# omerbt/Splice

Measured on AMD Instinct MI355X. Metric: opt_steps_per_sec, higher is better.
Workload: dtype bf16

## Files before the change

### include/splice_hip.h

```cpp
#ifndef SPLICE_HIP_H
#define SPLICE_HIP_H
#include <stddef.h>
#include <stdint.h>

#ifdef __cplusplus
extern "C" {
#endif

typedef uint16_t splice_bf16;
typedef void* splice_stream_t;

#define SPLICE_OK 0
#define SPLICE_ERR_ARG -1
#define SPLICE_ERR_HIP -2
#define SPLICE_ERR_STATE -3
#define SPLICE_ERR_NOMEM -4

int splice_version(void);
int splice_dev_switches(void);
const char* splice_last_error(void);

typedef struct splice_gemm_epilogue {
    const float* bias;
    const float* resid;
    int ldr, resid_mod;
    float* out_f32;
    int ldo;
    splice_bf16* out_bf;
    int ldbf;
    splice_bf16* out_bf_t;
    int ldt;
    splice_bf16* out_pre;
    int ldp, pre_row_lo;
    const splice_bf16* aux;
    int ldaux;
    float* out_f32_cols;
    int ld_cols, col_lo, col_hi;
    float alpha;
    int ksplit;
    long long slab_stride;
    const splice_bf16* rd_other;
    int ld_rd, rd_rows;
    float* rowdot;
    const float* row_scale;
    const float* col_scale;
    uint8_t* out_f8;
    int ld8;
    uint8_t* out_f8_t;
    int ldt8;
} splice_gemm_epilogue;

enum {
    SPLICE_EPI_BIAS = 1, SPLICE_EPI_RESID = 2, SPLICE_EPI_OUT_F32 = 4, SPLICE_EPI_OUT_BF = 8,
    SPLICE_EPI_OUT_T = 16, SPLICE_EPI_GELU = 32, SPLICE_EPI_GELU_GRAD = 64,
    SPLICE_EPI_COLS_F32 = 128, SPLICE_EPI_ALPHA = 256, SPLICE_EPI_ROWDOT = 512, SPLICE_EPI_SCALE_RC = 1024, SPLICE_EPI_OUT_F8 = 2048,
    SPLICE_EPI_OUT_F8T = 4096
};

int splice_gemm_nt_bf16(unsigned flags, const splice_bf16* A, int lda, const splice_bf16* B, int ldb,
                        int M, int N, int K, const splice_gemm_epilogue* epi, splice_stream_t stream);

int splice_gemm_nt_fp8(unsigned flags, const uint8_t* A, int lda, const uint8_t* B, int ldb, int M, int N, int K,
                       const splice_gemm_epilogue* epi, splice_stream_t stream);
int splice_quantize_rows_fp8(const float* x, int ldx, uint8_t* q, int ldq, float* scale, int rows, int cols, splice_stream_t stream);
int splice_gemm_splitk_slabs(int M, int ksplit);
int splice_gemm_force_tile(int tile);
int splice_attention_variant(int variant);
int splice_attention_qfold(int on);
int splice_attention_bwd_variant(int variant);

int splice_layernorm_fwd(const float* x, const float* gamma, const float* beta, splice_bf16* y,
                         float* mean, float* rstd, int rows, int D, float eps, splice_stream_t stream);
int splice_layernorm_bwd(const float* dy, const float* x, const float* gamma, const float* mean,
                         const float* rstd, const float* g_in, float* g_out, splice_bf16* g_out_bf,
                         int rows, int D, splice_stream_t stream);

int splice_attention_fwd(const splice_bf16* qkv, const splice_bf16* qkvT, int ldt, int B, int T, int Tld,
                         int D, int H, float scale, splice_bf16* out, float* lse, splice_stream_t stream);
int splice_attention_fwd_fp8(const uint8_t* qkv8, const uint8_t* qkvT8, int ldt8, int B, int T, int Tld, int D, int H, float scale,
                             splice_bf16* out, float* lse, splice_stream_t stream);
int splice_attention_bwd(const splice_bf16* qkv, const splice_bf16* qkvT, int ldt, int B, int T, int Tld,
                         int D, int H, float scale, const splice_bf16* out, const float* lse,
                         const splice_bf16* dout, const splice_bf16* doutT, float* delta,
                         splice_bf16* dqkv, splice_stream_t stream);
int splice_attention_probs(const splice_bf16* qkv, int B, int T, int Tld, int D, int H, float scale,
                           const float* lse, float* probs, splice_stream_t stream);

int splice_augment_structure(const float* img, float* out, float* scratch, int H, int W, int flip, int n_ops, const int* order,
                             const float* factors, float blur_sigma, splice_stream_t stream);

size_t splice_keys_selfsim_ws_bytes(int T, int D);
int splice_keys_selfsim_fwd(const float* K, int ldk, int T, int D, float eps, float* S, void* ws,
                            splice_stream_t stream);
int splice_keys_selfsim_bwd(const float* dS, const float* S, int T, int D, float eps, float* dK, int lddk,
                            int accumulate, void* ws, splice_stream_t stream);

int splice_mse(const float* a, int lda, const float* b, int ldb, int rows, int cols, float weight,
               float* loss_accum, float* grad, int ldg, splice_stream_t stream);

int splice_patchify(const float* img, splice_bf16* patches, int B, int H, int W, int p, int Tld,
                    int normalize, splice_stream_t stream);
int splice_unpatchify(const float* dpatches, float* dimg, int B, int H, int W, int p, int Tld,
                      int normalize, splice_stream_t stream);
int splice_cast_f32_bf16(const float* x, splice_bf16* y, size_t n, splice_stream_t stream);
int splice_cast_bf16_f32(const splice_bf16* x, float* y, size_t n, splice_stream_t stream);
int splice_transpose_f32_bf16(const float* x, splice_bf16* y, int rows, int cols, int ldy, splice_stream_t stream);
int splice_resize_bilinear_fwd(const float* in, float* out, int planes, int h, int w, int oh, int ow, splice_stream_t stream);
int splice_resize_bilinear_bwd(const float* dout, float* din, int planes, int h, int w, int oh, int ow, splice_stream_t stream);

int splice_vit_create(int patch, int dim, int depth, int heads, void** out_handle);
void splice_vit_destroy(void* vit);
int splice_vit_set_param(void* vit, const char* name, const float* data, long long numel, splice_stream_t stream);
float splice_vit_qscale(void* vit);
int splice_vit_params_complete(void* vit);
int splice_vit_enable_fp8(void* vit, splice_stream_t stream);
int splice_vit_ctx_create(void* vit, int B, int H, int W, const float* pos_TD, int need_grad,
                          splice_stream_t stream, void** out_ctx);
void splice_vit_ctx_destroy(void* ctx);
int splice_vit_ctx_info(void* ctx, int* T, int* Tld, int* rows);
int splice_vit_ctx_set_top_cls_only(void* ctx, int on);
int splice_vit_ctx_set_fp8(void* ctx, int mode);
int splice_vit_forward(void* ctx, const float* img, int normalize, splice_stream_t stream);
int splice_vit_forward_ex(void* ctx, const float* img, int normalize, int grad_pass_begin, splice_stream_t stream);
int splice_vit_forward_passes(void* ctx, const float* img, int normalize, int grad_pass_begin, int pass_begin, int pass_end,
                              splice_stream_t stream);
int splice_vit_get_tensor(void* ctx, int kind, int layer, void** out_ptr);
int splice_vit_read_tensor(void* ctx, int kind, int layer, void* dst, size_t bytes, splice_stream_t stream);
int splice_vit_backward(void* ctx, int pass_begin, int pass_end, const float* const* d_block,
                        const float* const* d_qkv, const float* const* d_keys, float* d_img,
                        int normalize, splice_stream_t stream);

int splice_gen_create(void** out_handle);
// ... 106 lines not shown
int splice_step_stop_state(void* step, splice_stop_state* out, splice_stream_t stream);
int splice_step_restore(void* step, int next_step_idx, const splice_stop_state* stop, splice_stream_t stream);
int splice_step_set_input_rows(void* step, int pairs_in, const int* rows);
int splice_plateau_update(splice_stop_state* state, const float* losses8, int pairs, int window, float rel, int patience, int min_steps,
                          int step_idx, int counted, splice_stream_t stream);

int splice_step_set_ema(void* step, float* ema, float decay, int start);
int splice_optim_step_pairs_ema(int kind, float* params, float* grads, const float* g2, float* m, float* v, float* ema, int n_pairs,
                                long long stride, long long n, const float* lr_dev, float hp0, float hp1, float eps, const int* step_dev,
                                const splice_stop_state* stop, int zero_grad, float ema_decay, int ema_start, splice_stream_t stream);

#define SPLICE_CLIP_CHUNK 4096
typedef struct splice_clip_state {
    float sumsq;
    float norm;
    float coef;
    int skip;
    int clipped;
    int skipped;
} splice_clip_state;
int splice_grad_norm_pairs(const float* grads, const float* g2, int n_pairs, long long stride, long long n, float max_norm, float* partials,
                           splice_clip_state* state, const splice_stop_state* stop, const int* step_dev, splice_stream_t stream);
int splice_optim_step_pairs_clip(int kind, float* params, float* grads, const float* g2, float* m, float* v, float* ema, int n_pairs,
                                 long long stride, long long n, const float* lr_dev, float hp0, float hp1, float eps, const int* step_dev,
                                 const splice_stop_state* stop, int zero_grad, float ema_decay, int ema_start, const splice_clip_state* clip,
                                 splice_stream_t stream);
int splice_optim_step_clip(int kind, float* params, float* grads, const float* g2, float* m, float* v, float* ema, long long n, float lr,
                           const float* lr_dev, float hp0, float hp1, float eps, int step, int zero_grad, float ema_decay, int ema_start,
                           const splice_clip_state* clip, splice_stream_t stream);
int splice_step_set_grad_clip(void* step, float max_norm, splice_clip_state* state);

typedef struct splice_clip_auto_state {
    float ref[2];
    int count[2];
    float thr;
    int regime;
} splice_clip_auto_state;
int splice_grad_norm_pairs_auto(const float* grads, const float* g2, int n_pairs, long long stride, long long n, float max_norm, float k,
                                float beta, int warmup, int regime, float* partials, splice_clip_state* state,
                                splice_clip_auto_state* auto_state, const splice_stop_state* stop, const int* step_dev,
                                splice_stream_t stream);
int splice_step_set_grad_clip_auto(void* step, float max_norm, float k, float beta, int warmup, splice_clip_state* state,
                                   splice_clip_auto_state* auto_state);

#define SPLICE_STOP_HISTORY 64
typedef struct splice_best_state {
    int best_step;
    int best_window;
} splice_best_state;
int splice_plateau_update_best(splice_stop_state* state, splice_best_state* best, float* means, const float* losses8, int pairs, int window,
                               float rel, int patience, int min_steps, int step_idx, int counted, splice_stream_t stream);
int splice_optim_step_pairs_best(int kind, float* params, float* grads, const float* g2, float* m, float* v, float* ema, int n_pairs,
                                 long long stride, long long n, const float* lr_dev, float hp0, float hp1, float eps, const int* step_dev,
                                 const splice_stop_state* stop, int zero_grad, float ema_decay, int ema_start, const splice_clip_state* clip,
                                 const splice_best_state* best, float* best_params, float* best_ema, splice_stream_t stream);
int splice_optim_step_pairs_ext(int kind, float* params, float* grads, const float* g2, float* m, float* v, float* w, float* ema, int n_pairs,
                                long long stride, long long n, const float* lr_dev, float hp0, float hp1, float eps, int step,
                                const int* step_dev, const splice_stop_state* stop, int zero_grad, float ema_decay, int ema_start,
                                const splice_clip_state* clip, const splice_best_state* best, float* best_params, float* best_ema,
                                const splice_optim_ext* options, splice_stream_t stream);
int splice_step_set_optimizer_ext(void* step, const splice_optim_ext* options, float* w);
int splice_step_set_keep_best(void* step, float* best_params, float* best_ema, splice_best_state* state, float* means);

int splice_step_set_loss_trace(void* step, float* trace, int capacity);

typedef struct splice_lr_state {
    float scale;
    int bad;
    int cuts;
    int last_cut_step;
} splice_lr_state;
int splice_step_set_lr_plateau(void* step, float factor, int patience, float min_scale, splice_lr_state* state, int* cut_steps);
int splice_plateau_update_lr(splice_stop_state* state, splice_lr_state* lr_state, int* cut_steps, const float* losses8, const float* lr_in,
                             int per_pair, float* lr_eff, int pairs, int window, float rel, int patience, int min_steps, float factor,
                             int lr_patience, float min_scale, int step_idx, int counted, splice_stream_t stream);

size_t splice_selfsim_loss_pairs_ws_bytes(int T, int D, int pairs);
int splice_selfsim_loss_pairs(const splice_bf16* k_tgt, const splice_bf16* k_x, int ldk, size_t k_pstride, const splice_bf16* kT_x, int ldt,
                              size_t kT_pstride, int T, int D, int pairs, float lambda, const float* e_scale_tab, int fp8, float eps,
                              float* loss_part, size_t part_pstride, float* dk, int lddk, size_t dk_pstride, void* ws, splice_stream_t stream);
int splice_mse_pairs(const float* a, int lda, size_t a_ps, const float* b, int ldb, size_t b_ps, int rows, int cols, float loss_weight,
                     float grad_weight, float* part, size_t part_ps, float* grad, int ldg, size_t g_ps, int pairs, const float* grad_tab,
                     splice_stream_t stream);
int splice_total_loss_pairs(float* lbase, size_t lstride, int lp, float w_ssim, float w_essim, float w_ecls, float w_cls, float w_id,
                            float* out8, int pairs, int n_a, int n_b, int n_c, int n_e, const float* wtab, int ssim_on, int entire,
                            splice_stream_t stream);
int splice_total_loss_pairs_trace(float* lbase, size_t lstride, int lp, float w_ssim, float w_essim, float w_ecls, float w_cls, float w_id,
                                  float* out8, int pairs, int n_a, int n_b, int n_c, int n_e, const float* wtab, int ssim_on, int entire,
                                  splice_stop_state* stop, int window, float rel, int patience, int min_steps, const int* dev_t,
                                  float* trace, int capacity, splice_stream_t stream);

int splice_attn_cls_fwd(const splice_bf16* qkv, const splice_bf16* qkvT, int ldt, int B, int T, int Tld, int D, int H, float scale, splice_bf16* out,
                        float* probs, splice_stream_t stream);
int splice_attn_cls_bwd(const splice_bf16* qkv, const splice_bf16* qkvT, int ldt, int B, int T, int Tld, int D, int H, float scale, const float* probs,
                        const float* dout_slabs, int n_slabs, size_t slab_stride, splice_bf16* dqkv, splice_stream_t stream);
int splice_ln_rows_fwd(float* x, size_t xs, const float* gamma, const float* beta, splice_bf16* y, size_t ys, float* mean, float* rstd, size_t ss,
                       int rows, int D, float eps, const float* slabs, int n_slabs, size_t slab_stride, const float* bias, const float* resid, size_t rs,
                       splice_stream_t stream);
int splice_ln_rows_bwd(float* dy, size_t dys, const float* x, size_t xs, const float* gamma, const float* mean, const float* rstd, size_t ss, float* g,
                       splice_bf16* g_bf, int rows, int D, int n_slabs, size_t slab_stride, splice_stream_t stream);
int splice_rows_finish(int mode, const float* slabs, int n_slabs, size_t slab_stride, int rows, int N, const float* bias, const float* resid, size_t rs,
                       float* out_f32, size_t os, splice_bf16* out_bf, splice_bf16* pre_bf, const splice_bf16* aux, size_t ps, int pre_lo,
                       splice_stream_t stream);

typedef struct splice_gen_conv_args {
    const float* in;
    const float* w;
    const float* bias;
    float* out;
    size_t in_nstride, in_cstride, out_nstride, out_cstride, w_jstride, w_cstride, p_nstride;
    int N, Cin, Hi, Wi, Cout, Ho, Wo, ks, stride, pad;
    int reflect, act, transposed, accumulate;
    float* ws;
    size_t ws_floats;
    int p_group, defer_reduce;
} splice_gen_conv_args;
#define SPLICE_GEN_CONV_FORM_INTS 5
int splice_gen_conv(const splice_gen_conv_args* args, int* form_out, splice_stream_t stream);
int splice_gen_conv_pair(const splice_gen_conv_args* a, const splice_gen_conv_args* b, int* forms_out, splice_stream_t stream);
int splice_gen_conv_reflect_dgrad(const splice_gen_conv_args* args, float* pad_scratch, size_t scratch_floats, splice_stream_t stream);

typedef struct splice_gen_wgrad_args {
    const float* x;
    const float* dy;
    float* ws;
    size_t ws_floats;
    size_t x_nstride, x_cstride, dy_nstride, dy_cstride;
    int N, Cin, Hi, Wi, Cout, Ho, Wo, ks, stride, pad, reflect;
} splice_gen_wgrad_args;
#define SPLICE_GEN_WGRAD_FORM_INTS 6
size_t splice_gen_conv_wgrad_ws_floats(int N, int Cin, int Cout, int ks, int Ho, int Wo);
int splice_gen_conv_wgrad(const splice_gen_wgrad_args* args, float* dw, int accumulate, int n_img, size_t p_nstride, int* form_out,
                          splice_stream_t stream);
int splice_gen_wgrad_reduce(const float* partials, int n, int chunks, float* dw, int accumulate, int n_img, size_t p_nstride, splice_stream_t stream);

typedef struct splice_gen_bn_args {
    float* y;
    float* out;
    size_t y_nstride, out_nstride;
    int N, C, HW, batch;
    const float* gamma;
    const float* beta;
    float eps, slope;
    size_t p_nstride;
    float* part;
    size_t part_floats;
    float* mean;
    float* rstd;
    const float* up_src;
    float* up_d_src;
    size_t up_src_ns, up_d_src_ns;
    int up_c0, up_h, up_w, up_Ho, up_Wo;
    const float* slabs;
    const float* bias;
    int ksplit;
    const float* da;
    float* dy;
    size_t da_nstride, dy_nstride;
    float* dgamma;
    float* dbeta;
    int accumulate;
    const float* da_slabs;
    int da_ksplit, da_accumulate;
    float* pre_y;
    size_t pre_y_ns;
    const float* pre_slabs;
    const float* pre_bias;
    int pre_ksplit, pre_C;
    const float* pre_gamma;
    const float* pre_beta;
    float* pre_mean;
    float* pre_rstd;
    float pre_slope;
    float* pre_dy;
    float* pre_dgamma;
    float* pre_dbeta;
} splice_gen_bn_args;
#define SPLICE_GEN_BN_FORM_INTS 7
// ... 19 lines not shown
```

### splice_amd/_lib.py

```python
import ctypes as C
import os

_HERE = os.path.dirname(os.path.abspath(__file__))
LIB_PATH = os.path.join(_HERE, "libsplice_hip.so")

_lib = None


class GemmEpilogue(C.Structure):
    _fields_ = [
        ("bias", C.c_void_p), ("resid", C.c_void_p), ("ldr", C.c_int), ("resid_mod", C.c_int),
        ("out_f32", C.c_void_p), ("ldo", C.c_int),
        ("out_bf", C.c_void_p), ("ldbf", C.c_int),
        ("out_bf_t", C.c_void_p), ("ldt", C.c_int),
        ("out_pre", C.c_void_p), ("ldp", C.c_int), ("pre_row_lo", C.c_int),
        ("aux", C.c_void_p), ("ldaux", C.c_int),
        ("out_f32_cols", C.c_void_p), ("ld_cols", C.c_int), ("col_lo", C.c_int), ("col_hi", C.c_int),
        ("alpha", C.c_float), ("ksplit", C.c_int), ("slab_stride", C.c_longlong),
        ("rd_other", C.c_void_p), ("ld_rd", C.c_int), ("rd_rows", C.c_int), ("rowdot", C.c_void_p),
        ("row_scale", C.c_void_p), ("col_scale", C.c_void_p),
        ("out_f8", C.c_void_p), ("ld8", C.c_int),
        ("out_f8_t", C.c_void_p), ("ldt8", C.c_int),
    ]


class GenArch(C.Structure):
    _fields_ = [("n_scales", C.c_int), ("in_channels", C.c_int), ("out_channels", C.c_int),
                ("down", C.c_int * 6), ("up", C.c_int * 6), ("skip", C.c_int * 6),
                ("filter_down", C.c_int * 6), ("filter_up", C.c_int * 6), ("filter_skip", C.c_int), ("reflect", C.c_int)]


class StepConfig(C.Structure):
    _fields_ = [
        ("crop_h", C.c_int), ("crop_w", C.c_int), ("vit_h", C.c_int), ("vit_w", C.c_int),
        ("ent_h", C.c_int), ("ent_w", C.c_int), ("ent_vit_h", C.c_int), ("ent_vit_w", C.c_int),
        ("lambda_global_cls", C.c_float), ("lambda_global_ssim", C.c_float), ("lambda_global_identity", C.c_float),
        ("lambda_entire_cls", C.c_float), ("lambda_entire_ssim", C.c_float),
        ("entire_every", C.c_int), ("cls_warmup", C.c_int),
        ("lr", C.c_float), ("beta1", C.c_float), ("beta2", C.c_float), ("eps", C.c_float),
        ("pairs", C.c_int), ("arena_stride", C.c_longlong), ("fp8_selfsim", C.c_int), ("top_cls_only", C.c_int), ("n_crops", C.c_int), ("n_crops_b", C.c_int),
    ]


class StopState(C.Structure):
    _fields_ = [("sum", C.c_float), ("count", C.c_int), ("windows", C.c_int), ("best", C.c_float), ("bad", C.c_int), ("stop_step", C.c_int)]


class ClipState(C.Structure):
    _fields_ = [("sumsq", C.c_float), ("norm", C.c_float), ("coef", C.c_float), ("skip", C.c_int), ("clipped", C.c_int), ("skipped", C.c_int)]


class ClipAutoState(C.Structure):
    _fields_ = [("ref", C.c_float * 2), ("count", C.c_int * 2), ("thr", C.c_float), ("regime", C.c_int)]


class BestState(C.Structure):
    _fields_ = [("best_step", C.c_int), ("best_window", C.c_int)]


class LrState(C.Structure):
    _fields_ = [("scale", C.c_float), ("bad", C.c_int), ("cuts", C.c_int), ("last_cut_step", C.c_int)]


class OptimExt(C.Structure):
    _fields_ = [("weight_decay", C.c_float), ("momentum", C.c_float), ("dampening", C.c_float), ("nesterov", C.c_int), ("decoupled", C.c_int),
                ("amsgrad", C.c_int), ("centered", C.c_int)]


def optim_ext(options):
    if isinstance(options, OptimExt):
        return options
    return OptimExt(float(options.get("weight_decay", 0.0)), float(options.get("momentum", 0.0)), float(options.get("dampening", 0.0)),
                    int(bool(options.get("nesterov", False))), int(bool(options.get("decoupled", False))), int(bool(options.get("amsgrad", False))),
                    int(bool(options.get("centered", False))))


class GenConvArgs(C.Structure):
    _fields_ = [("in", C.c_void_p), ("w", C.c_void_p), ("bias", C.c_void_p), ("out", C.c_void_p)] + \
               [(n, C.c_size_t) for n in ("in_nstride", "in_cstride", "out_nstride", "out_cstride", "w_jstride", "w_cstride", "p_nstride")] + \
               [(n, C.c_int) for n in ("N", "Cin", "Hi", "Wi", "Cout", "Ho", "Wo", "ks", "stride", "pad", "reflect", "act", "transposed", "accumulate")] + \
               [("ws", C.c_void_p), ("ws_floats", C.c_size_t), ("p_group", C.c_int), ("defer_reduce", C.c_int)]


class GenWgradArgs(C.Structure):
    _fields_ = [("x", C.c_void_p), ("dy", C.c_void_p), ("ws", C.c_void_p), ("ws_floats", C.c_size_t)] + \
               [(n, C.c_size_t) for n in ("x_nstride", "x_cstride", "dy_nstride", "dy_cstride")] + \
               [(n, C.c_int) for n in ("N", "Cin", "Hi", "Wi", "Cout", "Ho", "Wo", "ks", "stride", "pad", "reflect")]


class GenBnArgs(C.Structure):
    _fields_ = [("y", C.c_void_p), ("out", C.c_void_p), ("y_nstride", C.c_size_t), ("out_nstride", C.c_size_t),
                ("N", C.c_int), ("C", C.c_int), ("HW", C.c_int), ("batch", C.c_int),
                ("gamma", C.c_void_p), ("beta", C.c_void_p), ("eps", C.c_float), ("slope", C.c_float), ("p_nstride", C.c_size_t),
                ("part", C.c_void_p), ("part_floats", C.c_size_t), ("mean", C.c_void_p), ("rstd", C.c_void_p),
                ("up_src", C.c_void_p), ("up_d_src", C.c_void_p), ("up_src_ns", C.c_size_t), ("up_d_src_ns", C.c_size_t),
                ("up_c0", C.c_int), ("up_h", C.c_int), ("up_w", C.c_int), ("up_Ho", C.c_int), ("up_Wo", C.c_int),
                ("slabs", C.c_void_p), ("bias", C.c_void_p), ("ksplit", C.c_int),
                ("da", C.c_void_p), ("dy", C.c_void_p), ("da_nstride", C.c_size_t), ("dy_nstride", C.c_size_t),
                ("dgamma", C.c_void_p), ("dbeta", C.c_void_p), ("accumulate", C.c_int),
                ("da_slabs", C.c_void_p), ("da_ksplit", C.c_int), ("da_accumulate", C.c_int),
                ("pre_y", C.c_void_p), ("pre_y_ns", C.c_size_t), ("pre_slabs", C.c_void_p), ("pre_bias", C.c_void_p),
                ("pre_ksplit", C.c_int), ("pre_C", C.c_int), ("pre_gamma", C.c_void_p), ("pre_beta", C.c_void_p),
                ("pre_mean", C.c_void_p), ("pre_rstd", C.c_void_p), ("pre_slope", C.c_float),
                ("pre_dy", C.c_void_p), ("pre_dgamma", C.c_void_p), ("pre_dbeta", C.c_void_p)]


GEN_CONV_FORM_INTS, GEN_WGRAD_FORM_INTS, GEN_BN_FORM_INTS = 5, 6, 7

STOP_HISTORY = 64

EPI_BIAS, EPI_RESID, EPI_OUT_F32, EPI_OUT_BF, EPI_OUT_T = 1, 2, 4, 8, 16
EPI_GELU, EPI_GELU_GRAD, EPI_COLS_F32, EPI_ALPHA, EPI_ROWDOT, EPI_SCALE_RC, EPI_OUT_F8, EPI_OUT_F8T = 32, 64, 128, 256, 512, 1024, 2048, 4096

_vp, _i, _f, _sz, _u = C.c_void_p, C.c_int, C.c_float, C.c_size_t, C.c_uint

_SIGNATURES = {
    "splice_version": ([], C.c_int),
    "splice_dev_switches": ([], C.c_int),
    "splice_last_error": ([], C.c_char_p),
    "splice_gemm_nt_bf16": ([_u, _vp, _i, _vp, _i, _i, _i, _i, C.POINTER(GemmEpilogue), _vp], _i),
    "splice_gemm_nt_fp8": ([_u, _vp, _i, _vp, _i, _i, _i, _i, C.POINTER(GemmEpilogue), _vp], _i),
    "splice_quantize_rows_fp8": ([_vp, _i, _vp, _i, _vp, _i, _i, _vp], _i),
    "splice_gemm_splitk_slabs": ([_i, _i], _i),
    "splice_gemm_force_tile": ([_i], _i),
    "splice_attention_variant": ([_i], _i),
    "splice_attention_qfold": ([_i], _i),
    "splice_attention_bwd_variant": ([_i], _i),
    "splice_layernorm_fwd": ([_vp, _vp, _vp, _vp, _vp, _vp, _i, _i, _f, _vp], _i),
    "splice_layernorm_bwd": ([_vp, _vp, _vp, _vp, _vp, _vp, _vp, _vp, _i, _i, _vp], _i),
    "splice_attention_fwd": ([_vp, _vp, _i, _i, _i, _i, _i, _i, _f, _vp, _vp, _vp], _i),
    "splice_attention_fwd_fp8": ([_vp, _vp, _i, _i, _i, _i, _i, _i, _f, _vp, _vp, _vp], _i),
    "splice_attention_bwd": ([_vp, _vp, _i, _i, _i, _i, _i, _i, _f, _vp, _vp, _vp, _vp, _vp, _vp, _vp], _i),
    "splice_attention_probs": ([_vp, _i, _i, _i, _i, _i, _f, _vp, _vp, _vp], _i),
    "splice_augment_structure": ([_vp, _vp, _vp, _i, _i, _i, _i, C.POINTER(C.c_int), C.POINTER(C.c_float), _f, _vp], _i),
    "splice_keys_selfsim_ws_bytes": ([_i, _i], _sz),
    "splice_keys_selfsim_fwd": ([_vp, _i, _i, _i, _f, _vp, _vp, _vp], _i),
    "splice_keys_selfsim_bwd": ([_vp, _vp, _i, _i, _f, _vp, _i, _i, _vp, _vp], _i),
    "splice_mse": ([_vp, _i, _vp, _i, _i, _i, _f, _vp, _vp, _i, _vp], _i),
    "splice_selfsim_loss_pairs_ws_bytes": ([_i, _i, _i], _sz),
    "splice_selfsim_loss_pairs": ([_vp, _vp, _i, _sz, _vp, _i, _sz, _i, _i, _i, _f, _vp, _i, _f, _vp, _sz, _vp, _i, _sz, _vp, _vp], _i),
    "splice_mse_pairs": ([_vp, _i, _sz, _vp, _i, _sz, _i, _i, _f, _f, _vp, _sz, _vp, _i, _sz, _i, _vp, _vp], _i),
    "splice_total_loss_pairs": ([_vp, _sz, _i, _f, _f, _f, _f, _f, _vp, _i, _i, _i, _i, _i, _vp, _i, _i, _vp], _i),
    "splice_attn_cls_fwd": ([_vp, _vp, _i, _i, _i, _i, _i, _i, _f, _vp, _vp, _vp], _i),
    "splice_attn_cls_bwd": ([_vp, _vp, _i, _i, _i, _i, _i, _i, _f, _vp, _vp, _i, _sz, _vp, _vp], _i),
    "splice_ln_rows_fwd": ([_vp, _sz, _vp, _vp, _vp, _sz, _vp, _vp, _sz, _i, _i, _f, _vp, _i, _sz, _vp, _vp, _sz, _vp], _i),
    "splice_ln_rows_bwd": ([_vp, _sz, _vp, _sz, _vp, _vp, _vp, _sz, _vp, _vp, _i, _i, _i, _sz, _vp], _i),
    "splice_rows_finish": ([_i, _vp, _i, _sz, _i, _i, _vp, _vp, _sz, _vp, _sz, _vp, _vp, _vp, _sz, _i, _vp], _i),
    "splice_gen_conv": ([C.POINTER(GenConvArgs), C.POINTER(_i), _vp], _i),
    "splice_gen_conv_pair": ([C.POINTER(GenConvArgs), C.POINTER(GenConvArgs), C.POINTER(_i), _vp], _i),
    "splice_gen_conv_reflect_dgrad": ([C.POINTER(GenConvArgs), _vp, _sz, _vp], _i),
    "splice_gen_conv_wgrad_ws_floats": ([_i, _i, _i, _i, _i, _i], _sz),
    "splice_gen_conv_wgrad": ([C.POINTER(GenWgradArgs), _vp, _i, _i, _sz, C.POINTER(_i), _vp], _i),
    "splice_gen_wgrad_reduce": ([_vp, _i, _i, _vp, _i, _i, _sz, _vp], _i),
    "splice_gen_bn_small_instance": ([_i], _i),
    "splice_gen_bn_form": ([_i, _i, _sz, _i, C.POINTER(_i)], _i),
    "splice_gen_bn_part_floats": ([_i, _i], _sz),
    "splice_gen_bn_fwd": ([C.POINTER(GenBnArgs), _vp], _i),
    "splice_gen_bn_bwd": ([C.POINTER(GenBnArgs), _vp], _i),
    "splice_gen_upsample2x_fwd": ([_vp, _sz, _vp, _sz, _i, _i, _i, _i, _i, _i, _vp], _i),
    "splice_gen_upsample2x_bwd": ([_vp, _sz, _vp, _sz, _i, _i, _i, _i, _i, _i, _vp], _i),
    "splice_gen_sigmoid_bias_part_floats": ([_i, _i], _sz),
    "splice_gen_sigmoid_bwd_bias": ([_vp, _vp, _vp, _i, _i, _i, _vp, _sz, _sz, _i, C.POINTER(_i), _vp], _i),
    "splice_patchify": ([_vp, _vp, _i, _i, _i, _i, _i, _i, _vp], _i),
    "splice_unpatchify": ([_vp, _vp, _i, _i, _i, _i, _i, _i, _vp], _i),
    "splice_cast_f32_bf16": ([_vp, _vp, _sz, _vp], _i),
    "splice_cast_bf16_f32": ([_vp, _vp, _sz, _vp], _i),
    "splice_transpose_f32_bf16": ([_vp, _vp, _i, _i, _i, _vp], _i),
    "splice_resize_bilinear_fwd": ([_vp, _vp, _i, _i, _i, _i, _i, _vp], _i),
    "splice_resize_bilinear_bwd": ([_vp, _vp, _i, _i, _i, _i, _i, _vp], _i),
    "splice_vit_create": ([_i, _i, _i, _i, C.POINTER(_vp)], _i),
    "splice_vit_destroy": ([_vp], None),
    "splice_vit_set_param": ([_vp, C.c_char_p, _vp, C.c_longlong, _vp], _i),
    "splice_vit_params_complete": ([_vp], _i),
    "splice_vit_enable_fp8": ([_vp, _vp], _i),
    "splice_vit_ctx_create": ([_vp, _i, _i, _i, _vp, _i, _vp, C.POINTER(_vp)], _i),
    "splice_vit_ctx_destroy": ([_vp], None),
    "splice_vit_ctx_info": ([_vp, C.POINTER(_i), C.POINTER(_i), C.POINTER(_i)], _i),
    "splice_vit_ctx_set_top_cls_only": ([_vp, _i], _i),
    "splice_vit_ctx_set_fp8": ([_vp, _i], _i),
    "splice_vit_forward": ([_vp, _vp, _i, _vp], _i),
    "splice_vit_forward_ex": ([_vp, _vp, _i, _i, _vp], _i),
    "splice_vit_forward_passes": ([_vp, _vp, _i, _i, _i, _i, _vp], _i),
    "splice_vit_get_tensor": ([_vp, _i, _i, C.POINTER(_vp)], _i),
    "splice_vit_qscale": ([_vp], C.c_float),
    "splice_vit_read_tensor": ([_vp, _i, _i, _vp, _sz, _vp], _i),
    "splice_vit_backward": ([_vp, _i, _i, C.POINTER(_vp), C.POINTER(_vp), C.POINTER(_vp), _vp, _i, _vp], _i),
    "splice_gen_create": ([C.POINTER(_vp)], _i),
    "splice_gen_create_arch": ([C.POINTER(GenArch), C.POINTER(_vp)], _i),
    "splice_gen_destroy": ([_vp], None),
    "splice_gen_param_count": ([_vp], C.c_longlong),
    "splice_gen_num_tensors": ([_vp], _i),
    "splice_gen_tensor_info": ([_vp, _i, C.POINTER(C.c_char_p), C.POINTER(C.c_longlong), C.POINTER(C.c_longlong)], _i),
    "splice_gen_plan_create": ([_vp, _i, _i, _i, _i, C.POINTER(_vp)], _i),
    "splice_gen_plan_destroy": ([_vp], None),
    "splice_gen_forward": ([_vp, _vp, _vp, _vp, _vp], _i),
    "splice_gen_forward_borrowed": ([_vp, _vp, _vp, _vp, _vp], _i),
    "splice_gen_backward": ([_vp, _vp, _vp, _vp, _i, _vp], _i),
    "splice_adam_step": ([_vp, _vp, _vp, _vp, C.c_longlong, _f, _f, _f, _f, _i, _i, _vp], _i),
    "splice_optim_step": ([_i, _vp, _vp, _vp, _vp, C.c_longlong, _f, _f, _f, _f, _i, _i, _vp], _i),
    "splice_optim_step_ex": ([_i, _vp, _vp, _vp, _vp, _vp, C.c_longlong, _f, _vp, _f, _f, _f, _i, _i, _vp], _i),
    "splice_optim_step_pairs": ([_i, _vp, _vp, _vp, _vp, _vp, _i, C.c_longlong, C.c_longlong, _vp, _f, _f, _f, _i, _i, _vp], _i),
    "splice_optim_step_ema": ([_i, _vp, _vp, _vp, _vp, _vp, _vp, C.c_longlong, _f, _vp, _f, _f, _f, _i, _i, _f, _i, _vp], _i),
    "splice_optim_step_pairs_ema": ([_i, _vp, _vp, _vp, _vp, _vp, _vp, _i, C.c_longlong, C.c_longlong, _vp, _f, _f, _f, _vp, _vp, _i, _f, _i, _vp], _i),
    "splice_step_set_ema": ([_vp, _vp, _f, _i], _i),
    "splice_grad_norm_pairs": ([_vp, _vp, _i, C.c_longlong, C.c_longlong, _f, _vp, _vp, _vp, _vp, _vp], _i),
    "splice_optim_step_pairs_clip": ([_i, _vp, _vp, _vp, _vp, _vp, _vp, _i, C.c_longlong, C.c_longlong, _vp, _f, _f, _f, _vp, _vp, _i, _f, _i, _vp, _vp], _i),
    "splice_optim_step_clip": ([_i, _vp, _vp, _vp, _vp, _vp, _vp, C.c_longlong, _f, _vp, _f, _f, _f, _i, _i, _f, _i, _vp, _vp], _i),
    "splice_step_set_grad_clip": ([_vp, _f, _vp], _i),
    "splice_grad_norm_pairs_auto": ([_vp, _vp, _i, C.c_longlong, C.c_longlong, _f, _f, _f, _i, _i, _vp, _vp, _vp, _vp, _vp, _vp], _i),
    "splice_step_set_grad_clip_auto": ([_vp, _f, _f, _f, _i, _vp, _vp], _i),
    "splice_plateau_update_best": ([_vp, _vp, _vp, _vp, _i, _i, _f, _i, _i, _i, _i, _vp], _i),
    "splice_optim_step_pairs_best": ([_i, _vp, _vp, _vp, _vp, _vp, _vp, _i, C.c_longlong, C.c_longlong, _vp, _f, _f, _f, _vp, _vp, _i, _f, _i, _vp, _vp, _vp, _vp, _vp], _i),
    "splice_step_set_keep_best": ([_vp, _vp, _vp, _vp, _vp], _i),
    "splice_step_set_loss_trace": ([_vp, _vp, _i], _i),
    "splice_total_loss_pairs_trace": ([_vp, _sz, _i, _f, _f, _f, _f, _f, _vp, _i, _i, _i, _i, _i, _vp, _i, _i, _vp, _i, _f, _i, _i, _vp, _vp, _i, _vp], _i),
    "splice_step_set_lr_plateau": ([_vp, _f, _i, _f, _vp, _vp], _i),
    "splice_plateau_update_lr": ([_vp, _vp, _vp, _vp, _vp, _i, _vp, _i, _i, _f, _i, _i, _f, _i, _f, _i, _i, _vp], _i),
    "splice_optim_step_ext": ([_i, _vp, _vp, _vp, _vp, _vp, _vp, C.c_longlong, _f, _vp, _f, _f, _f, _i, _i, C.POINTER(OptimExt), _vp], _i),
    "splice_optim_step_pairs_ext": ([_i, _vp, _vp, _vp, _vp, _vp, _vp, _vp, _i, C.c_longlong, C.c_longlong, _vp, _f, _f, _f, _i, _vp, _vp, _i, _f, _i, _vp, _vp,
                                     _vp, _vp, C.POINTER(OptimExt), _vp], _i),
    "splice_step_set_optimizer_ext": ([_vp, C.POINTER(OptimExt), _vp], _i),
    "splice_prof_begin": ([_i], _i),
    "splice_prof_end": ([C.POINTER(_f), C.POINTER(_i)], _i),
    "splice_prof_end_ex": ([C.POINTER(_f), C.POINTER(_i), C.POINTER(_i)], _i),
    "splice_prof_end_detail": ([C.POINTER(_f), C.POINTER(_i), C.POINTER(_i), C.c_char_p, _i], _i),
    "splice_prof_active": ([], _i),
    "splice_step_use_graph": ([_vp, _i], _i),
# ... 69 lines not shown
```

### splice_amd/csrc/capi.hip

```cpp
#include <stdarg.h>
#include <stdio.h>

#include "gen_kernels.h"
#include "kernels.h"

static thread_local char g_err[512] = "";

void splice_set_error(const char* fmt, ...) {
    va_list ap;
    va_start(ap, fmt);
    vsnprintf(g_err, sizeof(g_err), fmt, ap);
    va_end(ap);
}

static int finish(int rc, const char* what) {
    if (rc != SPLICE_OK) {
        splice_set_error("%s: invalid argument", what);
        return rc;
    }
    const hipError_t e = hipGetLastError();
    if (e != hipSuccess) {
        splice_set_error("%s: HIP error %d (%s)", what, (int)e, hipGetErrorString(e));
        return SPLICE_ERR_HIP;
    }
// ... 52 lines not shown
    a.qkv = qkv; a.qkvT = qkvT; a.ldt = ldt; a.B = B; a.T = T; a.Tld = Tld; a.D = D; a.H = H; a.scale = scale;
    a.out = out; a.lse = lse; a.qfold = attn_qfold_hook();
    return finish(attn_fwd_launch(&a, ST(stream)), "splice_attention_fwd");
}
int splice_attention_fwd_fp8(const uint8_t* qkv8, const uint8_t* qkvT8, int ldt8, int B, int T, int Tld, int D, int H, float scale,
                             splice_bf16* out, float* lse, splice_stream_t stream) {
    if (!qkv8 || !qkvT8 || !out || !lse) return finish(SPLICE_ERR_ARG, "splice_attention_fwd_fp8");
    AttnArgs a = {};
    a.qkv8 = qkv8; a.qkvT8 = qkvT8; a.ldt8 = ldt8; a.ldt = 4; a.B = B; a.T = T; a.Tld = Tld; a.D = D; a.H = H; a.scale = scale;
    a.out = out; a.lse = lse;
    return finish(attn_fwd_launch(&a, ST(stream)), "splice_attention_fwd_fp8");
}
int splice_attention_bwd(const splice_bf16* qkv, const splice_bf16* qkvT, int ldt, int B, int T, int Tld, int D, int H,
                         float scale, const splice_bf16* out, const float* lse, const splice_bf16* dout,
                         const splice_bf16* doutT, float* delta, splice_bf16* dqkv, splice_stream_t stream) {
    AttnArgs a = {};
    a.qkv = qkv; a.qkvT = qkvT; a.ldt = ldt; a.B = B; a.T = T; a.Tld = Tld; a.D = D; a.H = H; a.scale = scale;
    a.out = const_cast<splice_bf16*>(out); a.lse = const_cast<float*>(lse);
    a.dout = dout; a.doutT = doutT; a.delta = delta; a.dqkv = dqkv; a.qfold = attn_qfold_hook();
    return finish(attn_bwd_launch(&a, ST(stream)), "splice_attention_bwd");
}
int splice_attention_probs(const splice_bf16* qkv, int B, int T, int Tld, int D, int H, float scale, const float* lse,
                           float* probs, splice_stream_t stream) {
    AttnArgs a = {};
    a.qkv = qkv; a.B = B; a.T = T; a.Tld = Tld; a.D = D; a.H = H; a.scale = scale; a.lse = const_cast<float*>(lse);
    return finish(attn_probs_launch(&a, probs, ST(stream)), "splice_attention_probs");
}

int splice_augment_structure(const float* img, float* out, float* scratch, int H, int W, int flip, int n_ops, const int* order,
                             const float* factors, float blur_sigma, splice_stream_t stream) {
    return finish(augment_structure_launch(img, out, scratch, H, W, flip, n_ops, order, factors, blur_sigma, ST(stream)), "splice_augment_structure");
}

size_t splice_keys_selfsim_ws_bytes(int T, int D) { return selfsim_ws_bytes(T, D); }
int splice_keys_selfsim_fwd(const float* K, int ldk, int T, int D, float eps, float* S, void* ws, splice_stream_t stream) {
    SelfSimWs w;
    selfsim_ws_carve(ws, T, D, &w);
    return finish(selfsim_fwd_launch(K, ldk, T, D, eps, S, w, ST(stream)), "splice_keys_selfsim_fwd");
}
int splice_keys_selfsim_bwd(const float* dS, const float* S, int T, int D, float eps, float* dK, int lddk, int accumulate,
                            void* ws, splice_stream_t stream) {
    SelfSimWs w;
    selfsim_ws_carve(ws, T, D, &w);
    return finish(selfsim_bwd_launch(dS, S, T, D, eps, dK, lddk, accumulate, w, ST(stream)), "splice_keys_selfsim_bwd");
}
int splice_mse(const float* a, int lda, const float* b, int ldb, int rows, int cols, float weight, float* loss_accum,
               float* grad, int ldg, splice_stream_t stream) {
    return finish(mse_launch(a, lda, b, ldb, rows, cols, weight, loss_accum, grad, ldg, ST(stream)), "splice_mse");
}

size_t splice_selfsim_loss_pairs_ws_bytes(int T, int D, int pairs) { return selfsim_batch_ws_bytes(T, D, pairs); }
int splice_selfsim_loss_pairs(const splice_bf16* k_tgt, const splice_bf16* k_x, int ldk, size_t k_pstride, const splice_bf16* kT_x, int ldt,
                              size_t kT_pstride, int T, int D, int pairs, float lambda, const float* e_scale_tab, int fp8, float eps,
                              float* loss_part, size_t part_pstride, float* dk, int lddk, size_t dk_pstride, void* ws, splice_stream_t stream) {
    const char* who = "splice_selfsim_loss_pairs";
    if (!k_tgt || !k_x || !kT_x || !loss_part || !dk || !ws || T < 1 || pairs < 1 || D < 64 || D % 64 || ldk < D || ldk % 8 || ldt % 8 ||
        k_pstride % 8 || kT_pstride % 8 || lddk < D)
        return finish(SPLICE_ERR_ARG, who);
    const int nt = (T + 63) / 64;
    if ((fp8 && D % 128) || (size_t)(nt * (nt + 1) / 2) > part_pstride) return finish(SPLICE_ERR_ARG, who);
    SelfSimBatch b = {};
    selfsim_batch_carve(ws, T, D, pairs, &b);
    b.ldk = ldk; b.ldt = ldt; b.k_pstride = k_pstride; b.kT_pstride = kT_pstride;
    b.k_tgt = k_tgt; b.k_x = k_x; b.kT_x = kT_x;
    b.loss_part = loss_part; b.part_pstride = part_pstride;
    b.dk = dk; b.dk_pstride = dk_pstride; b.lddk = lddk;
    b.eps = eps;
    b.fp8 = fp8 != 0;
    b.loss_scale = 1.0f / ((float)T * (float)T);
    b.e_scale = 4.0f * lambda * b.loss_scale;
    b.e_scale_tab = e_scale_tab;
    const int rc = selfsim_target_launch(b, ST(stream));
    if (rc != SPLICE_OK) return finish(rc, who);
    return finish(selfsim_loss_launch(b, ST(stream)), who);
}
int splice_mse_pairs(const float* a, int lda, size_t a_ps, const float* b, int ldb, size_t b_ps, int rows, int cols, float loss_weight,
                     float grad_weight, float* part, size_t part_ps, float* grad, int ldg, size_t g_ps, int pairs, const float* grad_tab,
                     splice_stream_t stream) {
    if (!a || !b || rows < 1 || cols < 1) return finish(SPLICE_ERR_ARG, "splice_mse_pairs");
    return finish(mse_batched_launch(a, lda, a_ps, b, ldb, b_ps, rows, cols, loss_weight, grad_weight, part, part_ps, grad, ldg, g_ps, pairs,
                                     ST(stream), grad_tab),
                  "splice_mse_pairs");
}

static bool attn_cls_args_ok(const void* qkv, const void* qkvT, int ldt, int B, int T, int Tld, int D, int H, size_t lds) {
    if (!qkv || !qkvT || B < 1 || T < 1 || T > Tld || Tld % 32 || ldt % 8 || (long long)ldt < (long long)B * Tld || D < 64 || D % 64 || H != D / 64)
        return false;
    int dev = 0, lim = 0;
    if (hipGetDevice(&dev) != hipSuccess || hipDeviceGetAttribute(&lim, hipDeviceAttributeMaxSharedMemoryPerBlock, dev) != hipSuccess) return false;
    return lds <= (size_t)(lim < 65536 ? lim : 65536);
}
int splice_attn_cls_fwd(const splice_bf16* qkv, const splice_bf16* qkvT, int ldt, int B, int T, int Tld, int D, int H, float scale, splice_bf16* out,
                        float* probs, splice_stream_t stream) {
    const char* who = "splice_attn_cls_fwd";
    if (!out || !probs || !attn_cls_args_ok(qkv, qkvT, ldt, B, T, Tld, D, H, ((size_t)Tld + Tld / 2 + 256 + 8) * sizeof(float)))
        return finish(SPLICE_ERR_ARG, who);
    return finish(attn_cls_fwd_launch(qkv, qkvT, ldt, B, T, Tld, D, H, scale, out, probs, ST(stream)), who);
}
int splice_attn_cls_bwd(const splice_bf16* qkv, const splice_bf16* qkvT, int ldt, int B, int T, int Tld, int D, int H, float scale, const float* probs,
                        const float* dout_slabs, int n_slabs, size_t slab_stride, splice_bf16* dqkv, splice_stream_t stream) {
    const char* who = "splice_attn_cls_bwd";
    if (!probs || !dout_slabs || !dqkv || n_slabs < 1 || n_slabs > 16 ||
        !attn_cls_args_ok(qkv, qkvT, ldt, B, T, Tld, D, H, ((size_t)Tld + Tld / 2 + 64 + 64 + 32 + 256 + 8) * sizeof(float)))
        return finish(SPLICE_ERR_ARG, who);
    return finish(attn_cls_bwd_launch(qkv, qkvT, ldt, B, T, Tld, D, H, scale, probs, dout_slabs, n_slabs, slab_stride, dqkv, ST(stream)), who);
}
int splice_ln_rows_fwd(float* x, size_t xs, const float* gamma, const float* beta, splice_bf16* y, size_t ys, float* mean, float* rstd, size_t ss,
                       int rows, int D, float eps, const float* slabs, int n_slabs, size_t slab_stride, const float* bias, const float* resid, size_t rs,
                       splice_stream_t stream) {
    const char* who = "splice_ln_rows_fwd";
    if (!x || !gamma || !beta || !y || !mean || !rstd || (slabs && (n_slabs < 1 || !bias || !resid))) return finish(SPLICE_ERR_ARG, who);
    return finish(ln_rows_fwd_launch(x, xs, gamma, beta, y, ys, mean, rstd, ss, rows, D, eps, slabs, n_slabs, slab_stride, bias, resid, rs, ST(stream)), who);
}
int splice_ln_rows_bwd(float* dy, size_t dys, const float* x, size_t xs, const float* gamma, const float* mean, const float* rstd, size_t ss, float* g,
                       splice_bf16* g_bf, int rows, int D, int n_slabs, size_t slab_stride, splice_stream_t stream) {
    const char* who = "splice_ln_rows_bwd";
    if (!dy || !x || !gamma || !mean || !rstd || !g || !g_bf) return finish(SPLICE_ERR_ARG, who);
    return finish(ln_rows_bwd_launch(dy, dys, x, xs, gamma, mean, rstd, ss, g, g_bf, rows, D, n_slabs, slab_stride, ST(stream)), who);
}
int splice_rows_finish(int mode, const float* slabs, int n_slabs, size_t slab_stride, int rows, int N, const float* bias, const float* resid, size_t rs,
                       float* out_f32, size_t os, splice_bf16* out_bf, splice_bf16* pre_bf, const splice_bf16* aux, size_t ps, int pre_lo,
                       splice_stream_t stream) {
    const char* who = "splice_rows_finish";
    if (mode < 0 || mode > 2 || !slabs || n_slabs < 1 || rows < 1 || N < 1 || (long long)rows * N > 0x7fffffffLL) return finish(SPLICE_ERR_ARG, who);
    if ((mode == 0 && (!out_f32 || !resid)) || (mode != 0 && !out_bf) || (mode == 2 && !aux)) return finish(SPLICE_ERR_ARG, who);
    return finish(rows_finish_launch(mode, slabs, n_slabs, slab_stride, rows, N, bias, resid, rs, out_f32, os, out_bf, pre_bf, aux, ps, pre_lo, ST(stream)), who);
}

static bool gen_conv_args_ok(const splice_gen_conv_args* g, bool reflect_dgrad) {
    if (!g || !g->in || !g->w || !g->out) return false;
    if (g->N < 1 || g->Cin < 1 || g->Hi < 1 || g->Wi < 1 || g->Cout < 1 || g->Ho < 1 || g->Wo < 1 || g->pad < 0) return false;
    if (g->ks != 1 && g->ks != 3 && g->ks != 5 && g->ks != 7) return false;
    if (g->stride != 1 && g->stride != 2) return false;
    if ((g->act != 0 && g->act != 1) || (g->reflect && g->transposed && !reflect_dgrad)) return false;
    const long long HWi = (long long)g->Hi * g->Wi, HWo = (long long)g->Ho * g->Wo;
    if (HWi > 0x1fffffffLL || HWo > 0x1fffffffLL) return false;
    if (g->in_cstride < (size_t)HWi || g->out_cstride < (size_t)HWo) return false;
    if (g->N > 1 && (g->in_nstride < (size_t)g->Cin * g->in_cstride || g->out_nstride < (size_t)g->Cout * g->out_cstride)) return false;
    if ((size_t)g->Cin * g->in_cstride > 0x1fffffffULL) return false;
    if ((size_t)g->Cout * g->w_jstride + (size_t)g->Cin * g->w_cstride + (size_t)g->ks * g->ks > 0x1fffffffULL) return false;
    if ((size_t)g->Cout * g->out_cstride > 0x7fffffffULL) return false;
    if (g->w_jstride < 1 || g->w_cstride < 1) return false;
    if (g->p_group < 0 || (g->p_group > 1 && (!g->p_nstride || g->N % g->p_group))) return false;
    if (g->reflect && !reflect_dgrad && (g->pad >= g->Hi || g->pad >= g->Wi)) return false;
    if (reflect_dgrad && (g->pad >= g->Ho || g->pad >= g->Wo || g->act)) return false;
    if (g->ws && g->ws_floats < 1) return false;
    if (g->defer_reduce && !g->ws) return false;
    return true;
}
static ConvArgs gen_conv_fill(const splice_gen_conv_args* g) {
    ConvArgs a = {};
    a.in = g->in; a.w = g->w; a.bias = g->bias; a.out = g->out;
    a.in_nstride = g->in_nstride; a.in_cstride = g->in_cstride; a.out_nstride = g->out_nstride; a.out_cstride = g->out_cstride;
    a.w_jstride = g->w_jstride; a.w_cstride = g->w_cstride; a.p_nstride = g->p_nstride;
    a.N = g->N; a.Cin = g->Cin; a.Hi = g->Hi; a.Wi = g->Wi; a.Cout = g->Cout; a.Ho = g->Ho; a.Wo = g->Wo;
    a.ks = g->ks; a.stride = g->stride; a.pad = g->pad;
    a.reflect = g->reflect; a.act = g->act; a.transposed = g->transposed; a.accumulate = g->accumulate;
    a.ws = g->ws; a.ws_floats = g->ws_floats; a.p_group = g->p_group; a.defer_reduce = g->defer_reduce;
    return a;
}
int splice_gen_conv(const splice_gen_conv_args* args, int* form_out, splice_stream_t stream) {
    const char* who = "splice_gen_conv";
    if (!gen_conv_args_ok(args, false)) return finish(SPLICE_ERR_ARG, who);
    const ConvArgs a = gen_conv_fill(args);
    if (form_out) conv_form_report(a, form_out);
    return finish(conv_launch(a, ST(stream)), who);
}
int splice_gen_conv_pair(const splice_gen_conv_args* a_args, const splice_gen_conv_args* b_args, int* forms_out, splice_stream_t stream) {
    const char* who = "splice_gen_conv_pair";
    if (!gen_conv_args_ok(a_args, false) || !gen_conv_args_ok(b_args, false)) return finish(SPLICE_ERR_ARG, who);
    const ConvArgs a = gen_conv_fill(a_args), b = gen_conv_fill(b_args);
    if (forms_out) { conv_form_report(a, forms_out); conv_form_report(b, forms_out + SPLICE_GEN_CONV_FORM_INTS); }
    return finish(conv_pair_launch(a, b, ST(stream)), who);
}
int splice_gen_conv_reflect_dgrad(const splice_gen_conv_args* args, float* pad_scratch, size_t scratch_floats, splice_stream_t stream) {
    const char* who = "splice_gen_conv_reflect_dgrad";
    if (!gen_conv_args_ok(args, true) || !pad_scratch) return finish(SPLICE_ERR_ARG, who);
    const size_t Hp = (size_t)args->Ho + 2 * args->pad, Wp = (size_t)args->Wo + 2 * args->pad;
    if (scratch_floats < (size_t)args->N * args->Cout * Hp * Wp || (size_t)args->Cout * Hp * Wp > 0x7fffffffULL) return finish(SPLICE_ERR_ARG, who);
    return finish(conv_reflect_dgrad_launch(gen_conv_fill(args), pad_scratch, ST(stream)), who);
}

static bool gen_wgrad_args_ok(const splice_gen_wgrad_args* g) {
    if (!g || !g->x || !g->dy) return false;
    if (g->N < 1 || g->Cin < 1 || g->Hi < 1 || g->Wi < 1 || g->Cout < 1 || g->Ho < 1 || g->Wo < 1 || g->pad < 0 || g->pad > 255) return false;
    if (g->ks != 1 && g->ks != 3 && g->ks != 5 && g->ks != 7) return false;
    if ((g->stride != 1 && g->stride != 2) || g->Cout > 128) return false;
    if (g->Hi > 65535 || g->Wi > 65535 || g->Ho > 65535 || g->Wo > 65535 || g->Cin > 65535) return false;
// ... 173 lines not shown
```

### splice_amd/csrc/gemm.h

```cpp
#pragma once
#include <atomic>
#include "common.h"

constexpr int GEMM_BK = 64;

typedef int mx8_t __attribute__((ext_vector_type(8)));
__device__ __forceinline__ f32x4 mfma16_fp8_mx(const u32x4& a0, const u32x4& a1, const u32x4& b0, const u32x4& b1, f32x4 c) {
    const mx8_t av = {(int)a0[0], (int)a0[1], (int)a0[2], (int)a0[3], (int)a1[0], (int)a1[1], (int)a1[2], (int)a1[3]};
    const mx8_t bv = {(int)b0[0], (int)b0[1], (int)b0[2], (int)b0[3], (int)b1[0], (int)b1[1], (int)b1[2], (int)b1[3]};
    return __builtin_amdgcn_mfma_scale_f32_16x16x128_f8f6f4(av, bv, c, 0 , 0 , 0, 0x7F7F7F7F, 0, 0x7F7F7F7F);
}

template <int BM, int BN, bool SWAP = false, bool FP8 = false, int WGM = 2>
struct GemmTile {
    static constexpr int NW = 2 * WGM;
    static constexpr int WROWS = BM / WGM;
    static constexpr int FM = WROWS / 16;
    static constexpr int FN = BN / 32;
    static constexpr int A_LOADS = BM * 8 / (64 * NW);
    static constexpr int B_LOADS = BN * 8 / (64 * NW);
    static constexpr int LDS_ELEMS = (BM + BN) * GEMM_BK;
    f32x4 acc[FM][FN];

    __device__ __forceinline__ void slice_mfma(const bf16_t* As, const bf16_t* Bs, int wm, int wn, int frow, int fchunk) {
// ... 268 lines not shown
        for (int j = 0; j < FN; ++j) { ssb[j] += __shfl_xor(ssb[j], 16, 64); ssb[j] += __shfl_xor(ssb[j], 32, 64); }
    }

    template <class F>
    __device__ __forceinline__ void for_each_cols(int m0, int n0, F&& f) {
        static_assert(SWAP, "for_each_cols needs the swapped fragment layout");
        const int lane = threadIdx.x & 63, wave = threadIdx.x >> 6;
        const int wm = wave >> 1, wn = wave & 1;
#pragma unroll
        for (int i = 0; i < FM; ++i)
#pragma unroll
            for (int j = 0; j < FN; ++j)
                f(m0 + wm * WROWS + i * 16 + (lane & 15), n0 + wn * (BN / 2) + j * 16 + (lane >> 4) * 4, acc[i][j]);
    }

    template <class F>
    __device__ __forceinline__ void for_each(int m0, int n0, F&& f) {
        const int lane = threadIdx.x & 63, wave = threadIdx.x >> 6;
        const int wm = wave >> 1, wn = wave & 1;
#pragma unroll
        for (int i = 0; i < FM; ++i)
#pragma unroll
            for (int j = 0; j < FN; ++j)
                f(m0 + wm * WROWS + i * 16 + (lane >> 4) * 4, n0 + wn * (BN / 2) + j * 16 + (lane & 15), acc[i][j]);
    }
};

constexpr int GEMM_VSPLIT_ROWS = 2401;
static inline int gemm_splitk_slabs(int M, int ks) { return (ks > 1 && M >= GEMM_VSPLIT_ROWS) ? 1 : ks; }

typedef splice_gemm_epilogue GemmEpi;
enum : unsigned {
    EPI_BIAS = SPLICE_EPI_BIAS, EPI_RESID = SPLICE_EPI_RESID, EPI_OUT_F32 = SPLICE_EPI_OUT_F32,
    EPI_OUT_BF = SPLICE_EPI_OUT_BF, EPI_OUT_T = SPLICE_EPI_OUT_T, EPI_GELU = SPLICE_EPI_GELU,
    EPI_GELU_GRAD = SPLICE_EPI_GELU_GRAD, EPI_COLS_F32 = SPLICE_EPI_COLS_F32, EPI_ALPHA = SPLICE_EPI_ALPHA,
    EPI_ROWDOT = SPLICE_EPI_ROWDOT, EPI_SCALE_RC = SPLICE_EPI_SCALE_RC, EPI_OUT_F8 = SPLICE_EPI_OUT_F8,
    EPI_OUT_F8T = SPLICE_EPI_OUT_F8T
};

template <unsigned FLAGS>
__device__ __forceinline__ void gemm_epilogue(const GemmEpi& e, int M, int N, int row0, int col, f32x4 v) {
    if (col >= N || row0 >= M) return;
    float b = 0.f;
    if (FLAGS & EPI_BIAS) b = e.bias[col];
    float x[4];
#pragma unroll
    for (int r = 0; r < 4; ++r) {
        x[r] = v[r];
        if (FLAGS & EPI_ALPHA) x[r] *= e.alpha;
        x[r] += b;
    }
    if (FLAGS & EPI_RESID) {
#pragma unroll
        for (int r = 0; r < 4; ++r)
            if (row0 + r < M) {
                const int rr = e.resid_mod ? (row0 + r) % e.resid_mod : (row0 + r);
                x[r] += e.resid[(size_t)rr * e.ldr + col];
            }
    }
    if (FLAGS & EPI_GELU_GRAD) {
#pragma unroll
        for (int r = 0; r < 4; ++r)
            if (row0 + r < M) x[r] *= gelu_grad_f(bf2f(e.aux[(size_t)(row0 + r) * e.ldaux + col]));
    }
    if (FLAGS & EPI_GELU) {
        if (e.out_pre) {
#pragma unroll
            for (int r = 0; r < 4; ++r)
                if (row0 + r < M) e.out_pre[(size_t)(row0 + r) * e.ldp + col] = f2bf(x[r]);
        }
#pragma unroll
        for (int r = 0; r < 4; ++r) x[r] = gelu_f(x[r]);
    }
    if (FLAGS & EPI_OUT_F32) {
#pragma unroll
        for (int r = 0; r < 4; ++r)
            if (row0 + r < M) e.out_f32[(size_t)(row0 + r) * e.ldo + col] = x[r];
    }
    if (FLAGS & EPI_OUT_BF) {
#pragma unroll
        for (int r = 0; r < 4; ++r)
            if (row0 + r < M) e.out_bf[(size_t)(row0 + r) * e.ldbf + col] = f2bf(x[r]);
    }
    if (FLAGS & EPI_OUT_T) {
        bf16_t* p = e.out_bf_t + (size_t)col * e.ldt + row0;
        if (row0 + 3 < M) {
            uint2 pk = {pack2bf(x[0], x[1]), pack2bf(x[2], x[3])};
            *reinterpret_cast<uint2*>(p) = pk;
        } else {
#pragma unroll
            for (int r = 0; r < 4; ++r)
                if (row0 + r < M) p[r] = f2bf(x[r]);
        }
    }
    if (FLAGS & EPI_COLS_F32) {
        if (col >= e.col_lo && col < e.col_hi) {
#pragma unroll
            for (int r = 0; r < 4; ++r)
                if (row0 + r < M) e.out_f32_cols[(size_t)(row0 + r) * e.ld_cols + (col - e.col_lo)] = x[r];
        }
    }
}

template <unsigned FLAGS, bool PRE = false>
__device__ __forceinline__ void gemm_epilogue_cols(const GemmEpi& e, int M, int N, int row, int col0, f32x4 v, float4 pre_bias = float4{},
                                                   float4 pre_resid = float4{}, uint2 pre_aux = uint2{}) {
    if (row >= M || col0 >= N) return;
    const bool full = PRE || col0 + 3 < N;
    float x[4] = {v[0], v[1], v[2], v[3]};
    if (FLAGS & EPI_ALPHA) {
#pragma unroll
        for (int r = 0; r < 4; ++r) x[r] *= e.alpha;
    }
    if (FLAGS & EPI_SCALE_RC) {
        const float rs = e.row_scale ? e.row_scale[row] : 1.0f;
#pragma unroll
        for (int r = 0; r < 4; ++r) x[r] *= rs * e.col_scale[min(col0 + r, N - 1)];
    }
    if (FLAGS & EPI_BIAS) {
        if (full) {
            const float4 b = PRE ? pre_bias : *reinterpret_cast<const float4*>(e.bias + col0);
            x[0] += b.x; x[1] += b.y; x[2] += b.z; x[3] += b.w;
        } else {
#pragma unroll
            for (int r = 0; r < 4; ++r) if (col0 + r < N) x[r] += e.bias[col0 + r];
        }
    }
    if (FLAGS & EPI_RESID) {
        const int rr = PRE ? 0 : (e.resid_mod ? row % e.resid_mod : row);
        const float* p = e.resid + (size_t)rr * e.ldr + col0;
        if (PRE || (full && !(e.ldr & 3))) {
            const float4 b = PRE ? pre_resid : *reinterpret_cast<const float4*>(p);
            x[0] += b.x; x[1] += b.y; x[2] += b.z; x[3] += b.w;
        } else {
#pragma unroll
            for (int r = 0; r < 4; ++r) if (col0 + r < N) x[r] += p[r];
        }
    }
    if (FLAGS & EPI_GELU_GRAD) {
        const bf16_t* p = e.aux + (size_t)row * e.ldaux + col0;
        if (PRE || (full && !(e.ldaux & 3))) {
            const uint2 u = PRE ? pre_aux : *reinterpret_cast<const uint2*>(p);
            x[0] *= gelu_grad_f(bf2f((bf16_t)(u.x & 0xFFFF))); x[1] *= gelu_grad_f(bf2f((bf16_t)(u.x >> 16)));
            x[2] *= gelu_grad_f(bf2f((bf16_t)(u.y & 0xFFFF))); x[3] *= gelu_grad_f(bf2f((bf16_t)(u.y >> 16)));
        } else {
#pragma unroll
            for (int r = 0; r < 4; ++r) if (col0 + r < N) x[r] *= gelu_grad_f(bf2f(p[r]));
        }
    }
    auto store_bf = [&](bf16_t* base, int ld) {
        bf16_t* p = base + (size_t)row * ld + col0;
        if (full && !(ld & 3)) *reinterpret_cast<uint2*>(p) = uint2{pack2bf(x[0], x[1]), pack2bf(x[2], x[3])};
        else {
#pragma unroll
            for (int r = 0; r < 4; ++r) if (col0 + r < N) p[r] = f2bf(x[r]);
        }
    };
    if (FLAGS & EPI_GELU) {
        if (e.out_pre && row >= e.pre_row_lo) store_bf(e.out_pre, e.ldp);
#pragma unroll
        for (int r = 0; r < 4; ++r) x[r] = gelu_f(x[r]);
    }
    if (FLAGS & EPI_OUT_F32) {
        float* p = e.out_f32 + (size_t)row * e.ldo + col0;
        if (full && !(e.ldo & 3)) *reinterpret_cast<float4*>(p) = float4{x[0], x[1], x[2], x[3]};
        else {
#pragma unroll
            for (int r = 0; r < 4; ++r) if (col0 + r < N) p[r] = x[r];
        }
    }
    if (FLAGS & EPI_OUT_BF) store_bf(e.out_bf, e.ldbf);
    if (FLAGS & EPI_OUT_T) {
#pragma unroll
        for (int r = 0; r < 4; ++r)
            if (col0 + r < N) e.out_bf_t[(size_t)(col0 + r) * e.ldt + row] = f2bf(x[r]);
    }
    if (FLAGS & EPI_COLS_F32) {
#pragma unroll
        for (int r = 0; r < 4; ++r) {
            const int c = col0 + r;
            if (c < N && c >= e.col_lo && c < e.col_hi) e.out_f32_cols[(size_t)row * e.ld_cols + (c - e.col_lo)] = x[r];
        }
    }
}

template <unsigned FLAGS, bool PRE, bool STORE_F32 = true>
__device__ __forceinline__ f32x4 gemm_frag_value(const GemmEpi& e, int M, int N, int row, int col0, f32x4 v, float4 pre_bias, float4 pre_resid,
                                                 uint2 pre_aux) {
    const bool inb = row < M && col0 < N;
    const int rowc = min(row, M - 1), colc = min(col0, N - 4);
    float x[4] = {v[0], v[1], v[2], v[3]};
    if (FLAGS & EPI_ALPHA) {
#pragma unroll
        for (int r = 0; r < 4; ++r) x[r] *= e.alpha;
    }
    if (FLAGS & EPI_SCALE_RC) {
        const float rs = e.row_scale ? e.row_scale[rowc] : 1.0f;
        const float4 cs = *reinterpret_cast<const float4*>(e.col_scale + colc);
        x[0] *= rs * cs.x; x[1] *= rs * cs.y; x[2] *= rs * cs.z; x[3] *= rs * cs.w;
    }
    if (FLAGS & EPI_BIAS) {
        const float4 b = PRE ? pre_bias : *reinterpret_cast<const float4*>(e.bias + colc);
        x[0] += b.x; x[1] += b.y; x[2] += b.z; x[3] += b.w;
    }
    if (FLAGS & EPI_RESID) {
        const int rr = e.resid_mod ? rowc % e.resid_mod : rowc;
        const float4 b = PRE ? pre_resid : *reinterpret_cast<const float4*>(e.resid + (size_t)rr * e.ldr + colc);
        x[0] += b.x; x[1] += b.y; x[2] += b.z; x[3] += b.w;
    }
    if (FLAGS & EPI_GELU_GRAD) {
        const uint2 u = PRE ? pre_aux : *reinterpret_cast<const uint2*>(e.aux + (size_t)rowc * e.ldaux + colc);
        x[0] *= gelu_grad_f(bf2f((bf16_t)(u.x & 0xFFFF))); x[1] *= gelu_grad_f(bf2f((bf16_t)(u.x >> 16)));
        x[2] *= gelu_grad_f(bf2f((bf16_t)(u.y & 0xFFFF))); x[3] *= gelu_grad_f(bf2f((bf16_t)(u.y >> 16)));
    }
    if (inb) {
        if ((FLAGS & EPI_OUT_F32) && STORE_F32) *reinterpret_cast<float4*>(e.out_f32 + (size_t)row * e.ldo + col0) = float4{x[0], x[1], x[2], x[3]};
        if (FLAGS & EPI_COLS_F32) {
#pragma unroll
            for (int r = 0; r < 4; ++r) {
                const int c = col0 + r;
                if (c >= e.col_lo && c < e.col_hi) e.out_f32_cols[(size_t)row * e.ld_cols + (c - e.col_lo)] = x[r];
            }
        }
    }
    return f32x4{x[0], x[1], x[2], x[3]};
}
template <int BM, int BN, bool TRANSPOSED>
__device__ __forceinline__ void gemm_stage_store(const f32x4 (&acc)[BM / 32][BN / 32], bf16_t* cs, bf16_t* out, int ld, int M, int N, int m0, int n0,
                                                 int row_lo) {
    constexpr int FMt = BM / 32, FNt = BN / 32;
    constexpr int R = TRANSPOSED ? BN : BM, Cc = TRANSPOSED ? BM : BN, PITCH = Cc + 8;
    const int lane = threadIdx.x & 63, wave = threadIdx.x >> 6, wm = wave >> 1, wn = wave & 1;
    __syncthreads();
#pragma unroll
    for (int i = 0; i < FMt; ++i)
#pragma unroll
        for (int j = 0; j < FNt; ++j) {
            const int lr = wm * (BM / 2) + i * 16 + (lane & 15), lc = wn * (BN / 2) + j * 16 + (lane >> 4) * 4;
            const f32x4 v = acc[i][j];
            if (!TRANSPOSED) {
                *reinterpret_cast<uint2*>(cs + lr * PITCH + lc) = uint2{pack2bf(v[0], v[1]), pack2bf(v[2], v[3])};
            } else {
#pragma unroll
                for (int r = 0; r < 4; ++r) cs[(lc + r) * PITCH + lr] = f2bf(v[r]);
            }
        }
    __syncthreads();
    const int r0 = TRANSPOSED ? n0 : m0, c0 = TRANSPOSED ? m0 : n0, Rm = TRANSPOSED ? N : M, Cm = TRANSPOSED ? M : N;
    constexpr int CH = Cc / 8;
    for (int c = threadIdx.x; c < R * CH; c += 256) {
        const int r = c / CH, k = (c % CH) * 8;
        const int gr = r0 + r, gc = c0 + k;
        if (gr >= Rm || gc >= Cm) continue;
        if (!TRANSPOSED && gr < row_lo) continue;
        const u32x4 v = *reinterpret_cast<const u32x4*>(cs + r * PITCH + k);
        bf16_t* q = out + (size_t)gr * ld + gc;
        if (gc + 7 < Cm && !(ld & 7)) st_out(reinterpret_cast<u32x4*>(q), v);
        else {
            const bf16_t* h = reinterpret_cast<const bf16_t*>(&v);
#pragma unroll
            for (int t = 0; t < 8; ++t)
                if (gc + t < Cm) q[t] = h[t];
        }
    }
}

__device__ __forceinline__ uint32_t pack4_e4m3_sat(const f32x4& v) {
    int w = 0;
    w = __builtin_amdgcn_cvt_pk_fp8_f32(fminf(fmaxf(v[0], -448.f), 448.f), fminf(fmaxf(v[1], -448.f), 448.f), w, false);
    w = __builtin_amdgcn_cvt_pk_fp8_f32(fminf(fmaxf(v[2], -448.f), 448.f), fminf(fmaxf(v[3], -448.f), 448.f), w, true);
    return (uint32_t)w;
}
template <int BM, int BN>
__device__ __forceinline__ void gemm_stage_store_f8(const f32x4 (&acc)[BM / 32][BN / 32], uint8_t* cs, uint8_t* out, int ld, int M, int N, int m0, int n0) {
    constexpr int FMt = BM / 32, FNt = BN / 32, PITCH = BN + 16, CH = BN / 16;
    const int lane = threadIdx.x & 63, wave = threadIdx.x >> 6, wm = wave >> 1, wn = wave & 1;
    __syncthreads();
#pragma unroll
    for (int i = 0; i < FMt; ++i)
#pragma unroll
        for (int j = 0; j < FNt; ++j) {
            const int lr = wm * (BM / 2) + i * 16 + (lane & 15), lc = wn * (BN / 2) + j * 16 + (lane >> 4) * 4;
            *reinterpret_cast<uint32_t*>(cs + lr * PITCH + lc) = pack4_e4m3_sat(acc[i][j]);
        }
    __syncthreads();
    for (int c = threadIdx.x; c < BM * CH; c += 256) {
        const int r = c / CH, k = (c % CH) * 16;
        const int gr = m0 + r, gc = n0 + k;
        if (gr >= M || gc >= N) continue;
        st_out(reinterpret_cast<u32x4*>(out + (size_t)gr * ld + gc), *reinterpret_cast<const u32x4*>(cs + r * PITCH + k));
    }
}

template <int BM, int BN>
__device__ __forceinline__ void gemm_stage_store_f8t(const f32x4 (&acc)[BM / 32][BN / 32], uint8_t* cs, uint8_t* out, int ld, int M, int N, int m0, int n0) {
    constexpr int FMt = BM / 32, FNt = BN / 32, PITCH = BM + 16, CH = BM / 16;
    const int lane = threadIdx.x & 63, wave = threadIdx.x >> 6, wm = wave >> 1, wn = wave & 1;
    __syncthreads();
#pragma unroll
    for (int i = 0; i < FMt; ++i)
#pragma unroll
        for (int j = 0; j < FNt; ++j) {
            const int lr = wm * (BM / 2) + i * 16 + (lane & 15), lc = wn * (BN / 2) + j * 16 + (lane >> 4) * 4;
            const uint32_t w = pack4_e4m3_sat(acc[i][j]);
#pragma unroll
            for (int r = 0; r < 4; ++r) cs[(lc + r) * PITCH + lr] = (uint8_t)(w >> (8 * r));
        }
    __syncthreads();
    for (int c = threadIdx.x; c < BN * CH; c += 256) {
        const int r = c / CH, k = (c % CH) * 16;
        const int gr = n0 + r, gc = m0 + k;
        if (gr >= N || gc >= M) continue;
        uint8_t* q = out + (size_t)gr * ld + gc;
        if (gc + 15 < M) st_out(reinterpret_cast<u32x4*>(q), *reinterpret_cast<const u32x4*>(cs + r * PITCH + k));
        else
            for (int t = 0; t < 16 && gc + t < M; ++t) q[t] = cs[r * PITCH + k + t];
    }
}

template <int BM, int BN>
__device__ __forceinline__ void gemm_stage_store_f32(const f32x4 (&acc)[BM / 32][BN / 32], float* cs, float* out, int ld, int M, int N, int m0, int n0) {
    constexpr int FMt = BM / 32, FNt = BN / 32, PITCH = BN + 4, CH = BN / 4;
    const int lane = threadIdx.x & 63, wave = threadIdx.x >> 6, wm = wave >> 1, wn = wave & 1;
    __syncthreads();
#pragma unroll
    for (int i = 0; i < FMt; ++i)
#pragma unroll
        for (int j = 0; j < FNt; ++j) {
            const int lr = wm * (BM / 2) + i * 16 + (lane & 15), lc = wn * (BN / 2) + j * 16 + (lane >> 4) * 4;
            *reinterpret_cast<f32x4*>(cs + lr * PITCH + lc) = acc[i][j];
        }
    __syncthreads();
    for (int c = threadIdx.x; c < BM * CH; c += 256) {
        const int r = c / CH, k = (c % CH) * 4;
        const int gr = m0 + r, gc = n0 + k;
        if (gr >= M || gc >= N) continue;
        st_out(reinterpret_cast<f32x4*>(out + (size_t)gr * ld + gc), *reinterpret_cast<const f32x4*>(cs + r * PITCH + k));
// ... 54 lines not shown
    GemmTile<BM, BN, true, FP8> tile;
    bool walked = false;
    if constexpr (FLAGS == EPI_OUT_F32 && NS == 2) {
        if (ksplit < -1) {
            const int vs = -ksplit, Kp = K / vs;
            f32x4 tot[GemmTile<BM, BN>::FM][GemmTile<BM, BN>::FN];
            for (int sl = 0; sl < vs; ++sl) {
                if (sl) __syncthreads();
                tile.run_glds(A, lda, B, ldb, M, N, Kp, m0, n0, gemm_smem, sl * Kp);
#pragma unroll
                for (int i = 0; i < GemmTile<BM, BN>::FM; ++i)
#pragma unroll
                    for (int j = 0; j < GemmTile<BM, BN>::FN; ++j) tot[i][j] = sl ? tot[i][j] + tile.acc[i][j] : tile.acc[i][j];
            }
#pragma unroll
            for (int i = 0; i < GemmTile<BM, BN>::FM; ++i)
#pragma unroll
                for (int j = 0; j < GemmTile<BM, BN>::FN; ++j) tile.acc[i][j] = tot[i][j];
            walked = true;
        }
    }
    constexpr bool HAS_OPERANDS = (FLAGS & (EPI_BIAS | EPI_RESID | EPI_GELU_GRAD)) != 0;
    constexpr bool STAGE_F32_FITS = (size_t)NS * GemmTile<BM, BN>::LDS_ELEMS * 2 >= (size_t)BM * (BN + 4) * 4;
    constexpr bool EARLY = NS >= 3 && !FP8;
    const bool pre_ok = HAS_OPERANDS && !(N & 3) && (!(FLAGS & EPI_RESID) || !(e.ldr & 3)) && (!(FLAGS & EPI_GELU_GRAD) || !(e.ldaux & 3));
    typedef GemmEpiOperands<BM, BN, FLAGS> Operands;
    Operands ops;
    if (walked) {
    } else if (NS == 2) tile.run_glds(A, lda, B, ldb, M, N, K, m0, n0, gemm_smem, kbeg);
    else if constexpr (EARLY)
        tile.template run_ring<(NS < 3 ? 3 : NS), Operands::NPRE, Operands::NRD>(A, lda, B, ldb, M, N, K, m0, n0, gemm_smem, kbeg, pre_ok, [&](bool pre) {
            if (Operands::NPRE && pre) ops.load_pre(e, M, N, m0, n0);
            if (Operands::NRD) ops.load_rd(e, M, m0, n0);
        });
    else tile.template run_ring<(NS < 3 ? 3 : NS)>(A, lda, B, ldb, M, N, K, m0, n0, gemm_smem, kbeg);
    const bool stage_ok = (FLAGS & EPI_OUT_BF) && !(N & 3) && (!(FLAGS & EPI_RESID) || !(e.ldr & 3)) && (!(FLAGS & EPI_GELU_GRAD) || !(e.ldaux & 3)) &&
                          (!(FLAGS & EPI_OUT_F32) || !(e.ldo & 3)) && (!(FLAGS & EPI_OUT_T) || !(e.ldt & 7));
    if constexpr ((FLAGS & EPI_OUT_F8) != 0 && (FLAGS & EPI_OUT_BF) == 0) {
        constexpr int FMt = GemmTile<BM, BN>::FM, FNt = GemmTile<BM, BN>::FN;
        static_assert((size_t)NS * GemmTile<BM, BN>::LDS_ELEMS >= (size_t)BM * (BN + 8), "the ring must hold one staged output tile");
        const int lane = threadIdx.x & 63, wave = threadIdx.x >> 6, wm = wave >> 1, wn = wave & 1;
        float4 pb[FNt];
#pragma unroll
        for (int j = 0; j < FNt; ++j)
            if (FLAGS & EPI_BIAS) pb[j] = *reinterpret_cast<const float4*>(e.bias + min(n0 + wn * (BN / 2) + j * 16 + (lane >> 4) * 4, N - 4));
#pragma unroll
        for (int i = 0; i < FMt; ++i)
#pragma unroll
            for (int j = 0; j < FNt; ++j)
                tile.acc[i][j] = gemm_frag_value<FLAGS, true>(e, M, N, m0 + wm * (BM / 2) + i * 16 + (lane & 15), n0 + wn * (BN / 2) + j * 16 + (lane >> 4) * 4,
                                                              tile.acc[i][j], pb[j], float4{}, uint2{});
        if (FLAGS & EPI_GELU) {
            if (e.out_pre) gemm_stage_store<BM, BN, false>(tile.acc, gemm_smem, e.out_pre, e.ldp, M, N, m0, n0, e.pre_row_lo);
#pragma unroll
            for (int i = 0; i < FMt; ++i)
#pragma unroll
                for (int j = 0; j < FNt; ++j)
#pragma unroll
                    for (int r = 0; r < 4; ++r) tile.acc[i][j][r] = gelu_f(tile.acc[i][j][r]);
        }
        gemm_stage_store_f8<BM, BN>(tile.acc, reinterpret_cast<uint8_t*>(gemm_smem), e.out_f8, e.ld8, M, N, m0, n0);
    } else if ((FLAGS & EPI_OUT_BF) && stage_ok) {
        constexpr int FMt = GemmTile<BM, BN>::FM, FNt = GemmTile<BM, BN>::FN;
        static_assert((size_t)NS * GemmTile<BM, BN>::LDS_ELEMS >= (size_t)BM * (BN + 8) && (size_t)NS * GemmTile<BM, BN>::LDS_ELEMS >= (size_t)BN * (BM + 8),
                      "the ring must hold one staged output tile");
        const int lane = threadIdx.x & 63, wave = threadIdx.x >> 6, wm = wave >> 1, wn = wave & 1;
        if (HAS_OPERANDS && !EARLY) ops.load_pre(e, M, N, m0, n0);
#pragma unroll
        for (int i = 0; i < FMt; ++i)
#pragma unroll
            for (int j = 0; j < FNt; ++j)
                tile.acc[i][j] = gemm_frag_value<FLAGS, HAS_OPERANDS>(e, M, N, m0 + wm * (BM / 2) + i * 16 + (lane & 15), n0 + wn * (BN / 2) + j * 16 + (lane >> 4) * 4,
                                                                      tile.acc[i][j], ops.pb[j], ops.pr[i][j], ops.pa[i][j]);
        if (FLAGS & EPI_GELU) {
            if (e.out_pre) gemm_stage_store<BM, BN, false>(tile.acc, gemm_smem, e.out_pre, e.ldp, M, N, m0, n0, e.pre_row_lo);
#pragma unroll
            for (int i = 0; i < FMt; ++i)
#pragma unroll
                for (int j = 0; j < FNt; ++j)
#pragma unroll
                    for (int r = 0; r < 4; ++r) tile.acc[i][j][r] = gelu_f(tile.acc[i][j][r]);
        }
        gemm_stage_store<BM, BN, false>(tile.acc, gemm_smem, e.out_bf, e.ldbf, M, N, m0, n0, 0);
        if (FLAGS & EPI_OUT_T) gemm_stage_store<BM, BN, true>(tile.acc, gemm_smem, e.out_bf_t, e.ldt, M, N, m0, n0, 0);
        if constexpr ((FLAGS & EPI_OUT_F8) != 0) gemm_stage_store_f8<BM, BN>(tile.acc, reinterpret_cast<uint8_t*>(gemm_smem), e.out_f8, e.ld8, M, N, m0, n0);
        if constexpr ((FLAGS & EPI_OUT_F8T) != 0) gemm_stage_store_f8t<BM, BN>(tile.acc, reinterpret_cast<uint8_t*>(gemm_smem), e.out_f8_t, e.ldt8, M, N, m0, n0);
        if (FLAGS & EPI_ROWDOT) {
#pragma unroll
            for (int i = 0; i < FMt; ++i)
#pragma unroll
                for (int j = 0; j < FNt; ++j)
#pragma unroll
                    for (int r = 0; r < 4; ++r) tile.acc[i][j][r] = bf2f(f2bf(tile.acc[i][j][r]));
        }
    } else if (STAGE_F32_FITS && (FLAGS & EPI_OUT_F32) && !(FLAGS & (EPI_OUT_BF | EPI_COLS_F32 | EPI_GELU_GRAD)) && !(N & 3) && !(e.ldo & 3) && (!(FLAGS & EPI_RESID) || !(e.ldr & 3))) {
        constexpr int FMt = GemmTile<BM, BN>::FM, FNt = GemmTile<BM, BN>::FN;
        const int lane = threadIdx.x & 63, wave = threadIdx.x >> 6, wm = wave >> 1, wn = wave & 1;
        if (HAS_OPERANDS && !EARLY) ops.load_pre(e, M, N, m0, n0);
#pragma unroll
        for (int i = 0; i < FMt; ++i)
#pragma unroll
            for (int j = 0; j < FNt; ++j)
                tile.acc[i][j] = gemm_frag_value<FLAGS, HAS_OPERANDS, false>(e, M, N, m0 + wm * (BM / 2) + i * 16 + (lane & 15),
                                                                             n0 + wn * (BN / 2) + j * 16 + (lane >> 4) * 4, tile.acc[i][j], ops.pb[j], ops.pr[i][j], uint2{});
        if constexpr (STAGE_F32_FITS) gemm_stage_store_f32<BM, BN>(tile.acc, reinterpret_cast<float*>(gemm_smem), e.out_f32, e.ldo, M, N, m0, n0);
    } else if (pre_ok) {
        constexpr int FMt = GemmTile<BM, BN>::FM, FNt = GemmTile<BM, BN>::FN;
        const int lane = threadIdx.x & 63, wave = threadIdx.x >> 6, wm = wave >> 1, wn = wave & 1;
        if (!EARLY) ops.load_pre(e, M, N, m0, n0);
#pragma unroll
        for (int i = 0; i < FMt; ++i)
#pragma unroll
            for (int j = 0; j < FNt; ++j)
                gemm_epilogue_cols<FLAGS, true>(e, M, N, m0 + wm * (BM / 2) + i * 16 + (lane & 15), n0 + wn * (BN / 2) + j * 16 + (lane >> 4) * 4,
                                                tile.acc[i][j], ops.pb[j], ops.pr[i][j], ops.pa[i][j]);
    } else {
        tile.for_each_cols(m0, n0, [&](int row, int col0, f32x4 v) { gemm_epilogue_cols<FLAGS>(e, M, N, row, col0, v); });
    }
    if (FLAGS & EPI_ROWDOT) {
        static_assert(!(FLAGS & EPI_ROWDOT) || BN == 64, "EPI_ROWDOT needs the 64-column tile");
        constexpr int FMt = GemmTile<BM, BN>::FM, FNt = GemmTile<BM, BN>::FN;
        const int lane = threadIdx.x & 63, wave = threadIdx.x >> 6, wm = wave >> 1, wn = wave & 1;
        float* red = reinterpret_cast<float*>(gemm_smem);
        __syncthreads();
        if (!EARLY) ops.load_rd(e, M, m0, n0);
#pragma unroll
        for (int i = 0; i < FMt; ++i) {
            const int lrow = wm * (BM / 2) + i * 16 + (lane & 15);
            const int row = m0 + lrow;
            float part = 0.f;
            if (row < M) {
#pragma unroll
                for (int j = 0; j < FNt; ++j) {
                    const uint2 o = ops.ov[i][j];
                    const f32x4 v = tile.acc[i][j];
                    part += bf2f(f2bf(v[0])) * bf2f((bf16_t)(o.x & 0xFFFF)) + bf2f(f2bf(v[1])) * bf2f((bf16_t)(o.x >> 16)) +
                            bf2f(f2bf(v[2])) * bf2f((bf16_t)(o.y & 0xFFFF)) + bf2f(f2bf(v[3])) * bf2f((bf16_t)(o.y >> 16));
                }
            }
            part += __shfl_xor(part, 16, 64);
            part += __shfl_xor(part, 32, 64);
            if (lane < 16) red[wn * BM + lrow] = part;
        }
        __syncthreads();
        if (threadIdx.x < BM) {
            const int row = m0 + threadIdx.x;
            if (row < M)
                e.rowdot[((size_t)(row / e.rd_rows) * (N / 64) + n0 / 64) * e.rd_rows + row % e.rd_rows] = red[threadIdx.x] + red[BM + threadIdx.x];
        }
    }
}

template <int BM, int BN, unsigned FLAGS, int NS, bool FP8 = false>
static inline void launch_gemm_nt(hipStream_t s, const bf16_t* A, int lda, const bf16_t* B, int ldb, int M, int N, int K,
                                  const GemmEpi& e) {
    const int tm = cdiv(M, BM), tn = cdiv(N, BN);
    int ksplit = (FLAGS == EPI_OUT_F32 && e.ksplit > 1 && K % (e.ksplit * GEMM_BK) == 0) ? e.ksplit : 1;
    if (NS == 2 && ksplit > 1 && gemm_splitk_slabs(M, ksplit) == 1) ksplit = -ksplit;
    const int grid = tm * tn * (ksplit > 1 ? ksplit : 1);
    int gm = 1;
    while ((gm + 1) * (gm + 1) * BM <= (tm * tn / 8 + 1) * BN && gm + 1 <= tm) ++gm;
    constexpr size_t lds = (size_t)NS * GemmTile<BM, BN>::LDS_ELEMS * sizeof(bf16_t);
    if (lds > 65536) {
        int dev = 0;
        (void)hipGetDevice(&dev);
        static std::atomic<unsigned long long> done_mask{0};
        const unsigned long long bit = 1ull << (dev & 63);
// ... 8 lines not shown
```

### splice_amd/csrc/gemm.hip

```cpp
#include "kernels.h"
#include "gemm8p.h"

static int g_force_tile = 0;
void gemm_force_tile(int t) { g_force_tile = t; }

template <unsigned FLAGS>
static int dispatch_tile(const bf16_t* A, int lda, const bf16_t* B, int ldb, int M, int N, int K, const GemmEpi& e,
                         hipStream_t s) {
    const long t128 = (long)cdiv(M, 128) * cdiv(N, 128);
    const long t12864 = (long)cdiv(M, 128) * cdiv(N, 64);
    if constexpr (FLAGS == (EPI_BIAS | EPI_OUT_BF) || FLAGS == (EPI_BIAS | EPI_GELU | EPI_OUT_BF) || FLAGS == (EPI_BIAS | EPI_RESID | EPI_OUT_F32)) {
        constexpr int on8p = 7;
        const int bit = (FLAGS & EPI_OUT_F32) ? 4 : (FLAGS & EPI_GELU) ? 2 : 1;
        const bool want = g_force_tile == 5 ? gemm8p_operands_ok(N, K, e, FLAGS) : (!g_force_tile && (on8p & bit) && gemm8p_shape_ok(M, N, K, lda, ldb, e, FLAGS));
        if (want) {
            launch_gemm8p<FLAGS>(s, A, lda, B, ldb, M, N, K, e);
            return SPLICE_OK;
        }
    }
    int tile, ring;
    if (g_force_tile && g_force_tile != 5) { tile = (FLAGS & EPI_ROWDOT) ? 3 : g_force_tile % 10; ring = g_force_tile / 10; }
    else {
        constexpr int t2min = 300;
        constexpr int t2ring = 3;
#ifndef SPLICE_T1MIN
#define SPLICE_T1MIN 230
#endif
#ifndef SPLICE_T96
#define SPLICE_T96 6
#endif
        constexpr int t1min = SPLICE_T1MIN;
        constexpr int bigm = 2401;
        tile = (FLAGS & EPI_ROWDOT) ? 3 : N <= 768 ? (M >= bigm ? 2 : 3) : t128 >= t1min ? 1 : t12864 >= t2min ? 2 : 3;
        const int ks = (FLAGS == EPI_OUT_F32 && e.ksplit > 1 && K % (e.ksplit * GEMM_BK) == 0) ? e.ksplit : 1;
        constexpr int ringk = 768;
        constexpr int ringwg = 640;
        ring = (tile == 3 && M <= 2400 && K / ks >= (ks > 1 ? 768 : ringk) && (long)cdiv(M, 64) * cdiv(N, 64) * ks <= ringwg) ? 1 : 0;
        if (tile == 2 && t2ring && M <= 2400) ring = t2ring == 3 ? 2 : 1;
        constexpr int shortns = 3;
        if (ring && tile == 3 && ks == 1 && K < 1536 && shortns == 3) ring = 2;
    }
    if constexpr ((FLAGS & EPI_ROWDOT) != 0) {
        if (ring == 2) launch_gemm_nt<64, 64, FLAGS, 3>(s, A, lda, B, ldb, M, N, K, e);
        else if (ring) launch_gemm_nt<64, 64, FLAGS, 4>(s, A, lda, B, ldb, M, N, K, e);
        else launch_gemm_nt<64, 64, FLAGS, 2>(s, A, lda, B, ldb, M, N, K, e);
    } else {
        if constexpr (FLAGS == (EPI_BIAS | EPI_RESID | EPI_OUT_F32)) {
            constexpr int t96 = SPLICE_T96;
            const long wg64 = (long)cdiv(M, 64) * cdiv(N, 64), wg96 = (long)cdiv(M, 64) * (N / 96);
            if (t96 && !(t96 == 5 && K < 1536) && !(t96 == 6 && K >= 1536) && tile == 3 && N % 96 == 0 && wg64 > 256 && wg96 <= 256) {
                if (K >= 1536 && t96 != 3) launch_gemm_nt<64, 96, FLAGS, 4>(s, A, lda, B, ldb, M, N, K, e);
                else launch_gemm_nt<64, 96, FLAGS, 3>(s, A, lda, B, ldb, M, N, K, e);
                return SPLICE_OK;
            }
        }
        if (tile == 3 && ring == 2) { launch_gemm_nt<64, 64, FLAGS, 3>(s, A, lda, B, ldb, M, N, K, e); return SPLICE_OK; }
        if (tile == 2 && ring == 2) { launch_gemm_nt<128, 64, FLAGS, 3>(s, A, lda, B, ldb, M, N, K, e); return SPLICE_OK; }
        switch (tile * 2 + (ring ? 1 : 0)) {
            case 2: launch_gemm_nt<128, 128, FLAGS, 2>(s, A, lda, B, ldb, M, N, K, e); break;
            case 3: launch_gemm_nt<128, 128, FLAGS, 4>(s, A, lda, B, ldb, M, N, K, e); break;
            case 4: launch_gemm_nt<128, 64, FLAGS, 2>(s, A, lda, B, ldb, M, N, K, e); break;
            case 5: launch_gemm_nt<128, 64, FLAGS, 4>(s, A, lda, B, ldb, M, N, K, e); break;
            case 6: launch_gemm_nt<64, 64, FLAGS, 2>(s, A, lda, B, ldb, M, N, K, e); break;
            default: launch_gemm_nt<64, 64, FLAGS, 4>(s, A, lda, B, ldb, M, N, K, e); break;
        }
    }
    return SPLICE_OK;
}

int gemm_nt_launch(unsigned flags, const bf16_t* A, int lda, const bf16_t* B, int ldb, int M, int N, int K,
                   const GemmEpi& e, hipStream_t s) {
    if (M < 1 || N < 1 || K < GEMM_BK || K % GEMM_BK || lda % 8 || ldb % 8) return SPLICE_ERR_ARG;
    if ((size_t)M * lda * sizeof(bf16_t) >= (1ull << 32) || (size_t)N * ldb * sizeof(bf16_t) >= (1ull << 32)) return SPLICE_ERR_ARG;
    if ((flags & EPI_OUT_T) && (e.ldt % 4)) return SPLICE_ERR_ARG;
    if ((flags & EPI_ROWDOT) && (N % 64 || !e.rd_other || !e.rowdot || e.rd_rows < 1 || e.ld_rd % 4)) return SPLICE_ERR_ARG;
#define CASE(F) case (F): return dispatch_tile<(F)>(A, lda, B, ldb, M, N, K, e, s)
    switch (flags) {
        CASE(EPI_BIAS | EPI_OUT_BF | EPI_OUT_T);
        CASE(EPI_BIAS | EPI_OUT_BF | EPI_OUT_T | EPI_COLS_F32);
        CASE(EPI_BIAS | EPI_OUT_F32);
        CASE(EPI_BIAS | EPI_OUT_BF);
        CASE(EPI_BIAS | EPI_RESID | EPI_OUT_F32);
        CASE(EPI_BIAS | EPI_GELU | EPI_OUT_BF);
        CASE(EPI_OUT_F32);
        CASE(EPI_OUT_F32 | EPI_ALPHA);
        CASE(EPI_OUT_BF);
        CASE(EPI_OUT_BF | EPI_OUT_T);
        CASE(EPI_OUT_BF | EPI_OUT_T | EPI_ROWDOT);
        CASE(EPI_OUT_BF | EPI_ROWDOT);
        CASE(EPI_GELU_GRAD | EPI_OUT_BF);
        default: return SPLICE_ERR_ARG;
    }
#undef CASE
}

template <unsigned FLAGS>
static int dispatch_fp8(const uint8_t* A, int lda, const uint8_t* B, int ldb, int M, int N, int K, const GemmEpi& e, hipStream_t s) {
    const bf16_t* a = reinterpret_cast<const bf16_t*>(A);
    const bf16_t* b = reinterpret_cast<const bf16_t*>(B);
    const long t128 = (long)cdiv(M, 128) * cdiv(N, 128), t12864 = (long)cdiv(M, 128) * cdiv(N, 64);
    constexpr int t1min8 = 230;
    constexpr int t2min8 = 300;
    if (N <= 768) {
        if (M >= 2401) launch_gemm_nt<128, 64, FLAGS, 2, true>(s, a, lda / 2, b, ldb / 2, M, N, K / 2, e);
        else launch_gemm_nt<64, 64, FLAGS, 4, true>(s, a, lda / 2, b, ldb / 2, M, N, K / 2, e);
    } else if (t128 >= t1min8) launch_gemm_nt<128, 128, FLAGS, 2, true>(s, a, lda / 2, b, ldb / 2, M, N, K / 2, e);
    else if (t12864 >= t2min8) launch_gemm_nt<128, 64, FLAGS, 3, true>(s, a, lda / 2, b, ldb / 2, M, N, K / 2, e);
    else launch_gemm_nt<64, 64, FLAGS, 3, true>(s, a, lda / 2, b, ldb / 2, M, N, K / 2, e);
    return SPLICE_OK;
}
int gemm_nt_fp8_launch(unsigned flags, const uint8_t* A, int lda, const uint8_t* B, int ldb, int M, int N, int K, const GemmEpi& e, hipStream_t s) {
    if (M < 1 || N < 1 || K < 128 || K % 128 || lda % 16 || ldb % 16) return SPLICE_ERR_ARG;
    if ((size_t)M * lda >= (1ull << 32) || (size_t)N * ldb >= (1ull << 32)) return SPLICE_ERR_ARG;
    if (!(flags & EPI_SCALE_RC) || !e.col_scale) return SPLICE_ERR_ARG;
    if ((flags & EPI_OUT_T) && (e.ldt % 4)) return SPLICE_ERR_ARG;
    if ((flags & EPI_OUT_F8) && (!e.out_f8 || N % 16 || e.ld8 % 16 || (e.out_pre && e.ldp % 8))) return SPLICE_ERR_ARG;
    if ((flags & EPI_OUT_F8T) && (!e.out_f8_t || e.ldt8 % 16)) return SPLICE_ERR_ARG;
    if ((flags & (EPI_OUT_F8 | EPI_OUT_F8T)) && (flags & EPI_OUT_BF) && (N % 16 || e.ldbf % 8 || ((flags & EPI_OUT_T) && e.ldt % 8))) return SPLICE_ERR_ARG;
#define CASE8(F) case (F): return dispatch_fp8<(F)>(A, lda, B, ldb, M, N, K, e, s)
    switch (flags) {
        CASE8(EPI_SCALE_RC | EPI_BIAS | EPI_OUT_BF);
        CASE8(EPI_SCALE_RC | EPI_BIAS | EPI_OUT_BF | EPI_OUT_F8 | EPI_OUT_F8T);
        CASE8(EPI_SCALE_RC | EPI_BIAS | EPI_OUT_BF | EPI_OUT_T);
        CASE8(EPI_SCALE_RC | EPI_BIAS | EPI_OUT_BF | EPI_OUT_T | EPI_COLS_F32);
        CASE8(EPI_SCALE_RC | EPI_BIAS | EPI_OUT_BF | EPI_OUT_T | EPI_OUT_F8 | EPI_OUT_F8T);
        CASE8(EPI_SCALE_RC | EPI_BIAS | EPI_OUT_BF | EPI_OUT_T | EPI_COLS_F32 | EPI_OUT_F8 | EPI_OUT_F8T);
        CASE8(EPI_SCALE_RC | EPI_OUT_F32);
        CASE8(EPI_SCALE_RC | EPI_BIAS | EPI_GELU | EPI_OUT_F8);
        CASE8(EPI_SCALE_RC | EPI_BIAS | EPI_RESID | EPI_OUT_F32);
        default: return SPLICE_ERR_ARG;
    }
#undef CASE8
}
```

### splice_amd/csrc/kernels.h

```cpp
#pragma once
#include "common.h"
#include "gemm.h"

struct AttnArgs {
    const bf16_t* qkv;
    const bf16_t* qkvT;
    int ldt;
    int B, T, Tld, D, H;
    float scale;
    bf16_t* out;
    float* lse;
    const bf16_t* dout;
    const bf16_t* doutT;
    float* delta;
    int delta_ready;
    bf16_t* dqkv;
    const uint8_t* qkv8;
    const uint8_t* qkvT8;
    int ldt8;
    int qfold;
};
int attn_fwd_launch(const AttnArgs* a, hipStream_t s);
int attn_bwd_launch(const AttnArgs* a, hipStream_t s);
int attn_probs_launch(const AttnArgs* a, float* probs, hipStream_t s);
void attn_set_variant(int v);
void attn_set_bwd_variant(int v);
int attn_qfold_hook();
void attn_set_qfold(int on);

int attn_cls_fwd_launch(const bf16_t* qkv, const bf16_t* qkvT, int ldt, int B, int T, int Tld, int D, int H, float scale, bf16_t* out, float* probs,
                        hipStream_t s);
int attn_cls_bwd_launch(const bf16_t* qkv, const bf16_t* qkvT, int ldt, int B, int T, int Tld, int D, int H, float scale, const float* probs,
                        const float* dout_slabs, int n_slabs, size_t slab_stride, bf16_t* dqkv, hipStream_t s);
int ln_rows_fwd_launch(float* x, size_t xs, const float* gamma, const float* beta, bf16_t* y, size_t ys, float* mean, float* rstd, size_t ss, int rows,
                       int D, float eps, const float* slabs, int n_slabs, size_t slab_stride, const float* bias, const float* resid, size_t rs, hipStream_t s);
int ln_rows_bwd_launch(float* dy, size_t dys, const float* x, size_t xs, const float* gamma, const float* mean, const float* rstd, size_t ss, float* g,
                       bf16_t* g_bf, int rows, int D, int n_slabs, size_t slab_stride, hipStream_t s);
int rows_finish_launch(int mode, const float* slabs, int n_slabs, size_t slab_stride, int rows, int N, const float* bias, const float* resid, size_t rs,
                       float* out_f32, size_t os, bf16_t* out_bf, bf16_t* pre_bf, const bf16_t* aux, size_t ps, int pre_lo, hipStream_t s);

int gemm_nt_launch(unsigned flags, const bf16_t* A, int lda, const bf16_t* B, int ldb, int M, int N, int K,
                   const GemmEpi& e, hipStream_t s);

void gemm_force_tile(int t);
int gemm_nt_fp8_launch(unsigned flags, const uint8_t* A, int lda, const uint8_t* B, int ldb, int M, int N, int K, const GemmEpi& e, hipStream_t s);

int layernorm_fwd_launch(const float* x, const float* gamma, const float* beta, bf16_t* y, float* mean, float* rstd,
                         int rows, int D, float eps, hipStream_t s);
int layernorm_fwd_fp8_launch(const float* x, const float* gamma, const float* beta, uint8_t* y, float* yscale, float* mean, float* rstd,
                             int rows, int D, float eps, hipStream_t s);
int quantize_rows_fp8_launch(const float* x, int ldx, uint8_t* q, int ldq, float* scale, int rows, int cols, hipStream_t s);
int quantize_rows_bf16_fp8_launch(const bf16_t* x, int ldx, uint8_t* q, int ldq, float* scale, int rows, int cols, hipStream_t s);
int quantize_keys_fp8_launch(const bf16_t* k, int ldk, size_t k_pstride, uint8_t* q, int ldq, size_t q_pstride, float* qnorm, int T, int Tp, int D,
                             int pairs, hipStream_t s);
int layernorm_bwd_launch(const float* dy, const float* x, const float* gamma, const float* mean, const float* rstd,
                         const float* g_in, float* g_out, bf16_t* g_out_bf, int rows, int D, hipStream_t s);
int layernorm_bwd_slabs_launch(const float* dy, int n_slabs, size_t slab_stride, const float* x, const float* gamma, const float* mean,
                               const float* rstd, const float* g_in, float* g_out, bf16_t* g_out_bf, int rows, int D, hipStream_t s);
int patchify_launch(const float* img, bf16_t* patches, int B, int H, int W, int p, int Tld, int normalize, hipStream_t s);
int unpatchify_launch(const float* dpatches, float* dimg, int B, int H, int W, int p, int Tld, int normalize, hipStream_t s);
int cast_f32_bf16_launch(const float* x, bf16_t* y, size_t n, hipStream_t s);
int cast_bf16_f32_launch(const bf16_t* x, float* y, size_t n, hipStream_t s);
int transpose_f32_to_bf16_launch(const float* x, bf16_t* y, int rows, int cols, int ldy, hipStream_t s);
int fill_f32_launch(float* x, float v, size_t n, hipStream_t s);
int dev_copy_launch(void* dst, const void* src, size_t bytes, hipStream_t s);
int dev_zero_launch(void* dst, size_t bytes, hipStream_t s);
int resize_bilinear_fwd_launch(const float* in, float* out, int planes, int h, int w, int oh, int ow, hipStream_t s);
int resize_bilinear_bwd_launch(const float* dout, float* din, int planes, int h, int w, int oh, int ow, hipStream_t s);
int add_f32_launch(float* y, const float* x, size_t n, hipStream_t s);

int augment_structure_launch(const float* img, float* out, float* scratch, int H, int W, int flip, int n_ops, const int* order,
                             const float* factors, float blur_sigma, hipStream_t s);

struct SelfSimWs {
    bf16_t* kbf;
    bf16_t* kbfT;
    float* norm;
    bf16_t* wmat;
    float* rowdot;
    int Tp;
};
size_t selfsim_ws_bytes(int T, int D);
void selfsim_ws_carve(void* base, int T, int D, SelfSimWs* ws);
int selfsim_fwd_launch(const float* K, int ldk, int T, int D, float eps, float* S, const SelfSimWs& ws, hipStream_t s);
int selfsim_bwd_launch(const float* dS, const float* S, int T, int D, float eps, float* dK, int lddk, int accumulate,
                       const SelfSimWs& ws, hipStream_t s);
struct SelfSimBatch {
    int T, Tp, D, pairs;
    int ldk, ldt;
    size_t k_pstride, kT_pstride;
    const bf16_t* k_tgt;
    const bf16_t* k_x;
    const bf16_t* kT_x;
    float* S_tgt;
    bf16_t* wmat;
    float *norm_tgt, *norm_x;
    float* rpart;
    float* loss_part;
    size_t part_pstride;
    float* dk;
    size_t dk_pstride; int lddk;
    float eps, e_scale, loss_scale;
    const float* e_scale_tab;
    int fp8;
    uint8_t *k8_tgt, *k8_x;
    float *qnorm_tgt, *qnorm_x;
};
size_t selfsim_batch_ws_bytes(int T, int D, int pairs);
void selfsim_batch_carve(void* base, int T, int D, int pairs, SelfSimBatch* b);
int selfsim_target_launch(const SelfSimBatch& b, hipStream_t s);
int selfsim_loss_launch(const SelfSimBatch& b, hipStream_t s);
int mse_batched_launch(const float* a, int lda, size_t a_ps, const float* b, int ldb, size_t b_ps, int rows, int cols, float loss_weight,
                       float grad_weight, float* part, size_t part_ps, float* grad, int ldg, size_t g_ps, int pairs, hipStream_t s,
                       const float* grad_tab = nullptr);
int mse_launch(const float* a, int lda, const float* b, int ldb, int rows, int cols, float weight, float* loss_accum,
               float* grad, int ldg, hipStream_t s);
#define SPLICE_MSE_PARTIALS 1024
int mse_partials_launch(const float* a, int lda, const float* b, int ldb, int rows, int cols, float loss_weight, float grad_weight,
                        float* part, float* grad, int ldg, hipStream_t s);
int mse2_launch(const float* a, int lda, const float* b, int ldb, int rows, int cols, float loss_weight, float grad_weight,
                float* loss_accum, float* grad, int ldg, hipStream_t s);
```

### splice_amd/csrc/selfsim.hip

```cpp
#include <map>
#include <mutex>
#include <utility>

#include "kernels.h"

static inline int round_up(int a, int b) { return (a + b - 1) / b * b; }
#define RC_SS(x) do { const int rc_ = (x); if (rc_ != SPLICE_OK) return rc_; } while (0)
constexpr int SS_RING = 4;
constexpr size_t SS_LDS = (size_t)SS_RING * GemmTile<64, 64>::LDS_ELEMS * sizeof(bf16_t);

size_t selfsim_ws_bytes(int T, int D) {
    const size_t Tp = round_up(T, 64);
    return Tp * D * 2 * 2 + Tp * 4 * 2 + Tp * Tp * 2 + 256;
}
void selfsim_ws_carve(void* base, int T, int D, SelfSimWs* ws) {
    const size_t Tp = round_up(T, 64);
    char* p = (char*)base;
    ws->Tp = (int)Tp;
    ws->kbf = (bf16_t*)p; p += Tp * D * 2;
    ws->kbfT = (bf16_t*)p; p += Tp * D * 2;
    ws->wmat = (bf16_t*)p; p += Tp * Tp * 2;
    ws->norm = (float*)p; p += Tp * 4;
    ws->rowdot = (float*)p;
}
// ... 377 lines not shown
    __shared__ float rdot[64];
    const int T = b.T, Tp = b.Tp, D = b.D, nt = Tp / 64, pair = blockIdx.y;
    if (b.e_scale_tab && b.e_scale_tab[pair] == 0.f) return;
    const int tiles_n = D / 64;
    const int t = xcd_remap(blockIdx.x, gridDim.x);
    const int m0 = (t / tiles_n) * 64, n0 = (t % tiles_n) * 64;
    const float* norm = b.norm_x + (size_t)pair * Tp;
    if (threadIdx.x < 64) {
        const int row = m0 + threadIdx.x;
        const float* rp = b.rpart + (size_t)pair * nt * Tp + row;
        float acc = 0.f;
        for (int k = 0; k < nt; ++k) acc += rp[(size_t)k * Tp];
        const float ni = norm[row];
        rdot[threadIdx.x] = row < T ? acc / fmaxf(ni * ni, 1e-30f) : 0.f;
    }
    __syncthreads();
    const bf16_t* W = b.wmat + (size_t)pair * Tp * Tp;
    const bf16_t* KT = b.kT_x + (size_t)pair * b.kT_pstride;
    const bf16_t* K = b.k_x + (size_t)pair * b.k_pstride;
    float* dK = b.dk + (size_t)pair * b.dk_pstride;
    GemmTile<64, 64> tile;
    tile.template run_ring<SS_RING>(W, Tp, KT, b.ldt, T, D, Tp, m0, n0, selfsim_smem);
    tile.for_each(m0, n0, [&](int row0, int col, f32x4 v) {
#pragma unroll
        for (int r = 0; r < 4; ++r) {
            const int row = row0 + r;
            if (row < T) dK[(size_t)row * b.lddk + col] = v[r] - rdot[row - m0] * bf2f(K[(size_t)row * b.ldk + col]);
        }
    });
}

int selfsim_norms_launch(const bf16_t* k, int ldk, size_t k_pstride, int T, int D, float* norm, int pairs, hipStream_t s) {
    if (D % 64 || ldk % 8) return SPLICE_ERR_ARG;
    const int Tp = round_up(T, 64);
    SPLICE_LAUNCH(selfsim_rownorm_kernel, dim3(cdiv(Tp, 4), pairs), dim3(256), 0, s, k, ldk, k_pstride, T, Tp, D, norm);
    return SPLICE_OK;
}
int selfsim_target_launch(const SelfSimBatch& b, hipStream_t s) {
    SpliceProfScope prof_scope(8); SPLICE_DEV_REGION(18);
    const int nt = b.Tp / 64;
    if (b.fp8) {
        if (b.D % 128) return SPLICE_ERR_ARG;
        RC_SS(quantize_keys_fp8_launch(b.k_tgt, b.ldk, b.k_pstride, b.k8_tgt, b.D, (size_t)b.Tp * b.D, b.qnorm_tgt, b.T, b.Tp, b.D, b.pairs, s));
        SPLICE_LAUNCH(selfsim_tgt_kernel<true>, dim3(nt * (nt + 1) / 2, b.pairs), dim3(256), SS_LDS, s, b);
        return SPLICE_OK;
    }
    SPLICE_LAUNCH(selfsim_tgt_kernel<false>, dim3(nt * (nt + 1) / 2, b.pairs), dim3(256), SS_LDS, s, b);
    return SPLICE_OK;
}
int selfsim_loss_launch(const SelfSimBatch& b, hipStream_t s) {
    SpliceProfScope prof_scope(8); SPLICE_DEV_REGION(18);
    const int nt = b.Tp / 64;
    if (nt * (nt + 1) / 2 > (int)b.part_pstride) return SPLICE_ERR_ARG;
    if (b.fp8) {
        if (b.D % 128) return SPLICE_ERR_ARG;
        RC_SS(selfsim_norms_launch(b.k_x, b.ldk, b.k_pstride, b.T, b.D, b.norm_x, b.pairs, s));
        RC_SS(quantize_keys_fp8_launch(b.k_x, b.ldk, b.k_pstride, b.k8_x, b.D, (size_t)b.Tp * b.D, b.qnorm_x, b.T, b.Tp, b.D, b.pairs, s));
        SPLICE_LAUNCH(selfsim_loss_kernel<true>, dim3(nt * (nt + 1) / 2, b.pairs), dim3(256), SS_LDS, s, b);
    } else {
        SPLICE_LAUNCH(selfsim_loss_kernel<false>, dim3(nt * (nt + 1) / 2, b.pairs), dim3(256), SS_LDS, s, b);
    }
    SPLICE_LAUNCH(selfsim_dk_kernel, dim3(nt * (b.D / 64), b.pairs), dim3(256), SS_LDS, s, b);
    return SPLICE_OK;
}
size_t selfsim_batch_ws_bytes(int T, int D, int pairs) {
    const size_t Tp = round_up(T, 64), nt = Tp / 64;
    return (size_t)pairs * (4 * Tp * 4 + nt * Tp * 4 + Tp * Tp * 2 + (size_t)T * T * 4 + 2 * Tp * D) + 2048;
}
void selfsim_batch_carve(void* base, int T, int D, int pairs, SelfSimBatch* b) {
    const size_t Tp = round_up(T, 64), nt = Tp / 64;
    char* p = (char*)base;
    b->T = T; b->Tp = (int)Tp; b->D = D; b->pairs = pairs;
    b->S_tgt = (float*)p; p += (size_t)pairs * T * T * 4; p = (char*)(((size_t)p + 255) & ~(size_t)255);
    b->wmat = (bf16_t*)p; p += (size_t)pairs * Tp * Tp * 2;
    b->norm_tgt = (float*)p; p += (size_t)pairs * Tp * 4;
    b->norm_x = (float*)p; p += (size_t)pairs * Tp * 4;
    b->qnorm_tgt = (float*)p; p += (size_t)pairs * Tp * 4;
    b->qnorm_x = (float*)p; p += (size_t)pairs * Tp * 4;
    b->rpart = (float*)p; p += (size_t)pairs * nt * Tp * 4; p = (char*)(((size_t)p + 255) & ~(size_t)255);
    b->k8_tgt = (uint8_t*)p; p += (size_t)pairs * Tp * D;
    b->k8_x = (uint8_t*)p;
}

__global__ __launch_bounds__(256) void mse_batched_kernel(const float* __restrict__ a, int lda, size_t a_ps, const float* __restrict__ bb, int ldb,
                                                          size_t b_ps, int rows, int cols, float wmean, float gmean, float* __restrict__ part,
                                                          size_t part_ps, float* __restrict__ grad, int ldg, size_t g_ps,
                                                          const float* __restrict__ gtab) {
    const int pair = blockIdx.y;
    if (gtab) {
        gmean = gtab[pair];
        if (gmean == 0.f) return;
    }
    a += (size_t)pair * a_ps; bb += (size_t)pair * b_ps; part += (size_t)pair * part_ps;
    if (grad) grad += (size_t)pair * g_ps;
    const size_t n = (size_t)rows * cols;
    float acc = 0.f;
    for (size_t i = (size_t)blockIdx.x * 256 + threadIdx.x; i < n; i += (size_t)gridDim.x * 256) {
        const int r = i / cols, c = i % cols;
        const float d = a[(size_t)r * lda + c] - bb[(size_t)r * ldb + c];
        acc += d * d;
        if (grad) grad[(size_t)r * ldg + c] = 2.0f * gmean * d;
    }
    __shared__ float red[4];
    acc = wave_sum(acc);
    if ((threadIdx.x & 63) == 0) red[threadIdx.x >> 6] = acc;
    __syncthreads();
    if (threadIdx.x == 0) part[blockIdx.x] = ((red[0] + red[1]) + (red[2] + red[3])) * wmean;
}
int mse_batched_launch(const float* a, int lda, size_t a_ps, const float* b, int ldb, size_t b_ps, int rows, int cols, float loss_weight,
                       float grad_weight, float* part, size_t part_ps, float* grad, int ldg, size_t g_ps, int pairs, hipStream_t s,
                       const float* grad_tab) {
    const size_t n = (size_t)rows * cols;
    if (!n || !part || pairs < 1) return SPLICE_ERR_ARG;
    size_t g = (n + 255) / 256;
    if (g > MSE_MAX_WG) g = MSE_MAX_WG;
    SPLICE_LAUNCH(mse_batched_kernel, dim3((unsigned)g, pairs), dim3(256), 0, s, a, lda, a_ps, b, ldb, b_ps, rows, cols, loss_weight / (float)n,
                       grad_weight / (float)n, part, part_ps, grad, ldg, g_ps, grad_tab);
    return SPLICE_OK;
}
```

### splice_amd/csrc/step_engine.hip

```cpp
#include <memory>
#include <vector>

#include <stdio.h>
#include <stdlib.h>
#include <string.h>

#include "gen_kernels.h"
#include "kernels.h"
#include "optim.h"
#include "plateau.h"
#include "step_graph.h"

enum { L_TOTAL = 0, L_GLOBAL_SSIM = 1, L_ENTIRE_SSIM = 2, L_ENTIRE_CLS = 3, L_GLOBAL_CLS = 4, L_GLOBAL_ID = 5, L_TERMS = 6 };
enum { LAM_CLS = 0, LAM_SSIM = 1, LAM_ID = 2, LAM_ECLS = 3, LAM_ESSIM = 4 };
enum { PW_ESCALE_G = 0, PW_ESCALE_E = 1, PW_CLS = 2, PW_ID = 3, PW_ECLS = 4, PW_LAMBDAS = 5, PW_ROWS = 10 };
static const int TERM_LAM[L_TERMS] = {-1, LAM_SSIM, LAM_ESSIM, LAM_ECLS, LAM_CLS, LAM_ID};
static const int TERM_ROW[L_TERMS] = {-1, PW_ESCALE_G, PW_ESCALE_E, PW_ECLS, PW_CLS, PW_ID};

struct VitView {
    void* ctx = nullptr;
    int B = 0, H = 0, W = 0, D = 0, depth = 0, heads = 0, patch = 0, T = 0, Tld = 0, rows = 0;
    float* d_block = nullptr;
    float* d_keys = nullptr;
    float* imgs = nullptr;
// ... 771 lines not shown
    SPLICE_LAUNCH(kernel, dim3(pairs), dim3(320), 0, (hipStream_t)stream, lbase, lstride, lp, w_ssim, w_essim, w_ecls, w_cls, w_id, out8, n_a, n_b, n_c, n_e, wtab,
                  ssim_on, entire, stop, dev_t, stop ? StopRule{window, rel, patience, min_steps} : StopRule{}, (splice_best_state*)nullptr, (float*)nullptr, trace,
                  capacity, NO_LR_RULE);
    return SPLICE_OK;
}

int splice_step_set_running_stats(void* h, float* running, long long stride) {
    SpliceStep* st = (SpliceStep*)h;
    if (!st || (running && st->P > 1 && stride <= 0)) return SPLICE_ERR_ARG;
    st->running = running; st->running_stride = stride;
    return SPLICE_OK;
}

static int place_passes(VitView& v, const float* src, int h, int w, int pass, int n, hipStream_t s) {
    return place_images(src, h, w, v.imgs + (size_t)pass * 3 * v.H * v.W, v.H, v.W, n, s);
}
static int zero_seeds(VitView& v, int pass, int n, hipStream_t s) {
    const size_t passD = (size_t)v.Tld * v.D;
    RC(dev_zero_launch(v.d_block + pass * passD, n * passD * sizeof(float), s));
    return dev_zero_launch(v.d_keys + pass * passD, n * passD * sizeof(float), s);
}

static int step_body(SpliceStep* st, float* params, float* grads, float* m, float* v, bool ssim_on, bool entire, hipStream_t s) {
    const splice_step_config& c = st->cfg;
    VitView &vg = st->vg, &ve = st->ve;
    const int P = st->P, Pa = st->Pa, Pb = st->Pb, pairs = st->pairs;
    const int nc = st->na < st->nb ? st->na : st->nb, Pc = pairs * nc;
    Term t[L_TERMS] = {};
    step_terms(st, ssim_on, entire, t);
    const StepPtrs ip = step_ptrs(st);
    const StepPtrs src = st->leader ? step_ptrs(st->leader) : ip;
    const bool do_gf = (st->phases & 1) != 0, do_v = (st->phases & 2) != 0, do_gb = (st->phases & 4) != 0;
    const bool gen_fwd = do_gf && !(st->ablate & 1), gen_bwd = do_gb && !(st->ablate & 2);
    auto chain_bwd = [&](VitView& vw, int p0, int p1, bool vit, float* d_img, int h, int w, float* d_lead, void* plan, float* arena, int accumulate,
                         bool gen, hipStream_t q) -> int {
        if (do_v) {
            if (vit) RC(splice_vit_backward(vw.ctx, p0, p1, vw.pb.data(), nullptr, vw.pk.data(), vw.d_imgs, 1, q));
            RC(unplace_grads(vw.d_imgs + (size_t)p0 * 3 * vw.H * vw.W, vw.H, vw.W, d_img, h, w, p1 - p0, q));
            if (st->leader) RC(add_f32_launch(d_lead, d_img, (size_t)(p1 - p0) * 3 * h * w, q));
        }
        if (gen) RC(splice_gen_backward(plan, params, d_img, arena, accumulate, q));
        return SPLICE_OK;
    };
    const int pA = 0, pB = Pa, pX = Pa + Pb, pY = 2 * Pa + Pb, pEnd = 2 * (Pa + Pb);
    const bool overlap = st->overlap && !splice_prof_active();
    hipStream_t s2 = overlap ? st->side_stream : s;
    if (overlap) {
        HIPCHK(hipEventRecord(st->ev(SpliceStep::EV_FORK), s));
        HIPCHK(hipStreamWaitEvent(s2, st->ev(SpliceStep::EV_FORK), 0));
    }
    if (gen_fwd) {
        RC(splice_gen_forward_borrowed(st->plan_b, params, src.b_in, ip.y, s2));
        if (overlap) HIPCHK(hipEventRecord(st->ev(SpliceStep::EV_GB), s2));
    }
    float *blk_g = nullptr, *qkv_g = nullptr;
    RC(splice_vit_get_tensor(vg.ctx, 0, vg.depth - 1, (void**)&blk_g));
    RC(splice_vit_get_tensor(vg.ctx, 3, vg.depth - 1, (void**)&qkv_g));
    const size_t passD = (size_t)vg.Tld * vg.D;
    SelfSimBatch sb = {};
    if (do_v) {
        RC(place_passes(vg, src.a_in, c.crop_h, c.crop_w, pA, Pa, s2));
        RC(place_passes(vg, src.b_in, st->cropb_h, st->cropb_w, pB, Pb, s2));
        if (!(st->ablate & 8)) RC(splice_vit_forward_passes(vg.ctx, vg.imgs, 1, pX, pA, pX, s2));
        RC(dev_zero_launch(st->losses, (size_t)P * st->lstride * sizeof(float), s2));
        RC(zero_seeds(vg, pX, Pa + Pb, s2));
        if (t[L_GLOBAL_SSIM].on) {
            RC(ssim_batch(st, vg, pA, pX, Pa, t[L_GLOBAL_SSIM], L_GLOBAL_SSIM, &sb));
            RC(selfsim_target_launch(sb, s2));
        }
    }
    if (overlap) HIPCHK(hipEventRecord(st->ev(SpliceStep::EV_JOIN), s2));
    if (gen_fwd) {
        RC(splice_gen_forward_borrowed(st->plan_a, params, src.a_in, ip.x, s));
        if (overlap) HIPCHK(hipStreamWaitEvent(s, st->ev(SpliceStep::EV_GB), 0));
    }
    if (do_v) {
        RC(place_passes(vg, src.x, c.crop_h, c.crop_w, pX, Pa, s));
        RC(place_passes(vg, src.y, st->cropb_h, st->cropb_w, pY, Pb, s));
        if (!(st->ablate & 16)) RC(splice_vit_forward_passes(vg.ctx, vg.imgs, 1, pX, pX, pEnd, s));
    }
    if (overlap) HIPCHK(hipStreamWaitEvent(s, st->ev(SpliceStep::EV_JOIN), 0));
    if (do_v) {
        if (t[L_GLOBAL_SSIM].on) RC(selfsim_loss_launch(sb, s));
        if (t[L_GLOBAL_CLS].on) {
            if (pairs > 1 && st->na != st->nb) {
                for (int i = 0; i < nc; ++i)
                    RC(mse_batched_launch(blk_g + (pX + i) * passD, vg.D, st->na * passD, blk_g + (pB + i) * passD, vg.D, st->nb * passD, 1, vg.D, 1.0f,
                                          t[L_GLOBAL_CLS].lambda, loss_part(st, L_GLOBAL_CLS) + (size_t)i * st->lstride, (size_t)nc * st->lstride,
                                          vg.d_block + (pX + i) * passD, vg.D, st->na * passD, pairs, s, nullptr));
            } else {
                RC(mse_batched_launch(blk_g + pX * passD, vg.D, passD, blk_g + pB * passD, vg.D, passD, 1, vg.D, 1.0f, t[L_GLOBAL_CLS].lambda,
                                      loss_part(st, L_GLOBAL_CLS), st->lstride, vg.d_block + pX * passD, vg.D, passD, Pc, s, t[L_GLOBAL_CLS].tab));
            }
        }
        if (t[L_GLOBAL_ID].on)
            RC(mse_batched_launch(keys_ptr(vg, qkv_g, pY), 3 * vg.D, 3 * passD, keys_ptr(vg, qkv_g, pB), 3 * vg.D, 3 * passD, vg.T, vg.D, 1.0f, t[L_GLOBAL_ID].lambda,
                                  loss_part(st, L_GLOBAL_ID), st->lstride, vg.d_keys + pY * passD, vg.D, passD, Pb, s, t[L_GLOBAL_ID].tab));
    }
    if (entire) {
        if (do_gf) RC(splice_gen_forward_borrowed(st->plan_e, params, src.e_in, ip.xe, s));
        if (do_v) {
            RC(place_passes(ve, src.e_in, c.ent_h, c.ent_w, 0, pairs, s));
            RC(place_passes(ve, src.xe, c.ent_h, c.ent_w, pairs, pairs, s));
            RC(splice_vit_forward_ex(ve.ctx, ve.imgs, 1, pairs, s));
            float* blk_e = nullptr;
            RC(splice_vit_get_tensor(ve.ctx, 0, ve.depth - 1, (void**)&blk_e));
            const size_t epassD = (size_t)ve.Tld * ve.D;
            RC(zero_seeds(ve, pairs, pairs, s));
            if (t[L_ENTIRE_SSIM].on) {
                SelfSimBatch se = {};
                RC(ssim_batch(st, ve, 0, pairs, pairs, t[L_ENTIRE_SSIM], L_ENTIRE_SSIM, &se));
                RC(selfsim_target_launch(se, s));
                RC(selfsim_loss_launch(se, s));
            }
            if (t[L_ENTIRE_CLS].on)
                RC(mse_batched_launch(blk_e + pairs * epassD, ve.D, epassD, blk_g + pB * passD, vg.D, st->nb * passD, 1, ve.D, 1.0f, t[L_ENTIRE_CLS].lambda,
                                      loss_part(st, L_ENTIRE_CLS), st->lstride, ve.d_block + pairs * epassD, ve.D, epassD, pairs, s, t[L_ENTIRE_CLS].tab));
        }
    }
    const bool stop_on = st->stop_rule.window > 0;
    auto bookkeeping = [&](hipStream_t q) -> int {
        if (do_v) {
            const bool grouped = st->crops_mode && pairs > 1;
            const int n1 = st->crops_mode ? P : 1;
            const auto kernel = st->lr_state ? (st->trace ? total_loss_kernel<true, true, true> : total_loss_kernel<true, false, true>)
                                : st->trace  ? (stop_on ? total_loss_kernel<true, true> : total_loss_kernel<false, true>)
                                             : (stop_on ? total_loss_kernel<true, false> : total_loss_kernel<false, false>);
            SPLICE_LAUNCH(kernel, dim3(pairs), dim3(320), 0, q, st->losses, st->lstride, (int)st->lp, t[L_GLOBAL_SSIM].lambda, t[L_ENTIRE_SSIM].lambda,
                          t[L_ENTIRE_CLS].lambda, t[L_GLOBAL_CLS].lambda, t[L_GLOBAL_ID].lambda, st->losses_out, grouped ? st->na : n1, grouped ? st->nb : n1, grouped ? nc : n1,
                          grouped ? 1 : n1, st->pw ? st->pw + (size_t)PW_LAMBDAS * P : nullptr, (int)ssim_on, (int)entire, st->stop, st->dev_t, st->stop_rule, st->best, st->best_means,
                          st->trace, st->trace_cap, st->lr_rule, st->lr_state, st->lr_cuts, (const float*)(st->pair_lr ? st->dev_lrs : st->dev_lr), st->pair_lr ? 1 : 0,
                          st->lr_eff);
        }
        if (!st->running || !gen_fwd) return SPLICE_OK;
        void* plans[3] = {st->plan_a, st->plan_b, nullptr};
        if (entire) { plans[1] = st->plan_e; plans[2] = st->plan_b; }
        return gen_running_stats_update(plans, entire ? 3 : 2, st->running, st->running_stride, 0.1f, stop_on ? st->stop : nullptr, st->dev_t, q);
    };
    const bool side_tail = overlap && !(st->ablate & 4);
    const float* adam_g2 = nullptr;
    if (!(st->ablate & 4)) {
        if (overlap) {
            HIPCHK(hipEventRecord(st->ev(SpliceStep::EV_FORK2), s));
            HIPCHK(hipStreamWaitEvent(s2, st->ev(SpliceStep::EV_FORK2), 0));
        }
        RC(chain_bwd(vg, pY, pEnd, !(st->ablate & 32), ip.dy, st->cropb_h, st->cropb_w, src.dy, st->plan_b, st->grads_b, 0, gen_bwd, s2));
        if (side_tail) {
            RC(bookkeeping(s2));
            HIPCHK(hipEventRecord(st->ev(SpliceStep::EV_JOIN2), s2));
        }
        RC(chain_bwd(vg, pX, pY, true, ip.dx, c.crop_h, c.crop_w, src.dx, st->plan_a, grads, st->accumulate, gen_bwd, s));
        if (overlap) HIPCHK(hipStreamWaitEvent(s, st->ev(SpliceStep::EV_JOIN2), 0));
        if (gen_bwd) {
            if (entire || st->skip_adam) RC(add_f32_launch(grads, st->grads_b, arena_floats(st), s));
            else adam_g2 = st->grads_b;
        }
    }
    if (entire) RC(chain_bwd(ve, pairs, 2 * pairs, true, ip.dxe, c.ent_h, c.ent_w, src.dxe, st->plan_e, grads, 1, do_gb, s));
    if (!side_tail) RC(bookkeeping(s));
    SPLICE_DEV_REGION(21);
    if (do_gb && !st->skip_adam) {
        OptimArgs a = {};
        a.kind = st->opt_kind; a.p = params; a.g = grads; a.g2 = adam_g2; a.m = m; a.v = v;
        a.n = arena_floats(st);
        a.lr = c.lr; a.hp0 = st->opt_hp0; a.hp1 = st->opt_hp1; a.eps = st->opt_eps; a.step_dev = st->dev_t;
        a.lr_dev = st->pair_lr ? st->dev_lrs : st->lr_set ? st->dev_lr : nullptr;
        a.lr_stride = st->pair_lr ? st->astride : 0;
        if (st->lr_state) { a.lr_dev = st->lr_eff; a.lr_stride = st->pairs > 1 ? st->astride : 0; }
        if (stop_on) { a.mask = st->stop; a.mask_step = st->dev_t; a.mask_stride = st->astride; }
        if (st->ema) { a.ema = st->ema; a.ema_decay = st->ema_decay; a.ema_start = st->ema_start; }
        if (st->clip) {
            ClipAutoRule rule = st->clip_rule;
            rule.regime = !ssim_on ? -1 : entire ? 1 : 0;
            RC(grad_norm_launch(grads, adam_g2, st->pairs, st->astride, (size_t)st->nparams, st->clip_norm, st->clip_partials, st->clip,
                                stop_on ? st->stop : nullptr, st->dev_t, s, st->trace, st->trace_cap, rule.records ? &rule : nullptr));
            a.clip = st->clip; a.clip_stride = st->astride;
        }
        if (st->best) { a.best = st->best; a.best_p = st->best_p; a.best_ema = st->best_ema; }
// ... 133 lines not shown
```

### splice_amd/csrc/vit_cls.hip

```cpp
#include "kernels.h"

#define LOG2E 1.4426950408889634f
constexpr int CLS_NV = 26;

__device__ __forceinline__ float block_sum256(float v, float* red) {
    v = wave_sum(v);
    __syncthreads();
    if ((threadIdx.x & 63) == 0) red[threadIdx.x >> 6] = v;
    __syncthreads();
    return (red[0] + red[1]) + (red[2] + red[3]);
}
__device__ __forceinline__ float block_max256(float v, float* red) {
    v = wave_max(v);
    __syncthreads();
    if ((threadIdx.x & 63) == 0) red[threadIdx.x >> 6] = v;
    __syncthreads();
    return fmaxf(fmaxf(red[0], red[1]), fmaxf(red[2], red[3]));
}

typedef __bf16 bf16x2v __attribute__((ext_vector_type(2)));
__device__ __forceinline__ float dot2bf(uint32_t a, uint32_t b, float acc) {
    return __builtin_amdgcn_fdot2_f32_bf16(__builtin_bit_cast(bf16x2v, a), __builtin_bit_cast(bf16x2v, b), acc, false);
}

__global__ __launch_bounds__(256) void attn_cls_fwd_kernel(const bf16_t* __restrict__ qkv, const bf16_t* __restrict__ qkvT, int ldt, int T, int Tld, int D,
                                                           float scale, bf16_t* __restrict__ out, float* __restrict__ probs) {
    extern __shared__ __attribute__((aligned(16))) float cls_smem[];
    float* p = cls_smem;
    uint32_t* pb = reinterpret_cast<uint32_t*>(p + Tld);
    float* po = reinterpret_cast<float*>(pb + Tld / 2);
    float* red = po + 256;
    const int h = blockIdx.x, b = blockIdx.y, H = gridDim.x;
    const size_t row0 = (size_t)b * Tld;
    const int d = threadIdx.x & 63, part = threadIdx.x >> 6;
    const bf16_t* vt = qkvT + (size_t)(2 * D + h * 64 + d) * ldt + row0;
    u32x4 qv[8], vpre[CLS_NV], kv[4][8];
    {
        const u32x4* qr = reinterpret_cast<const u32x4*>(qkv + row0 * 3 * D + h * 64);
#pragma unroll
        for (int c = 0; c < 8; ++c) qv[c] = qr[c];
    }
#pragma unroll
    for (int i = 0; i < CLS_NV; ++i) vpre[i] = *reinterpret_cast<const u32x4*>(vt + min(8 * part + 32 * i, Tld - 8));
    auto load_keys = [&](int j0) {
#pragma unroll
        for (int u = 0; u < 4; ++u) {
            const u32x4* kr = reinterpret_cast<const u32x4*>(qkv + (row0 + min(j0 + 256 * u, T - 1)) * 3 * D + D + h * 64);
#pragma unroll
            for (int c = 0; c < 8; ++c) kv[u][c] = kr[c];
        }
    };
    load_keys(threadIdx.x);
    float mx = -1e30f;
    for (int j0 = threadIdx.x; j0 < T; j0 += 4 * 256) {
        if (j0 != (int)threadIdx.x) load_keys(j0);
#pragma unroll
        for (int u = 0; u < 4; ++u) {
            const int j = j0 + 256 * u;
            if (j >= T) break;
            float s = 0.f;
#pragma unroll
            for (int c = 0; c < 8; ++c)
#pragma unroll
                for (int e = 0; e < 4; ++e) s = dot2bf(qv[c][e], kv[u][c][e], s);
            s *= scale;
            p[j] = s;
            mx = fmaxf(mx, s);
        }
    }
    mx = block_max256(mx, red);
    float sum = 0.f;
    for (int j = threadIdx.x; j < Tld; j += 256) {
        const float e = j < T ? __builtin_amdgcn_exp2f((p[j] - mx) * LOG2E) : 0.f;
        p[j] = e;
        sum += e;
    }
    sum = block_sum256(sum, red);
    const float inv = 1.0f / sum;
    float* pg = probs + ((size_t)b * H + h) * Tld;
    for (int j2 = threadIdx.x; j2 < Tld / 2; j2 += 256) {
        const float v0 = p[2 * j2] * inv, v1 = p[2 * j2 + 1] * inv;
        *reinterpret_cast<float2*>(pg + 2 * j2) = float2{v0, v1};
        pb[j2] = pack2bf(v0, v1);
    }
    __syncthreads();
    float acc = 0.f;
#pragma unroll
    for (int i = 0; i < CLS_NV; ++i) {
        const int j = 8 * part + 32 * i;
        if (j < Tld) {
            const u32x4 pv = *reinterpret_cast<const u32x4*>(pb + j / 2);
#pragma unroll
            for (int e = 0; e < 4; ++e) acc = dot2bf(pv[e], vpre[i][e], acc);
        }
    }
#pragma unroll 2
    for (int j = 8 * part + 32 * CLS_NV; j < Tld; j += 32) {
        const u32x4 v = *reinterpret_cast<const u32x4*>(vt + j);
        const u32x4 pv = *reinterpret_cast<const u32x4*>(pb + j / 2);
#pragma unroll
        for (int e = 0; e < 4; ++e) acc = dot2bf(pv[e], v[e], acc);
    }
    po[part * 64 + d] = acc;
    __syncthreads();
    if (threadIdx.x < 64) out[(size_t)b * D + h * 64 + threadIdx.x] = f2bf((po[threadIdx.x] + po[64 + threadIdx.x]) + (po[128 + threadIdx.x] + po[192 + threadIdx.x]));
}

__global__ __launch_bounds__(256) void attn_cls_bwd_kernel(const bf16_t* __restrict__ qkv, const bf16_t* __restrict__ qkvT, int ldt, int T, int Tld, int D,
                                                           float scale, const float* __restrict__ probs, const float* __restrict__ dout ,
                                                           int n_slabs, size_t slab_stride, bf16_t* __restrict__ dqkv) {
    extern __shared__ __attribute__((aligned(16))) float cls_smem[];
    float* ds = cls_smem;
    uint32_t* dsb = reinterpret_cast<uint32_t*>(ds + Tld);
    float* q = reinterpret_cast<float*>(dsb + Tld / 2);
    float* dO = q + 64;
    uint32_t* dOb = reinterpret_cast<uint32_t*>(dO + 64);
    float* pq = reinterpret_cast<float*>(dOb + 32);
    float* red = pq + 256;
    const int h = blockIdx.x, b = blockIdx.y, H = gridDim.x, z = blockIdx.z, nz = gridDim.z;
    const size_t row0 = (size_t)b * Tld;
    const float* pg = probs + ((size_t)b * H + h) * Tld;
    if (threadIdx.x < 64) {
        q[threadIdx.x] = bf2f(qkv[row0 * 3 * D + h * 64 + threadIdx.x]);
        float sv[16];
#pragma unroll
        for (int sl = 0; sl < 16; ++sl) sv[sl] = dout[(size_t)min(sl, n_slabs - 1) * slab_stride + (size_t)b * D + h * 64 + threadIdx.x];
        float v = 0.f;
#pragma unroll
        for (int sl = 0; sl < 16; ++sl)
            if (sl < n_slabs) v += sv[sl];
        const bf16_t vb = f2bf(v);
        dO[threadIdx.x] = bf2f(vb);
        reinterpret_cast<bf16_t*>(dOb)[threadIdx.x] = vb;
    }
    const int d = threadIdx.x & 63, part = threadIdx.x >> 6;
    const bf16_t* kt = qkvT + (size_t)(D + h * 64 + d) * ldt + row0;
    u32x4 kpre[CLS_NV], vv[4][8];
    float pj4[4];
    if (z == 0) {
#pragma unroll
        for (int i = 0; i < CLS_NV; ++i) kpre[i] = *reinterpret_cast<const u32x4*>(kt + min(8 * part + 32 * i, Tld - 8));
    }
    auto load_values = [&](int j0) {
#pragma unroll
        for (int u = 0; u < 4; ++u) {
            const int jc = min(j0 + 256 * u, T - 1);
            const u32x4* vr = reinterpret_cast<const u32x4*>(qkv + (row0 + jc) * 3 * D + 2 * D + h * 64);
#pragma unroll
            for (int c = 0; c < 8; ++c) vv[u][c] = vr[c];
            pj4[u] = pg[jc];
        }
    };
    load_values(threadIdx.x);
    __syncthreads();
    u32x4 dov[8];
#pragma unroll
    for (int c = 0; c < 8; ++c) dov[c] = *reinterpret_cast<const u32x4*>(dOb + 4 * c);
    float dl = 0.f;
    for (int j0 = threadIdx.x; j0 < T; j0 += 4 * 256) {
        if (j0 != (int)threadIdx.x) load_values(j0);
#pragma unroll
        for (int u = 0; u < 4; ++u) {
            const int j = j0 + 256 * u;
            if (j >= T) break;
            float s = 0.f;
#pragma unroll
            for (int c = 0; c < 8; ++c)
#pragma unroll
                for (int e = 0; e < 4; ++e) s = dot2bf(dov[c][e], vv[u][c][e], s);
            ds[j] = s;
            dl += pj4[u] * s;
        }
    }
    const float delta = block_sum256(dl, red);
    for (int j = threadIdx.x; j < Tld; j += 256) {
        const float pj = j < T ? pg[j] : 0.f;
        const float dsj = j < T ? pj * (ds[j] - delta) * scale : 0.f;
        reinterpret_cast<bf16_t*>(dsb)[j] = f2bf(dsj);
        if ((j >> 8) % nz != z) continue;
        bf16_t* r = dqkv + (row0 + j) * 3 * D + h * 64;
        u32x4* rq = reinterpret_cast<u32x4*>(r);
        u32x4* rk = reinterpret_cast<u32x4*>(r + D);
        u32x4* rv = reinterpret_cast<u32x4*>(r + 2 * D);
#pragma unroll 2
        for (int c = 0; c < 8; ++c) {
            if (j != 0) rq[c] = u32x4{0u, 0u, 0u, 0u};
            if (j >= T) {
                rk[c] = u32x4{0u, 0u, 0u, 0u};
                rv[c] = u32x4{0u, 0u, 0u, 0u};
                continue;
            }
            rk[c] =u32x4{pack2bf(dsj * q[8 * c], dsj * q[8 * c + 1]), pack2bf(dsj * q[8 * c + 2], dsj * q[8 * c + 3]),
                          pack2bf(dsj * q[8 * c + 4], dsj * q[8 * c + 5]), pack2bf(dsj * q[8 * c + 6], dsj * q[8 * c + 7])};
            rv[c] = u32x4{pack2bf(pj * dO[8 * c], pj * dO[8 * c + 1]), pack2bf(pj * dO[8 * c + 2], pj * dO[8 * c + 3]),
                          pack2bf(pj * dO[8 * c + 4], pj * dO[8 * c + 5]), pack2bf(pj * dO[8 * c + 6], pj * dO[8 * c + 7])};
        }
    }
    if (z != 0) return;
    __syncthreads();
    float acc = 0.f;
#pragma unroll
    for (int i = 0; i < CLS_NV; ++i) {
        const int j = 8 * part + 32 * i;
        if (j < Tld) {
            const u32x4 dv4 = *reinterpret_cast<const u32x4*>(dsb + j / 2);
#pragma unroll
            for (int e = 0; e < 4; ++e) acc = dot2bf(dv4[e], kpre[i][e], acc);
        }
    }
#pragma unroll 2
    for (int j = 8 * part + 32 * CLS_NV; j < Tld; j += 32) {
        const u32x4 v = *reinterpret_cast<const u32x4*>(kt + j);
        const u32x4 dv4 = *reinterpret_cast<const u32x4*>(dsb + j / 2);
#pragma unroll
        for (int e = 0; e < 4; ++e) acc = dot2bf(dv4[e], v[e], acc);
    }
    pq[part * 64 + d] = acc;
    __syncthreads();
    if (threadIdx.x < 64)
        dqkv[row0 * 3 * D + h * 64 + threadIdx.x] = f2bf((pq[threadIdx.x] + pq[64 + threadIdx.x]) + (pq[128 + threadIdx.x] + pq[192 + threadIdx.x]));
}

int attn_cls_fwd_launch(const bf16_t* qkv, const bf16_t* qkvT, int ldt, int B, int T, int Tld, int D, int H, float scale, bf16_t* out, float* probs,
                        hipStream_t s) {
    if (D / 64 != H || D % 64) return SPLICE_ERR_ARG;
    const size_t lds = (size_t)(Tld + Tld / 2 + 256 + 8) * sizeof(float);
    SPLICE_LAUNCH(attn_cls_fwd_kernel, dim3(H, B), dim3(256), lds, s, qkv, qkvT, ldt, T, Tld, D, scale, out, probs);
    return SPLICE_OK;
}
int attn_cls_bwd_launch(const bf16_t* qkv, const bf16_t* qkvT, int ldt, int B, int T, int Tld, int D, int H, float scale, const float* probs,
                        const float* dout_slabs, int n_slabs, size_t slab_stride, bf16_t* dqkv, hipStream_t s) {
    if (D / 64 != H || D % 64 || n_slabs < 1 || n_slabs > 16) return SPLICE_ERR_ARG;
    const size_t lds = (size_t)(Tld + Tld / 2 + 64 + 64 + 32 + 256 + 8) * sizeof(float);
    const int nz = Tld > 768 ? 4 : Tld > 256 ? 2 : 1;
    SPLICE_LAUNCH(attn_cls_bwd_kernel, dim3(H, B, nz), dim3(256), lds, s, qkv, qkvT, ldt, T, Tld, D, scale, probs, dout_slabs, n_slabs, slab_stride, dqkv);
    return SPLICE_OK;
}

constexpr int LNR_MAXC = 3;
constexpr int LNR_SB = 16;
__global__ __launch_bounds__(256) void ln_rows_fwd_kernel(float* __restrict__ x, size_t xs, const float* __restrict__ gamma, const float* __restrict__ beta,
                                                          bf16_t* __restrict__ y, size_t ys, float* __restrict__ mean_o, float* __restrict__ rstd_o, size_t ss,
                                                          int rows, int D, float eps, const float* __restrict__ slabs, int n_slabs, size_t slab_stride,
                                                          const float* __restrict__ bias, const float* __restrict__ resid, size_t rs) {
    __shared__ float red[4];
    const int row = blockIdx.x;
    float* xr = x + (size_t)row * xs;
    float v[LNR_MAXC], gv[LNR_MAXC], bv[LNR_MAXC];
#pragma unroll
    for (int i = 0; i < LNR_MAXC; ++i) {
        const int c = min((int)threadIdx.x + 256 * i, D - 1);
        gv[i] = gamma[c]; bv[i] = beta[c];
        v[i] = slabs ? bias[c] + resid[(size_t)row * rs + c] : xr[c];
    }
    if (slabs) {
        for (int s0 = 0; s0 < n_slabs; s0 += LNR_SB) {
            float t[LNR_SB][LNR_MAXC];
#pragma unroll
            for (int k = 0; k < LNR_SB; ++k) {
                const int sl = min(s0 + k, n_slabs - 1);
#pragma unroll
                for (int i = 0; i < LNR_MAXC; ++i) t[k][i] = slabs[(size_t)sl * slab_stride + (size_t)row * D + min((int)threadIdx.x + 256 * i, D - 1)];
            }
#pragma unroll
            for (int k = 0; k < LNR_SB; ++k)
                if (s0 + k < n_slabs) {
#pragma unroll
                    for (int i = 0; i < LNR_MAXC; ++i) v[i] += t[k][i];
                }
        }
#pragma unroll
        for (int i = 0; i < LNR_MAXC; ++i)
            if ((int)threadIdx.x + 256 * i < D) xr[threadIdx.x + 256 * i] = v[i];
    }
    float sum = 0.f;
#pragma unroll
    for (int i = 0; i < LNR_MAXC; ++i)
        if ((int)threadIdx.x + 256 * i < D) sum += v[i];
    const float mean = block_sum256(sum, red) / (float)D;
    float sq = 0.f;
#pragma unroll
    for (int i = 0; i < LNR_MAXC; ++i)
        if ((int)threadIdx.x + 256 * i < D) { const float d = v[i] - mean; sq += d * d; }
    const float rstd = rsqrtf(block_sum256(sq, red) / (float)D + eps);
    if (threadIdx.x == 0) { mean_o[(size_t)row * ss] = mean; rstd_o[(size_t)row * ss] = rstd; }
    bf16_t* yr = y + (size_t)row * ys;
#pragma unroll
    for (int i = 0; i < LNR_MAXC; ++i)
        if ((int)threadIdx.x + 256 * i < D) yr[threadIdx.x + 256 * i] = f2bf((v[i] - mean) * rstd * gv[i] + bv[i]);
}
__global__ __launch_bounds__(256) void ln_rows_bwd_kernel(float* __restrict__ dy, size_t dys, const float* __restrict__ x, size_t xs,
                                                          const float* __restrict__ gamma, const float* __restrict__ mean_i, const float* __restrict__ rstd_i,
                                                          size_t ss, float* __restrict__ g, bf16_t* __restrict__ g_bf, int rows, int D, int n_slabs,
                                                          size_t slab_stride) {
    __shared__ float red[4];
    const int row = blockIdx.x;
    const float* xr = x + (size_t)row * xs;
    float* dr = dy + (size_t)row * dys;
    float* gr = g + (size_t)row * xs;
    bf16_t* gb = g_bf + (size_t)row * xs;
    const float mean = mean_i[(size_t)row * ss], rstd = rstd_i[(size_t)row * ss];
    float v[LNR_MAXC], gv[LNR_MAXC], xv[LNR_MAXC], g0[LNR_MAXC];
#pragma unroll
    for (int i = 0; i < LNR_MAXC; ++i) {
        const int c = min((int)threadIdx.x + 256 * i, D - 1);
        v[i] = dr[c]; gv[i] = gamma[c]; xv[i] = xr[c]; g0[i] = gr[c];
    }
    if (n_slabs > 1) {
        for (int s0 = 1; s0 < n_slabs; s0 += LNR_SB) {
            float t[LNR_SB][LNR_MAXC];
#pragma unroll
            for (int k = 0; k < LNR_SB; ++k) {
                const int sl = min(s0 + k, n_slabs - 1);
#pragma unroll
                for (int i = 0; i < LNR_MAXC; ++i) t[k][i] = dr[(size_t)sl * slab_stride + min((int)threadIdx.x + 256 * i, D - 1)];
            }
#pragma unroll
            for (int k = 0; k < LNR_SB; ++k)
// ... 74 lines not shown
```

### splice_amd/csrc/vit_engine.hip

```cpp
#include <string.h>

#include <string>
#include <vector>

#include "kernels.h"


struct Linear {
    bf16_t* w = nullptr;
    bf16_t* wT = nullptr;
    float* b = nullptr;
    int out = 0, in = 0;
    uint8_t* w8 = nullptr;
    float* w8_scale = nullptr;
};
struct LayerW {
    float *ln1_g = nullptr, *ln1_b = nullptr, *ln2_g = nullptr, *ln2_b = nullptr;
    Linear qkv, proj, fc1, fc2;
};

struct SpliceVit {
    int patch = 0, dim = 0, depth = 0, heads = 0, hidden = 0;
    int device = 0;
    std::vector<LayerW> layers;
// ... 199 lines not shown
    v->fp8 = 1;
    return SPLICE_OK;
}

float splice_vit_qscale(void* h) { return h ? ((SpliceVit*)h)->qscale : 1.0f; }

int splice_vit_params_complete(void* h) {
    SpliceVit* v = (SpliceVit*)h;
    if (!v) return 0;
    bool ok = v->cls && v->pos && v->pe.w && v->pe.b;
    for (auto& L : v->layers)
        ok = ok && L.ln1_g && L.ln1_b && L.ln2_g && L.ln2_b && L.qkv.w && L.qkv.b && L.proj.w && L.proj.b && L.fc1.w &&
             L.fc1.b && L.fc2.w && L.fc2.b;
    return ok ? 1 : 0;
}

int splice_vit_ctx_create(void* h, int B, int H, int W, const float* pos_TD, int need_grad, splice_stream_t stream, void** out);
}

__global__ void pos_eff_kernel(float* pos_eff, const float* pos, const float* cls, const float* pe_bias, int T, int Tld, int D) {
    const size_t n = (size_t)Tld * D;
    for (size_t i = (size_t)blockIdx.x * blockDim.x + threadIdx.x; i < n; i += (size_t)gridDim.x * blockDim.x) {
        const int t = i / D, d = i % D;
        float v;
        if (t == 0) v = cls[d] + pos[d] - pe_bias[d];
        else if (t < T) v = pos[(size_t)t * D + d];
        else v = -pe_bias[d];
        pos_eff[i] = v;
    }
}

extern "C" {

int splice_vit_ctx_create(void* h, int B, int H, int W, const float* pos_TD, int need_grad, splice_stream_t stream, void** out) {
    SpliceVit* v = (SpliceVit*)h;
    hipStream_t s = (hipStream_t)stream;
    if (!v || !out || B < 1 || !splice_vit_params_complete(h)) {
        splice_set_error("splice_vit_ctx_create: bad handle / incomplete weights / B<1");
        return SPLICE_ERR_STATE;
    }
    const int p = v->patch, D = v->dim, Hd = v->hidden, pp3 = 3 * p * p;
    if (H < p || W < p) return SPLICE_ERR_ARG;
    SpliceVitCtx* c = new SpliceVitCtx();
    c->vit = v; c->B = B; c->H = H; c->W = W; c->need_grad = need_grad;
    c->T = 1 + (H / p) * (W / p);
    c->Tld = (c->T + 31) / 32 * 32;
    c->rows = B * c->Tld;
    const size_t rows = c->rows;
    const int L = v->depth;
    int rc = SPLICE_OK;
#define A(ptr, n) if (rc == SPLICE_OK) rc = dev_alloc(c->allocs, &(ptr), (size_t)(n))
    A(c->pos_eff, (size_t)c->Tld * D);
    A(c->patches, rows * pp3);
    c->xs.resize(L + 1); c->xmid.resize(L); c->mean1.resize(L); c->rstd1.resize(L); c->mean2.resize(L); c->rstd2.resize(L);
    c->qkv.resize(L); c->attn_out.resize(L); c->hpre.resize(L); c->lse.resize(L);
    for (int l = 0; l <= L; ++l) A(c->xs[l], rows * D);
    for (int l = 0; l < L; ++l) {
        A(c->xmid[l], rows * D);
        A(c->mean1[l], rows); A(c->rstd1[l], rows); A(c->mean2[l], rows); A(c->rstd2[l], rows);
        A(c->qkv[l], rows * 3 * D); A(c->attn_out[l], rows * D);
        A(c->hpre[l], rows * Hd);
        A(c->lse[l], (size_t)B * v->heads * c->Tld);
    }
    A(c->qkv_last_f32, rows * 3 * D);
    A(c->qkvT_last, rows * 3 * D);
    A(c->ln_out, rows * D);
    A(c->cls_attn, (size_t)B * D); A(c->cls_ln, (size_t)B * D); A(c->cls_h, (size_t)B * Hd); A(c->cls_probs, (size_t)B * v->heads * c->Tld);
    A(c->cls_slabs, (size_t)16 * B * Hd);
    if (need_grad) { A(c->cls_dh, (size_t)B * Hd); A(c->cls_dout, (size_t)B * D); A(c->cls_dln, (size_t)B * D); }
    A(c->hact, rows * Hd);
    if (need_grad) {
        A(c->g, rows * D); A(c->g_bf, rows * D); A(c->dh, rows * Hd); A(c->dln, rows * D * 4);
        A(c->dout, rows * D); A(c->dqkv, rows * 3 * D);
        A(c->delta, (size_t)B * v->heads * c->Tld);
        A(c->dpatches, rows * pp3);
    }
#undef A
    if (rc != SPLICE_OK) {
        for (void* q : c->allocs) (void)hipFree(q);
        delete c;
        return rc;
    }
    SPLICE_LAUNCH(pos_eff_kernel, dim3(grid_n((size_t)c->Tld * D)), dim3(256), 0, s, c->pos_eff, pos_TD, v->cls, v->pe.b, c->T, c->Tld, D);
    *out = c;
    return SPLICE_OK;
}

void splice_vit_ctx_destroy(void* ctx) {
    SpliceVitCtx* c = (SpliceVitCtx*)ctx;
    if (!c) return;
    for (void* p : c->allocs) (void)hipFree(p);
    delete c;
}

int splice_vit_ctx_info(void* ctx, int* T, int* Tld, int* rows) {
    SpliceVitCtx* c = (SpliceVitCtx*)ctx;
    if (!c) return SPLICE_ERR_ARG;
    if (T) *T = c->T;
    if (Tld) *Tld = c->Tld;
    if (rows) *rows = c->rows;
    return SPLICE_OK;
}

int splice_vit_ctx_set_top_cls_only(void* ctx, int on) {
    SpliceVitCtx* c = (SpliceVitCtx*)ctx;
    if (!c) return SPLICE_ERR_ARG;
    c->top_cls_only = on ? 1 : 0;
    return SPLICE_OK;
}

int splice_vit_ctx_set_fp8(void* ctx, int mode) {
    SpliceVitCtx* c = (SpliceVitCtx*)ctx;
    if (!c || mode < 0 || mode > 3 || mode == 2) return SPLICE_ERR_ARG;
    if (mode && !c->vit->fp8) { splice_set_error("splice_vit_ctx_set_fp8: the engine has no e4m3 weights (splice_vit_enable_fp8 first)"); return SPLICE_ERR_STATE; }
    const size_t rows = c->rows;
    if (mode && !c->ln_out8) {
        RC(dev_alloc(c->allocs, &c->ln_out8, rows * c->vit->dim));
        RC(dev_alloc(c->allocs, &c->ln_scale, rows));
        RC(dev_alloc(c->allocs, &c->hact8, rows * c->vit->hidden));
    }
    if ((mode & 2) && !c->qkv8) {
        RC(dev_alloc(c->allocs, &c->qkv8, rows * 3 * c->vit->dim));
        RC(dev_alloc(c->allocs, &c->qkvT8, rows * 3 * c->vit->dim));
    }
    c->fp8 = mode;
    return SPLICE_OK;
}

int splice_vit_ctx_dims(void* ctx, int* B, int* H, int* W, int* D, int* depth, int* heads, int* patch) {
    SpliceVitCtx* c = (SpliceVitCtx*)ctx;
    if (!c) return SPLICE_ERR_ARG;
    if (B) *B = c->B;
    if (H) *H = c->H;
    if (W) *W = c->W;
    if (D) *D = c->vit->dim;
    if (depth) *depth = c->vit->depth;
    if (heads) *heads = c->vit->heads;
    if (patch) *patch = c->vit->patch;
    return SPLICE_OK;
}

int splice_vit_forward_ex(void* ctx, const float* img, int normalize, int grad_pass_begin, splice_stream_t stream) {
    SpliceVitCtx* c = (SpliceVitCtx*)ctx;
    if (!c) return SPLICE_ERR_ARG;
    return splice_vit_forward_passes(ctx, img, normalize, grad_pass_begin, 0, c->B, stream);
}
int splice_vit_forward(void* ctx, const float* img, int normalize, splice_stream_t stream) {
    return splice_vit_forward_ex(ctx, img, normalize, 0, stream);
}
int splice_vit_forward_passes(void* ctx, const float* img, int normalize, int grad_pass_begin, int pass_begin, int pass_end,
                              splice_stream_t stream) {
    SpliceVitCtx* c = (SpliceVitCtx*)ctx;
    if (!c || !img || grad_pass_begin < 0 || grad_pass_begin > c->B || pass_begin < 0 || pass_end > c->B || pass_begin >= pass_end)
        return SPLICE_ERR_ARG;
    c->grad_pass_begin = grad_pass_begin;
    SpliceVit* v = c->vit;
    hipStream_t s = (hipStream_t)stream;
    const int D = v->dim, Hd = v->hidden, pp3 = 3 * v->patch * v->patch, L = v->depth;
    const int Bp = pass_end - pass_begin, R = Bp * c->Tld;
    const size_t r0 = (size_t)pass_begin * c->Tld;
    bf16_t* patches = c->patches + r0 * pp3;
    bf16_t* ln_out = c->ln_out + r0 * D;
    bf16_t* hact = c->hact + r0 * Hd;
    RC(patchify_launch(img + (size_t)pass_begin * 3 * c->H * c->W, patches, Bp, c->H, c->W, v->patch, c->Tld, normalize, s));
    {
        GemmEpi e = {};
        e.bias = v->pe.b; e.resid = c->pos_eff; e.ldr = D; e.resid_mod = c->Tld; e.out_f32 = c->xs[0] + r0 * D; e.ldo = D;
        RC(gemm_nt_launch(EPI_BIAS | EPI_RESID | EPI_OUT_F32, patches, pp3, v->pe.w, pp3, R, D, pp3, e, s));
    }
    for (int l = 0; l < L; ++l) {
        const LayerW& W = v->layers[l];
        float* x_in = c->xs[l] + r0 * D;
        float* x_mid = c->xmid[l] + r0 * D;
        const bool fp8 = (c->fp8 & 1) && c->ln_out8 && W.qkv.w8;
        const bool fp8_attn = fp8 && (c->fp8 & 2) && c->qkv8;
        {
            SpliceProfScope ps(10); SPLICE_DEV_REGION(1);
            if (fp8) RC(layernorm_fwd_fp8_launch(x_in, W.ln1_g, W.ln1_b, c->ln_out8 + r0 * D, c->ln_scale + r0, c->mean1[l] + r0, c->rstd1[l] + r0, R, D, 1e-6f, s));
            else RC(layernorm_fwd_launch(x_in, W.ln1_g, W.ln1_b, ln_out, c->mean1[l] + r0, c->rstd1[l] + r0, R, D, 1e-6f, s));
        }
        {
            GemmEpi e = {};
            e.bias = W.qkv.b; e.out_bf = c->qkv[l] + r0 * 3 * D; e.ldbf = 3 * D;
            unsigned fl = EPI_BIAS | EPI_OUT_BF;
            if (l == L - 1) {
                fl |= EPI_OUT_T | EPI_COLS_F32;
                e.out_bf_t = c->qkvT_last + r0; e.ldt = c->rows;
                e.out_f32_cols = c->qkv_last_f32 + r0 * 3 * D; e.ld_cols = 3 * D; e.col_lo = 0; e.col_hi = 3 * D;
            }
            SpliceProfScope ps(l == L - 1 ? 0 : 2); SPLICE_DEV_REGION(2);
            if (fp8) {
                e.row_scale = c->ln_scale + r0; e.col_scale = W.qkv.w8_scale;
                if (fp8_attn && !(l == L - 1 && c->top_cls_only)) {
                    fl |= EPI_OUT_F8 | EPI_OUT_F8T;
                    e.out_f8 = c->qkv8 + r0 * 3 * D; e.ld8 = 3 * D; e.out_f8_t = c->qkvT8 + r0; e.ldt8 = c->rows;
                }
                RC(gemm_nt_fp8_launch(fl | EPI_SCALE_RC, c->ln_out8 + r0 * D, D, W.qkv.w8, D, R, 3 * D, D, e, s));
            } else {
                RC(gemm_nt_launch(fl, ln_out, D, W.qkv.w, D, R, 3 * D, D, e, s));
            }
        }
        if (l == L - 1 && c->top_cls_only) {
            SPLICE_DEV_REGION(19);
            const int rs = c->Tld * D, hs = c->Tld * Hd;
            bf16_t* cattn = c->cls_attn + (size_t)pass_begin * D;
            bf16_t* cln = c->cls_ln + (size_t)pass_begin * D;
            bf16_t* ch = c->cls_h + (size_t)pass_begin * Hd;
            RC(attn_cls_fwd_launch(c->qkv[l] + r0 * 3 * D, c->qkvT_last + r0, c->rows, Bp, c->T, c->Tld, D, v->heads, v->qfold ? kLn2 : 0.125f, cattn,
                                   c->cls_probs + (size_t)pass_begin * v->heads * c->Tld, s));
            const size_t sstr = (size_t)c->B * Hd;
            float* slabs = c->cls_slabs + (size_t)pass_begin * Hd;
            auto ks_of = [](int K) { int n = K / 64, k = 16; while (k > 1 && n % k) --k; return k; };
            {
                GemmEpi e = {};
                e.out_f32 = slabs; e.ldo = D; e.ksplit = ks_of(D); e.slab_stride = (long long)sstr;
                RC(gemm_nt_launch(EPI_OUT_F32, cattn, D, W.proj.w, D, Bp, D, D, e, s));
                RC(ln_rows_fwd_launch(x_mid, rs, W.ln2_g, W.ln2_b, cln, D, c->mean2[l] + r0, c->rstd2[l] + r0, c->Tld, Bp, D, 1e-6f, slabs, e.ksplit, sstr,
                                      W.proj.b, x_in, rs, s));
            }
            {
                GemmEpi e = {};
                e.out_f32 = slabs; e.ldo = Hd; e.ksplit = ks_of(D); e.slab_stride = (long long)sstr;
                RC(gemm_nt_launch(EPI_OUT_F32, cln, D, W.fc1.w, D, Bp, Hd, D, e, s));
                const int lo = c->grad_pass_begin - pass_begin;
                RC(rows_finish_launch(1, slabs, e.ksplit, sstr, Bp, Hd, W.fc1.b, nullptr, 0, nullptr, 0, ch, c->need_grad ? c->hpre[l] + r0 * Hd : nullptr, nullptr, hs,
                                      lo > 0 ? lo : 0, s));
            }
            {
                GemmEpi e = {};
                e.out_f32 = slabs; e.ldo = D; e.ksplit = ks_of(Hd); e.slab_stride = (long long)sstr;
                RC(gemm_nt_launch(EPI_OUT_F32, ch, Hd, W.fc2.w, Hd, Bp, D, Hd, e, s));
                RC(rows_finish_launch(0, slabs, e.ksplit, sstr, Bp, D, W.fc2.b, x_mid, rs, c->xs[l + 1] + r0 * D, rs, nullptr, nullptr, nullptr, 0, 0, s));
            }
            continue;
        }
        {
            AttnArgs a = {};
            a.qkv = c->qkv[l] + r0 * 3 * D; a.B = Bp; a.T = c->T; a.Tld = c->Tld; a.D = D; a.H = v->heads;
            a.scale = v->qfold ? kLn2 : 0.125f; a.qfold = v->qfold; a.out = c->attn_out[l] + r0 * D; a.lse = c->lse[l] + (size_t)pass_begin * v->heads * c->Tld;
            if (fp8_attn) { a.qkv8 = c->qkv8 + r0 * 3 * D; a.qkvT8 = c->qkvT8 + r0; a.ldt8 = c->rows; }
            SpliceProfScope ps(3); SPLICE_DEV_REGION(3);
            RC(attn_fwd_launch(&a, s));
        }
        {
            GemmEpi e = {};
            e.bias = W.proj.b; e.resid = x_in; e.ldr = D; e.out_f32 = x_mid; e.ldo = D;
            SpliceProfScope ps(9); SPLICE_DEV_REGION(4);
            RC(gemm_nt_launch(EPI_BIAS | EPI_RESID | EPI_OUT_F32, c->attn_out[l] + r0 * D, D, W.proj.w, D, R, D, D, e, s));
        }
        {
            SpliceProfScope ps(10); SPLICE_DEV_REGION(1);
            if (fp8) RC(layernorm_fwd_fp8_launch(x_mid, W.ln2_g, W.ln2_b, c->ln_out8 + r0 * D, c->ln_scale + r0, c->mean2[l] + r0, c->rstd2[l] + r0, R, D, 1e-6f, s));
            else RC(layernorm_fwd_launch(x_mid, W.ln2_g, W.ln2_b, ln_out, c->mean2[l] + r0, c->rstd2[l] + r0, R, D, 1e-6f, s));
        }
        {
            GemmEpi e = {};
            e.bias = W.fc1.b; e.out_bf = hact; e.ldbf = Hd; e.out_pre = c->need_grad ? c->hpre[l] + r0 * Hd : nullptr; e.ldp = Hd;
            const long lo = (long)c->grad_pass_begin * c->Tld - (long)r0;
            e.pre_row_lo = lo > 0 ? (int)lo : 0;
            SpliceProfScope ps(1); SPLICE_DEV_REGION(5);
            if (fp8) {
                e.out_bf = nullptr; e.out_f8 = c->hact8 + r0 * Hd; e.ld8 = Hd;
                e.row_scale = c->ln_scale + r0; e.col_scale = W.fc1.w8_scale;
                RC(gemm_nt_fp8_launch(EPI_SCALE_RC | EPI_BIAS | EPI_GELU | EPI_OUT_F8, c->ln_out8 + r0 * D, D, W.fc1.w8, D, R, Hd, D, e, s));
            } else {
                RC(gemm_nt_launch(EPI_BIAS | EPI_GELU | EPI_OUT_BF, ln_out, D, W.fc1.w, D, R, Hd, D, e, s));
            }
        }
        {
            GemmEpi e = {};
            e.bias = W.fc2.b; e.resid = x_mid; e.ldr = D; e.out_f32 = c->xs[l + 1] + r0 * D; e.ldo = D;
// ... 17 lines not shown
    if (!c || !out || layer < 0 || layer >= c->vit->depth) return SPLICE_ERR_ARG;
    switch (kind) {
        case 0: *out = c->xs[layer + 1]; break;
        case 1: *out = c->qkv[layer]; break;
        case 2: *out = c->attn_out[layer]; break;
        case 3: *out = c->qkv_last_f32; break;
        case 4: *out = c->lse[layer]; break;
        case 5: *out = c->xs[0]; break;
        case 6: if (layer != c->vit->depth - 1) return SPLICE_ERR_ARG; *out = c->qkvT_last; break;
        case 7: *out = c->qkv[layer]; break;
        default: return SPLICE_ERR_ARG;
    }
    return SPLICE_OK;
}

int splice_vit_read_tensor(void* ctx, int kind, int layer, void* dst, size_t bytes, splice_stream_t stream) {
    void* src = nullptr;
    RC(splice_vit_get_tensor(ctx, kind, layer, &src));
    HIPCHK(hipMemcpyAsync(dst, src, bytes, hipMemcpyDeviceToDevice, (hipStream_t)stream));
    SpliceVitCtx* c = (SpliceVitCtx*)ctx;
    if (c->vit->qfold && (kind == 1 || kind == 3)) {
        const int D = c->vit->dim;
        const size_t rows = bytes / ((size_t)3 * D * (kind == 1 ? 2 : 4));
        if (kind == 1) hipLaunchKernelGGL(scale_cols_bf16_kernel, dim3(grid_n(rows * D)), dim3(256), 0, (hipStream_t)stream, (bf16_t*)dst, 3 * D, (int)rows, D, 1.0f / c->vit->qscale);
        else hipLaunchKernelGGL(scale_cols_f32_kernel, dim3(grid_n(rows * D)), dim3(256), 0, (hipStream_t)stream, (float*)dst, 3 * D, (int)rows, D, 1.0f / c->vit->qscale);
    }
    return SPLICE_OK;
}

int splice_vit_backward(void* ctx, int pass_begin, int pass_end, const float* const* d_block, const float* const* d_qkv,
                        const float* const* d_keys, float* d_img, int normalize, splice_stream_t stream) {
    SpliceVitCtx* c = (SpliceVitCtx*)ctx;
    if (!c || !c->need_grad || !c->forward_done || pass_begin < c->grad_pass_begin || pass_end > c->B || pass_begin >= pass_end || !d_img) {
        splice_set_error("splice_vit_backward: bad ctx / range / no forward / ctx created without need_grad");
        return SPLICE_ERR_STATE;
    }
    SpliceVit* v = c->vit;
    hipStream_t s = (hipStream_t)stream;
    const int D = v->dim, Hd = v->hidden, pp3 = 3 * v->patch * v->patch, L = v->depth;
    const size_t r0 = (size_t)pass_begin * c->Tld;
    const int R = (pass_end - pass_begin) * c->Tld;
    const int Bp = pass_end - pass_begin;
    float* g = c->g + r0 * D;
    bf16_t* g_bf = c->g_bf + r0 * D;
    bool g_live = false;
    const size_t slab = (size_t)c->rows * D;
    const int tiles1 = cdiv(c->Tld, 64) * cdiv(D, 64);
    const int ks = (tiles1 * 3 <= 640 && D % 192 == 0) ? 3 : (tiles1 <= 640 && D % 128 == 0) ? 2 : 1;
    for (int l = L - 1; l >= 0; --l) {
        const LayerW& W = v->layers[l];
        const float* db = d_block ? d_block[l] : nullptr;
        const float* dq = d_qkv ? d_qkv[l] : nullptr;
        const float* dk = d_keys ? d_keys[l] : nullptr;
        if (db) {
            SPLICE_LAUNCH(grad_stream_kernel, dim3(grid_n((size_t)R * D)), dim3(256), 0, s, g, g_bf, db + r0 * D, (size_t)R * D, g_live ? 0 : 1);
            g_live = true;
        }
        if (!g_live && !dq && !dk) continue;
        bf16_t* dqkv = c->dqkv + r0 * 3 * D;
        const float* g_after_mlp = nullptr;
        if (g_live && l == L - 1 && c->top_cls_only) {
            SPLICE_DEV_REGION(20);
            const int rs = c->Tld * D, hs = c->Tld * Hd;
            bf16_t* cdh = c->cls_dh + (size_t)pass_begin * Hd;
            const size_t sstr = (size_t)c->B * Hd;
            float* slabs = c->cls_slabs + (size_t)pass_begin * Hd;
            auto ks_of = [](int K) { int n = K / 64, k = 16; while (k > 1 && n % k) --k; return k; };
            {
                GemmEpi e = {};
                e.out_f32 = slabs; e.ldo = Hd; e.ksplit = ks_of(D); e.slab_stride = (long long)sstr;
                RC(gemm_nt_launch(EPI_OUT_F32, g_bf, rs, W.fc2.wT, D, Bp, Hd, D, e, s));
                RC(rows_finish_launch(2, slabs, e.ksplit, sstr, Bp, Hd, nullptr, nullptr, 0, nullptr, 0, cdh, nullptr, c->hpre[l] + r0 * Hd, hs, 0, s));
            }
            {
                GemmEpi e = {};
                e.out_f32 = slabs; e.ldo = D; e.ksplit = ks_of(Hd); e.slab_stride = (long long)sstr;
                RC(gemm_nt_launch(EPI_OUT_F32, cdh, Hd, W.fc1.wT, Hd, Bp, D, Hd, e, s));
                RC(ln_rows_bwd_launch(slabs, D, c->xmid[l] + r0 * D, rs, W.ln2_g, c->mean2[l] + r0, c->rstd2[l] + r0, c->Tld, g, g_bf, Bp, D, e.ksplit, sstr, s));
            }
            {
                GemmEpi e = {};
                e.out_f32 = slabs; e.ldo = D; e.ksplit = ks_of(D); e.slab_stride = (long long)sstr;
                RC(gemm_nt_launch(EPI_OUT_F32, g_bf, rs, W.proj.wT, D, Bp, D, D, e, s));
                RC(attn_cls_bwd_launch(c->qkv[l] + r0 * 3 * D, c->qkvT_last + r0, c->rows, Bp, c->T, c->Tld, D, v->heads, v->qfold ? kLn2 : 0.125f,
                                       c->cls_probs + (size_t)pass_begin * v->heads * c->Tld, slabs, e.ksplit, sstr, dqkv, s));
            }
            g_after_mlp = g;
        } else if (g_live) {
            {
                GemmEpi e = {};
                e.aux = c->hpre[l] + r0 * Hd; e.ldaux = Hd; e.out_bf = c->dh + r0 * Hd; e.ldbf = Hd;
                SpliceProfScope ps(11); SPLICE_DEV_REGION(7);
                RC(gemm_nt_launch(EPI_GELU_GRAD | EPI_OUT_BF, g_bf, D, W.fc2.wT, D, R, Hd, D, e, s));
            }
            {
                GemmEpi e = {};
                e.out_f32 = c->dln + r0 * D; e.ldo = D; e.ksplit = ks; e.slab_stride = (long long)slab;
                SpliceProfScope ps(5); SPLICE_DEV_REGION(8);
                RC(gemm_nt_launch(EPI_OUT_F32, c->dh + r0 * Hd, Hd, W.fc1.wT, Hd, R, D, Hd, e, s));
            }
            {
                SpliceProfScope ps(10); SPLICE_DEV_REGION(9);
                RC(layernorm_bwd_slabs_launch(c->dln + r0 * D, gemm_splitk_slabs(R, ks), slab, c->xmid[l] + r0 * D, W.ln2_g, c->mean2[l] + r0, c->rstd2[l] + r0, g, g, g_bf, R, D, s));
            }
            {
                GemmEpi e = {};
                e.out_bf = c->dout + r0 * D; e.ldbf = D;
                e.rd_other = c->attn_out[l] + r0 * D; e.ld_rd = D; e.rd_rows = c->Tld;
                e.rowdot = c->delta + (size_t)pass_begin * v->heads * c->Tld;
                SpliceProfScope ps(11); SPLICE_DEV_REGION(10);
                RC(gemm_nt_launch(EPI_OUT_BF | EPI_ROWDOT, g_bf, D, W.proj.wT, D, R, D, D, e, s));
            }
            {
                AttnArgs a = {};
                a.qkv = c->qkv[l] + r0 * 3 * D; a.B = Bp; a.T = c->T; a.Tld = c->Tld;
                a.D = D; a.H = v->heads; a.scale = v->qfold ? kLn2 : 0.125f; a.qfold = v->qfold; a.out = c->attn_out[l] + r0 * D;
                a.lse = c->lse[l] + (size_t)pass_begin * v->heads * c->Tld;
                a.dout = c->dout + r0 * D; a.doutT = nullptr; a.delta = c->delta + (size_t)pass_begin * v->heads * c->Tld; a.delta_ready = 1; a.dqkv = dqkv;
                SpliceProfScope ps(6); SPLICE_DEV_REGION(11);
                RC(attn_bwd_launch(&a, s));
            }
            g_after_mlp = g;
        } else {
            RC(dev_zero_launch(dqkv, (size_t)R * 3 * D * sizeof(bf16_t), s));
        }
        if (dq) SPLICE_LAUNCH(add_f32_into_bf16_kernel, dim3(grid_n((size_t)R * 3 * D)), dim3(256), 0, s, dqkv, 3 * D, 0, dq + r0 * 3 * D, 3 * D, R, 3 * D, v->qfold ? D : 0, 1.0f / v->qscale);
        if (dk) SPLICE_LAUNCH(add_f32_into_bf16_kernel, dim3(grid_n((size_t)R * D)), dim3(256), 0, s, dqkv, 3 * D, D, dk + r0 * D, D, R, D, 0, 1.0f);
        {
            GemmEpi e = {};
            e.out_f32 = c->dln + r0 * D; e.ldo = D; e.ksplit = ks; e.slab_stride = (long long)slab;
            SpliceProfScope ps(5); SPLICE_DEV_REGION(12);
            RC(gemm_nt_launch(EPI_OUT_F32, dqkv, 3 * D, W.qkv.wT, 3 * D, R, D, 3 * D, e, s));
        }
        {
            SpliceProfScope ps(10); SPLICE_DEV_REGION(9);
            RC(layernorm_bwd_slabs_launch(c->dln + r0 * D, gemm_splitk_slabs(R, ks), slab, c->xs[l] + r0 * D, W.ln1_g, c->mean1[l] + r0, c->rstd1[l] + r0, g_after_mlp, g, g_bf, R, D, s));
        }
        g_live = true;
    }
    if (!g_live) {
        RC(dev_zero_launch(d_img + (size_t)pass_begin * 3 * c->H * c->W, (size_t)Bp * 3 * c->H * c->W * sizeof(float), s));
        return SPLICE_OK;
    }
    {
        GemmEpi e = {};
        e.out_f32 = c->dpatches + r0 * pp3; e.ldo = pp3;
        RC(gemm_nt_launch(EPI_OUT_F32, g_bf, D, v->pe.wT, D, R, pp3, D, e, s));
    }
    RC(unpatchify_launch(c->dpatches + r0 * pp3, d_img + (size_t)pass_begin * 3 * c->H * c->W, Bp, c->H, c->W, v->patch, c->Tld, normalize, s));
    const hipError_t e = hipGetLastError();
    if (e != hipSuccess) { splice_set_error("splice_vit_backward: %s", hipGetErrorString(e)); return SPLICE_ERR_HIP; }
    return SPLICE_OK;
}
}
```

Measured before the change: 271.6.

## Fuse MSE terms, fold dk into CLS attention bwd, and trim transposed QKV stores

Adds a paired MSE kernel that computes the global CLS and identity MSE terms in one launch instead of two. It also folds the external key gradient into the CLS-only attention backward kernel, so a separate add pass is no longer needed. The top-layer QKV GEMM now writes the transposed output and f32 column copy only for the column ranges actually used, and the column store is vectorised to float4. These changes cut launch count and memory traffic, at the cost of new memsets at context creation and more epilogue branching.

```diff
diff --git a/include/splice_hip.h b/include/splice_hip.h
--- a/include/splice_hip.h
+++ b/include/splice_hip.h
@@ -48,6 +48,7 @@
     int ld8;
     uint8_t* out_f8_t;
     int ldt8;
+    int t_lo, t_hi;
 } splice_gemm_epilogue;
 
 enum {
@@ -320,6 +321,24 @@
 int splice_mse_pairs(const float* a, int lda, size_t a_ps, const float* b, int ldb, size_t b_ps, int rows, int cols, float loss_weight,
                      float grad_weight, float* part, size_t part_ps, float* grad, int ldg, size_t g_ps, int pairs, const float* grad_tab,
                      splice_stream_t stream);
+typedef struct splice_mse_term {
+    const float* a;
+    int lda;
+    size_t a_ps;
+    const float* b;
+    int ldb;
+    size_t b_ps;
+    int rows, cols;
+    float loss_weight, grad_weight;
+    float* part;
+    size_t part_ps;
+    float* grad;
+    int ldg;
+    size_t g_ps;
+    int pairs;
+    const float* grad_tab;
+} splice_mse_term;
+int splice_mse_pairs2(const splice_mse_term* terms, splice_stream_t stream);
 int splice_total_loss_pairs(float* lbase, size_t lstride, int lp, float w_ssim, float w_essim, float w_ecls, float w_cls, float w_id,
                             float* out8, int pairs, int n_a, int n_b, int n_c, int n_e, const float* wtab, int ssim_on, int entire,
                             splice_stream_t stream);
@@ -332,6 +351,8 @@
                         float* probs, splice_stream_t stream);
 int splice_attn_cls_bwd(const splice_bf16* qkv, const splice_bf16* qkvT, int ldt, int B, int T, int Tld, int D, int H, float scale, const float* probs,
                         const float* dout_slabs, int n_slabs, size_t slab_stride, splice_bf16* dqkv, splice_stream_t stream);
+int splice_attn_cls_bwd_dk(const splice_bf16* qkv, const splice_bf16* qkvT, int ldt, int B, int T, int Tld, int D, int H, float scale, const float* probs,
+                           const float* dout_slabs, int n_slabs, size_t slab_stride, const float* dk_add, splice_bf16* dqkv, splice_stream_t stream);
 int splice_ln_rows_fwd(float* x, size_t xs, const float* gamma, const float* beta, splice_bf16* y, size_t ys, float* mean, float* rstd, size_t ss,
                        int rows, int D, float eps, const float* slabs, int n_slabs, size_t slab_stride, const float* bias, const float* resid, size_t rs,
                        splice_stream_t stream);
diff --git a/splice_amd/_lib.py b/splice_amd/_lib.py
--- a/splice_amd/_lib.py
+++ b/splice_amd/_lib.py
@@ -21,6 +21,16 @@
         ("row_scale", C.c_void_p), ("col_scale", C.c_void_p),
         ("out_f8", C.c_void_p), ("ld8", C.c_int),
         ("out_f8_t", C.c_void_p), ("ldt8", C.c_int),
+        ("t_lo", C.c_int), ("t_hi", C.c_int),
+    ]
+
+
+class MseTerm(C.Structure):
+    _fields_ = [
+        ("a", C.c_void_p), ("lda", C.c_int), ("a_ps", C.c_size_t), ("b", C.c_void_p), ("ldb", C.c_int), ("b_ps", C.c_size_t),
+        ("rows", C.c_int), ("cols", C.c_int), ("loss_weight", C.c_float), ("grad_weight", C.c_float),
+        ("part", C.c_void_p), ("part_ps", C.c_size_t), ("grad", C.c_void_p), ("ldg", C.c_int), ("g_ps", C.c_size_t),
+        ("pairs", C.c_int), ("grad_tab", C.c_void_p),
     ]
 
 
@@ -140,9 +150,11 @@
     "splice_selfsim_loss_pairs_ws_bytes": ([_i, _i, _i], _sz),
     "splice_selfsim_loss_pairs": ([_vp, _vp, _i, _sz, _vp, _i, _sz, _i, _i, _i, _f, _vp, _i, _f, _vp, _sz, _vp, _i, _sz, _vp, _vp], _i),
     "splice_mse_pairs": ([_vp, _i, _sz, _vp, _i, _sz, _i, _i, _f, _f, _vp, _sz, _vp, _i, _sz, _i, _vp, _vp], _i),
+    "splice_mse_pairs2": ([_vp, _vp], _i),
     "splice_total_loss_pairs": ([_vp, _sz, _i, _f, _f, _f, _f, _f, _vp, _i, _i, _i, _i, _i, _vp, _i, _i, _vp], _i),
     "splice_attn_cls_fwd": ([_vp, _vp, _i, _i, _i, _i, _i, _i, _f, _vp, _vp, _vp], _i),
     "splice_attn_cls_bwd": ([_vp, _vp, _i, _i, _i, _i, _i, _i, _f, _vp, _vp, _i, _sz, _vp, _vp], _i),
+    "splice_attn_cls_bwd_dk": ([_vp, _vp, _i, _i, _i, _i, _i, _i, _f, _vp, _vp, _i, _sz, _vp, _vp, _vp], _i),
     "splice_ln_rows_fwd": ([_vp, _sz, _vp, _vp, _vp, _sz, _vp, _vp, _sz, _i, _i, _f, _vp, _i, _sz, _vp, _vp, _sz, _vp], _i),
     "splice_ln_rows_bwd": ([_vp, _sz, _vp, _sz, _vp, _vp, _vp, _sz, _vp, _vp, _i, _i, _i, _sz, _vp], _i),
     "splice_rows_finish": ([_i, _vp, _i, _sz, _i, _i, _vp, _vp, _sz, _vp, _sz, _vp, _vp, _vp, _sz, _i, _vp], _i),
diff --git a/splice_amd/csrc/capi.hip b/splice_amd/csrc/capi.hip
--- a/splice_amd/csrc/capi.hip
+++ b/splice_amd/csrc/capi.hip
@@ -158,6 +158,10 @@
                                      ST(stream), grad_tab),
                   "splice_mse_pairs");
 }
+int splice_mse_pairs2(const splice_mse_term* terms, splice_stream_t stream) {
+    if (!terms) return finish(SPLICE_ERR_ARG, "splice_mse_pairs2");
+    return finish(mse_pair_launch(terms, ST(stream)), "splice_mse_pairs2");
+}
 
 static bool attn_cls_args_ok(const void* qkv, const void* qkvT, int ldt, int B, int T, int Tld, int D, int H, size_t lds) {
     if (!qkv || !qkvT || B < 1 || T < 1 || T > Tld || Tld % 32 || ldt % 8 || (long long)ldt < (long long)B * Tld || D < 64 || D % 64 || H != D / 64)
@@ -180,6 +184,14 @@
         !attn_cls_args_ok(qkv, qkvT, ldt, B, T, Tld, D, H, ((size_t)Tld + Tld / 2 + 64 + 64 + 32 + 256 + 8) * sizeof(float)))
         return finish(SPLICE_ERR_ARG, who);
     return finish(attn_cls_bwd_launch(qkv, qkvT, ldt, B, T, Tld, D, H, scale, probs, dout_slabs, n_slabs, slab_stride, dqkv, ST(stream)), who);
+}
+int splice_attn_cls_bwd_dk(const splice_bf16* qkv, const splice_bf16* qkvT, int ldt, int B, int T, int Tld, int D, int H, float scale, const float* probs,
+                           const float* dout_slabs, int n_slabs, size_t slab_stride, const float* dk_add, splice_bf16* dqkv, splice_stream_t stream) {
+    const char* who = "splice_attn_cls_bwd_dk";
+    if (!probs || !dout_slabs || !dqkv || !dk_add || (reinterpret_cast<size_t>(dk_add) & 15) || n_slabs < 1 || n_slabs > 16 ||
+        !attn_cls_args_ok(qkv, qkvT, ldt, B, T, Tld, D, H, ((size_t)Tld + Tld / 2 + 64 + 64 + 32 + 256 + 8) * sizeof(float)))
+        return finish(SPLICE_ERR_ARG, who);
+    return finish(attn_cls_bwd_launch(qkv, qkvT, ldt, B, T, Tld, D, H, scale, probs, dout_slabs, n_slabs, slab_stride, dqkv, ST(stream), dk_add), who);
 }
 int splice_ln_rows_fwd(float* x, size_t xs, const float* gamma, const float* beta, splice_bf16* y, size_t ys, float* mean, float* rstd, size_t ss,
                        int rows, int D, float eps, const float* slabs, int n_slabs, size_t slab_stride, const float* bias, const float* resid, size_t rs,
diff --git a/splice_amd/csrc/gemm.h b/splice_amd/csrc/gemm.h
--- a/splice_amd/csrc/gemm.h
+++ b/splice_amd/csrc/gemm.h
@@ -374,7 +374,7 @@
         for (int r = 0; r < 4; ++r)
             if (row0 + r < M) e.out_bf[(size_t)(row0 + r) * e.ldbf + col] = f2bf(x[r]);
     }
-    if (FLAGS & EPI_OUT_T) {
+    if ((FLAGS & EPI_OUT_T) && col >= e.t_lo && col < e.t_hi) {
         bf16_t* p = e.out_bf_t + (size_t)col * e.ldt + row0;
         if (row0 + 3 < M) {
             uint2 pk = {pack2bf(x[0], x[1]), pack2bf(x[2], x[3])};
@@ -465,7 +465,7 @@
     if (FLAGS & EPI_OUT_T) {
 #pragma unroll
         for (int r = 0; r < 4; ++r)
-            if (col0 + r < N) e.out_bf_t[(size_t)(col0 + r) * e.ldt + row] = f2bf(x[r]);
+            if (col0 + r < N && col0 + r >= e.t_lo && col0 + r < e.t_hi) e.out_bf_t[(size_t)(col0 + r) * e.ldt + row] = f2bf(x[r]);
     }
     if (FLAGS & EPI_COLS_F32) {
 #pragma unroll
@@ -508,10 +508,15 @@
     if (inb) {
         if ((FLAGS & EPI_OUT_F32) && STORE_F32) *reinterpret_cast<float4*>(e.out_f32 + (size_t)row * e.ldo + col0) = float4{x[0], x[1], x[2], x[3]};
         if (FLAGS & EPI_COLS_F32) {
-#pragma unroll
-            for (int r = 0; r < 4; ++r) {
-                const int c = col0 + r;
-                if (c >= e.col_lo && c < e.col_hi) e.out_f32_cols[(size_t)row * e.ld_cols + (c - e.col_lo)] = x[r];
+            const bool vec = !((e.ld_cols | e.col_lo) & 3) && !(reinterpret_cast<uintptr_t>(e.out_f32_cols) & 15);
+            if (vec && col0 >= e.col_lo && col0 + 3 < e.col_hi) {
+                *reinterpret_cast<float4*>(e.out_f32_cols + (size_t)row * e.ld_cols + (col0 - e.col_lo)) = float4{x[0], x[1], x[2], x[3]};
+            } else {
+#pragma unroll
+                for (int r = 0; r < 4; ++r) {
+                    const int c = col0 + r;
+                    if (c >= e.col_lo && c < e.col_hi) e.out_f32_cols[(size_t)row * e.ld_cols + (c - e.col_lo)] = x[r];
+                }
             }
         }
     }
@@ -519,7 +524,7 @@
 }
 template <int BM, int BN, bool TRANSPOSED>
 __device__ __forceinline__ void gemm_stage_store(const f32x4 (&acc)[BM / 32][BN / 32], bf16_t* cs, bf16_t* out, int ld, int M, int N, int m0, int n0,
-                                                 int row_lo) {
+                                                 int row_lo, int row_hi = 0) {
     constexpr int FMt = BM / 32, FNt = BN / 32;
     constexpr int R = TRANSPOSED ? BN : BM, Cc = TRANSPOSED ? BM : BN, PITCH = Cc + 8;
     const int lane = threadIdx.x & 63, wave = threadIdx.x >> 6, wm = wave >> 1, wn = wave & 1;
@@ -544,7 +549,7 @@
         const int r = c / CH, k = (c % CH) * 8;
         const int gr = r0 + r, gc = c0 + k;
         if (gr >= Rm || gc >= Cm) continue;
-        if (!TRANSPOSED && gr < row_lo) continue;
+        if (TRANSPOSED ? (gr < row_lo || gr >= row_hi) : gr < row_lo) continue;
         const u32x4 v = *reinterpret_cast<const u32x4*>(cs + r * PITCH + k);
         bf16_t* q = out + (size_t)gr * ld + gc;
         if (gc + 7 < Cm && !(ld & 7)) st_out(reinterpret_cast<u32x4*>(q), v);
@@ -765,7 +770,7 @@
                     for (int r = 0; r < 4; ++r) tile.acc[i][j][r] = gelu_f(tile.acc[i][j][r]);
         }
         gemm_stage_store<BM, BN, false>(tile.acc, gemm_smem, e.out_bf, e.ldbf, M, N, m0, n0, 0);
-        if (FLAGS & EPI_OUT_T) gemm_stage_store<BM, BN, true>(tile.acc, gemm_smem, e.out_bf_t, e.ldt, M, N, m0, n0, 0);
+        if ((FLAGS & EPI_OUT_T) && n0 < e.t_hi && n0 + BN > e.t_lo) gemm_stage_store<BM, BN, true>(tile.acc, gemm_smem, e.out_bf_t, e.ldt, M, N, m0, n0, e.t_lo, e.t_hi);
         if constexpr ((FLAGS & EPI_OUT_F8) != 0) gemm_stage_store_f8<BM, BN>(tile.acc, reinterpret_cast<uint8_t*>(gemm_smem), e.out_f8, e.ld8, M, N, m0, n0);
         if constexpr ((FLAGS & EPI_OUT_F8T) != 0) gemm_stage_store_f8t<BM, BN>(tile.acc, reinterpret_cast<uint8_t*>(gemm_smem), e.out_f8_t, e.ldt8, M, N, m0, n0);
         if (FLAGS & EPI_ROWDOT) {
diff --git a/splice_amd/csrc/gemm.hip b/splice_amd/csrc/gemm.hip
--- a/splice_amd/csrc/gemm.hip
+++ b/splice_amd/csrc/gemm.hip
@@ -68,8 +68,15 @@
     return SPLICE_OK;
 }
 
+static inline GemmEpi epi_with_t_window(const GemmEpi& e_in, int N) {
+    GemmEpi e = e_in;
+    if (e.t_hi <= 0) { e.t_lo = 0; e.t_hi = N; }
+    return e;
+}
+
 int gemm_nt_launch(unsigned flags, const bf16_t* A, int lda, const bf16_t* B, int ldb, int M, int N, int K,
-                   const GemmEpi& e, hipStream_t s) {
+                   const GemmEpi& e_in, hipStream_t s) {
+    const GemmEpi e = epi_with_t_window(e_in, N);
     if (M < 1 || N < 1 || K < GEMM_BK || K % GEMM_BK || lda % 8 || ldb % 8) return SPLICE_ERR_ARG;
     if ((size_t)M * lda * sizeof(bf16_t) >= (1ull << 32) || (size_t)N * ldb * sizeof(bf16_t) >= (1ull << 32)) return SPLICE_ERR_ARG;
     if ((flags & EPI_OUT_T) && (e.ldt % 4)) return SPLICE_ERR_ARG;
@@ -109,7 +116,8 @@
     else launch_gemm_nt<64, 64, FLAGS, 3, true>(s, a, lda / 2, b, ldb / 2, M, N, K / 2, e);
     return SPLICE_OK;
 }
-int gemm_nt_fp8_launch(unsigned flags, const uint8_t* A, int lda, const uint8_t* B, int ldb, int M, int N, int K, const GemmEpi& e, hipStream_t s) {
+int gemm_nt_fp8_launch(unsigned flags, const uint8_t* A, int lda, const uint8_t* B, int ldb, int M, int N, int K, const GemmEpi& e_in, hipStream_t s) {
+    const GemmEpi e = epi_with_t_window(e_in, N);
     if (M < 1 || N < 1 || K < 128 || K % 128 || lda % 16 || ldb % 16) return SPLICE_ERR_ARG;
     if ((size_t)M * lda >= (1ull << 32) || (size_t)N * ldb >= (1ull << 32)) return SPLICE_ERR_ARG;
     if (!(flags & EPI_SCALE_RC) || !e.col_scale) return SPLICE_ERR_ARG;
diff --git a/splice_amd/csrc/kernels.h b/splice_amd/csrc/kernels.h
--- a/splice_amd/csrc/kernels.h
+++ b/splice_amd/csrc/kernels.h
@@ -31,7 +31,7 @@
 int attn_cls_fwd_launch(const bf16_t* qkv, const bf16_t* qkvT, int ldt, int B, int T, int Tld, int D, int H, float scale, bf16_t* out, float* probs,
                         hipStream_t s);
 int attn_cls_bwd_launch(const bf16_t* qkv, const bf16_t* qkvT, int ldt, int B, int T, int Tld, int D, int H, float scale, const float* probs,
-                        const float* dout_slabs, int n_slabs, size_t slab_stride, bf16_t* dqkv, hipStream_t s);
+                        const float* dout_slabs, int n_slabs, size_t slab_stride, bf16_t* dqkv, hipStream_t s, const float* dk_add = nullptr);
 int ln_rows_fwd_launch(float* x, size_t xs, const float* gamma, const float* beta, bf16_t* y, size_t ys, float* mean, float* rstd, size_t ss, int rows,
                        int D, float eps, const float* slabs, int n_slabs, size_t slab_stride, const float* bias, const float* resid, size_t rs, hipStream_t s);
 int ln_rows_bwd_launch(float* dy, size_t dys, const float* x, size_t xs, const float* gamma, const float* mean, const float* rstd, size_t ss, float* g,
@@ -113,6 +113,7 @@
 int mse_batched_launch(const float* a, int lda, size_t a_ps, const float* b, int ldb, size_t b_ps, int rows, int cols, float loss_weight,
                        float grad_weight, float* part, size_t part_ps, float* grad, int ldg, size_t g_ps, int pairs, hipStream_t s,
                        const float* grad_tab = nullptr);
+int mse_pair_launch(const splice_mse_term* two, hipStream_t s);
 int mse_launch(const float* a, int lda, const float* b, int ldb, int rows, int cols, float weight, float* loss_accum,
                float* grad, int ldg, hipStream_t s);
 #define SPLICE_MSE_PARTIALS 1024
diff --git a/splice_amd/csrc/selfsim.hip b/splice_amd/csrc/selfsim.hip
--- a/splice_amd/csrc/selfsim.hip
+++ b/splice_amd/csrc/selfsim.hip
@@ -483,30 +483,46 @@
     b->k8_x = (uint8_t*)p;
 }
 
+__device__ __forceinline__ void mse_term_body(const float* __restrict__ a, int lda, size_t a_ps, const float* __restrict__ bb, int ldb, size_t b_ps, int rows,
+                                              int cols, float wmean, float gmean, float* __restrict__ part, size_t part_ps, float* __restrict__ grad, int ldg,
+                                              size_t g_ps, const float* __restrict__ gtab, int pair, unsigned bx, unsigned gx, float* red) {
+    if (gtab) {
+        gmean = gtab[pair];
+        if (gmean == 0.f) return;
+    }
+    a += (size_t)pair * a_ps; bb += (size_t)pair * b_ps; part += (size_t)pair * part_ps;
+    if (grad) grad += (size_t)pair * g_ps;
+    const size_t n = (size_t)rows * cols;
+    float acc = 0.f;
+    for (size_t i = (size_t)bx * 256 + threadIdx.x; i < n; i += (size_t)gx * 256) {
+        const int r = i / cols, c = i % cols;
+        const float d = a[(size_t)r * lda + c] - bb[(size_t)r * ldb + c];
+        acc += d * d;
+        if (grad) grad[(size_t)r * ldg + c] = 2.0f * gmean * d;
+    }
+    acc = wave_sum(acc);
+    if ((threadIdx.x & 63) == 0) red[threadIdx.x >> 6] = acc;
+    __syncthreads();
+    if (threadIdx.x == 0) part[bx] = ((red[0] + red[1]) + (red[2] + red[3])) * wmean;
+}
 __global__ __launch_bounds__(256) void mse_batched_kernel(const float* __restrict__ a, int lda, size_t a_ps, const float* __restrict__ bb, int ldb,
                                                           size_t b_ps, int rows, int cols, float wmean, float gmean, float* __restrict__ part,
                                                           size_t part_ps, float* __restrict__ grad, int ldg, size_t g_ps,
                                                           const float* __restrict__ gtab) {
-    const int pair = blockIdx.y;
-    if (gtab) {
-        gmean = gtab[pair];
-        if (gmean == 0.f) return;
-    }
-    a += (size_t)pair * a_ps; bb += (size_t)pair * b_ps; part += (size_t)pair * part_ps;
-    if (grad) grad += (size_t)pair * g_ps;
-    const size_t n = (size_t)rows * cols;
-    float acc = 0.f;
-    for (size_t i = (size_t)blockIdx.x * 256 + threadIdx.x; i < n; i += (size_t)gridDim.x * 256) {
-        const int r = i / cols, c = i % cols;
-        const float d = a[(size_t)r * lda + c] - bb[(size_t)r * ldb + c];
-        acc += d * d;
-        if (grad) grad[(size_t)r * ldg + c] = 2.0f * gmean * d;
-    }
     __shared__ float red[4];
-    acc = wave_sum(acc);
-    if ((threadIdx.x & 63) == 0) red[threadIdx.x >> 6] = acc;
-    __syncthreads();
-    if (threadIdx.x == 0) part[blockIdx.x] = ((red[0] + red[1]) + (red[2] + red[3])) * wmean;
+    mse_term_body(a, lda, a_ps, bb, ldb, b_ps, rows, cols, wmean, gmean, part, part_ps, grad, ldg, g_ps, gtab, blockIdx.y, blockIdx.x, gridDim.x, red);
+}
+struct MsePairArgs {
+    splice_mse_term t[2];
+    unsigned wgs[2];
+};
+__global__ __launch_bounds__(256) void mse_pair_kernel(MsePairArgs p) {
+    __shared__ float red[4];
+    const int k = blockIdx.x >= p.wgs[0] ? 1 : 0;
+    const splice_mse_term& t = p.t[k];
+    if ((int)blockIdx.y >= t.pairs) return;
+    mse_term_body(t.a, t.lda, t.a_ps, t.b, t.ldb, t.b_ps, t.rows, t.cols, t.loss_weight, t.grad_weight, t.part, t.part_ps, t.grad, t.ldg, t.g_ps, t.grad_tab,
+                  blockIdx.y, blockIdx.x - (k ? p.wgs[0] : 0u), p.wgs[k], red);
 }
 int mse_batched_launch(const float* a, int lda, size_t a_ps, const float* b, int ldb, size_t b_ps, int rows, int cols, float loss_weight,
                        float grad_weight, float* part, size_t part_ps, float* grad, int ldg, size_t g_ps, int pairs, hipStream_t s,
@@ -519,3 +535,20 @@
                        grad_weight / (float)n, part, part_ps, grad, ldg, g_ps, grad_tab);
     return SPLICE_OK;
 }
+int mse_pair_launch(const splice_mse_term* two, hipStream_t s) {
+    MsePairArgs p = {};
+    int pairs = 0;
+    for (int k = 0; k < 2; ++k) {
+        const size_t n = (size_t)two[k].rows * two[k].cols;
+        if (two[k].rows < 1 || two[k].cols < 1 || !two[k].a || !two[k].b || !two[k].part || two[k].pairs < 1) return SPLICE_ERR_ARG;
+        size_t g = (n + 255) / 256;
+        if (g > MSE_MAX_WG) g = MSE_MAX_WG;
+        p.t[k] = two[k];
+        p.t[k].loss_weight = two[k].loss_weight / (float)n;
+        p.t[k].grad_weight = two[k].grad_weight / (float)n;
+        p.wgs[k] = (unsigned)g;
+        if (two[k].pairs > pairs) pairs = two[k].pairs;
+    }
+    SPLICE_LAUNCH(mse_pair_kernel, dim3(p.wgs[0] + p.wgs[1], pairs), dim3(256), 0, s, p);
+    return SPLICE_OK;
+}
diff --git a/splice_amd/csrc/step_engine.hip b/splice_amd/csrc/step_engine.hip
--- a/splice_amd/csrc/step_engine.hip
+++ b/splice_amd/csrc/step_engine.hip
@@ -877,7 +877,20 @@
     if (overlap) HIPCHK(hipStreamWaitEvent(s, st->ev(SpliceStep::EV_JOIN), 0));
     if (do_v) {
         if (t[L_GLOBAL_SSIM].on) RC(selfsim_loss_launch(sb, s));
-        if (t[L_GLOBAL_CLS].on) {
+        const bool mse_paired = t[L_GLOBAL_CLS].on && t[L_GLOBAL_ID].on && !(pairs > 1 && st->na != st->nb);
+        if (mse_paired) {
+            splice_mse_term two[2] = {};
+            two[0].a = blk_g + pX * passD; two[0].lda = vg.D; two[0].a_ps = passD; two[0].b = blk_g + pB * passD; two[0].ldb = vg.D; two[0].b_ps = passD;
+            two[0].rows = 1; two[0].cols = vg.D; two[0].loss_weight = 1.0f; two[0].grad_weight = t[L_GLOBAL_CLS].lambda;
+            two[0].part = loss_part(st, L_GLOBAL_CLS); two[0].part_ps = st->lstride; two[0].grad = vg.d_block + pX * passD; two[0].ldg = vg.D; two[0].g_ps = passD;
+            two[0].pairs = Pc; two[0].grad_tab = t[L_GLOBAL_CLS].tab;
+            two[1].a = keys_ptr(vg, qkv_g, pY); two[1].lda = 3 * vg.D; two[1].a_ps = 3 * passD; two[1].b = keys_ptr(vg, qkv_g, pB); two[1].ldb = 3 * vg.D;
+            two[1].b_ps = 3 * passD; two[1].rows = vg.T; two[1].cols = vg.D; two[1].loss_weight = 1.0f; two[1].grad_weight = t[L_GLOBAL_ID].lambda;
+            two[1].part = loss_part(st, L_GLOBAL_ID); two[1].part_ps = st->lstride; two[1].grad = vg.d_keys + pY * passD; two[1].ldg = vg.D; two[1].g_ps = passD;
+            two[1].pairs = Pb; two[1].grad_tab = t[L_GLOBAL_ID].tab;
+            RC(mse_pair_launch(two, s));
+        }
+        if (t[L_GLOBAL_CLS].on && !mse_paired) {
             if (pairs > 1 && st->na != st->nb) {
                 for (int i = 0; i < nc; ++i)
                     RC(mse_batched_launch(blk_g + (pX + i) * passD, vg.D, st->na * passD, blk_g + (pB + i) * passD, vg.D, st->nb * passD, 1, vg.D, 1.0f,
@@ -888,7 +901,7 @@
                                       loss_part(st, L_GLOBAL_CLS), st->lstride, vg.d_block + pX * passD, vg.D, passD, Pc, s, t[L_GLOBAL_CLS].tab));
             }
         }
-        if (t[L_GLOBAL_ID].on)
+        if (t[L_GLOBAL_ID].on && !mse_paired)
             RC(mse_batched_launch(keys_ptr(vg, qkv_g, pY), 3 * vg.D, 3 * passD, keys_ptr(vg, qkv_g, pB), 3 * vg.D, 3 * passD, vg.T, vg.D, 1.0f, t[L_GLOBAL_ID].lambda,
                                   loss_part(st, L_GLOBAL_ID), st->lstride, vg.d_keys + pY * passD, vg.D, passD, Pb, s, t[L_GLOBAL_ID].tab));
     }
diff --git a/splice_amd/csrc/vit_cls.hip b/splice_amd/csrc/vit_cls.hip
--- a/splice_amd/csrc/vit_cls.hip
+++ b/splice_amd/csrc/vit_cls.hip
@@ -106,9 +106,10 @@
     if (threadIdx.x < 64) out[(size_t)b * D + h * 64 + threadIdx.x] = f2bf((po[threadIdx.x] + po[64 + threadIdx.x]) + (po[128 + threadIdx.x] + po[192 + threadIdx.x]));
 }
 
+template <bool DK>
 __global__ __launch_bounds__(256) void attn_cls_bwd_kernel(const bf16_t* __restrict__ qkv, const bf16_t* __restrict__ qkvT, int ldt, int T, int Tld, int D,
                                                            float scale, const float* __restrict__ probs, const float* __restrict__ dout ,
-                                                           int n_slabs, size_t slab_stride, bf16_t* __restrict__ dqkv) {
+                                                           int n_slabs, size_t slab_stride, bf16_t* __restrict__ dqkv, const float* __restrict__ dk_add) {
     extern __shared__ __attribute__((aligned(16))) float cls_smem[];
     float* ds = cls_smem;
     uint32_t* dsb = reinterpret_cast<uint32_t*>(ds + Tld);
@@ -172,6 +173,13 @@
             dl += pj4[u] * s;
         }
     }
+    float4 ka[16];
+    const int j_first = (int)threadIdx.x + 256 * z;
+    if (DK && j_first < Tld) {
+        const float4* ar = reinterpret_cast<const float4*>(dk_add + (row0 + j_first) * D + h * 64);
+#pragma unroll
+        for (int c = 0; c < 16; ++c) ka[c] = ar[c];
+    }
     const float delta = block_sum256(dl, red);
     for (int j = threadIdx.x; j < Tld; j += 256) {
         const float pj = j < T ? pg[j] : 0.f;
@@ -182,6 +190,26 @@
         u32x4* rq = reinterpret_cast<u32x4*>(r);
         u32x4* rk = reinterpret_cast<u32x4*>(r + D);
         u32x4* rv = reinterpret_cast<u32x4*>(r + 2 * D);
+        if (DK && j != j_first) {
+            const float4* ar = reinterpret_cast<const float4*>(dk_add + (row0 + j) * D + h * 64);
+#pragma unroll
+            for (int c = 0; c < 16; ++c) ka[c] = ar[c];
+        }
+        if (DK) {
+#pragma unroll
+            for (int c = 0; c < 8; ++c) {
+                if (j != 0) rq[c] = u32x4{0u, 0u, 0u, 0u};
+                const float4 a0 = ka[2 * c], a1 = ka[2 * c + 1];
+                auto kv = [&](int i, float add) { return bf2f(j < T ? f2bf(dsj * q[8 * c + i]) : (bf16_t)0) + add; };
+                rk[c] = u32x4{pack2bf(kv(0, a0.x), kv(1, a0.y)), pack2bf(kv(2, a0.z), kv(3, a0.w)), pack2bf(kv(4, a1.x), kv(5, a1.y)),
+                              pack2bf(kv(6, a1.z), kv(7, a1.w))};
+                if (j >= T) rv[c] = u32x4{0u, 0u, 0u, 0u};
+                else
+                    rv[c] = u32x4{pack2bf(pj * dO[8 * c], pj * dO[8 * c + 1]), pack2bf(pj * dO[8 * c + 2], pj * dO[8 * c + 3]),
+                                  pack2bf(pj * dO[8 * c + 4], pj * dO[8 * c + 5]), pack2bf(pj * dO[8 * c + 6], pj * dO[8 * c + 7])};
+            }
+            continue;
+        }
 #pragma unroll 2
         for (int c = 0; c < 8; ++c) {
             if (j != 0) rq[c] = u32x4{0u, 0u, 0u, 0u};
@@ -229,11 +257,14 @@
     return SPLICE_OK;
 }
 int attn_cls_bwd_launch(const bf16_t* qkv, const bf16_t* qkvT, int ldt, int B, int T, int Tld, int D, int H, float scale, const float* probs,
-                        const float* dout_slabs, int n_slabs, size_t slab_stride, bf16_t* dqkv, hipStream_t s) {
-    if (D / 64 != H || D % 64 || n_slabs < 1 || n_slabs > 16) return SPLICE_ERR_ARG;
+                        const float* dout_slabs, int n_slabs, size_t slab_stride, bf16_t* dqkv, hipStream_t s, const float* dk_add) {
+    if (D / 64 != H || D % 64 || n_slabs < 1 || n_slabs > 16 || (reinterpret_cast<size_t>(dk_add) & 15)) return SPLICE_ERR_ARG;
     const size_t lds = (size_t)(Tld + Tld / 2 + 64 + 64 + 32 + 256 + 8) * sizeof(float);
     const int nz = Tld > 768 ? 4 : Tld > 256 ? 2 : 1;
-    SPLICE_LAUNCH(attn_cls_bwd_kernel, dim3(H, B, nz), dim3(256), lds, s, qkv, qkvT, ldt, T, Tld, D, scale, probs, dout_slabs, n_slabs, slab_stride, dqkv);
+    if (dk_add)
+        SPLICE_LAUNCH(attn_cls_bwd_kernel<true>, dim3(H, B, nz), dim3(256), lds, s, qkv, qkvT, ldt, T, Tld, D, scale, probs, dout_slabs, n_slabs, slab_stride, dqkv, dk_add);
+    else
+        SPLICE_LAUNCH(attn_cls_bwd_kernel<false>, dim3(H, B, nz), dim3(256), lds, s, qkv, qkvT, ldt, T, Tld, D, scale, probs, dout_slabs, n_slabs, slab_stride, dqkv, dk_add);
     return SPLICE_OK;
 }
 
diff --git a/splice_amd/csrc/vit_engine.hip b/splice_amd/csrc/vit_engine.hip
--- a/splice_amd/csrc/vit_engine.hip
+++ b/splice_amd/csrc/vit_engine.hip
@@ -305,6 +305,10 @@
         return rc;
     }
     SPLICE_LAUNCH(pos_eff_kernel, dim3(grid_n((size_t)c->Tld * D)), dim3(256), 0, s, c->pos_eff, pos_TD, v->cls, v->pe.b, c->T, c->Tld, D);
+    if (hipMemsetAsync(c->qkv_last_f32, 0, rows * 3 * D * sizeof(float), s) != hipSuccess || hipMemsetAsync(c->qkvT_last, 0, rows * 3 * D * sizeof(bf16_t), s) != hipSuccess) {
+        splice_vit_ctx_destroy(c);
+        return SPLICE_ERR_HIP;
+    }
     *out = c;
     return SPLICE_OK;
 }
@@ -410,6 +414,10 @@
                 fl |= EPI_OUT_T | EPI_COLS_F32;
                 e.out_bf_t = c->qkvT_last + r0; e.ldt = c->rows;
                 e.out_f32_cols = c->qkv_last_f32 + r0 * 3 * D; e.ld_cols = 3 * D; e.col_lo = 0; e.col_hi = 3 * D;
+                if (c->top_cls_only && !fp8) {
+                    e.out_f32_cols += D; e.col_lo = D; e.col_hi = 2 * D;
+                    e.t_lo = D; e.t_hi = 3 * D;
+                }
             }
             SpliceProfScope ps(l == L - 1 ? 0 : 2); SPLICE_DEV_REGION(2);
             if (fp8) {
@@ -593,8 +601,10 @@
                 GemmEpi e = {};
                 e.out_f32 = slabs; e.ldo = D; e.ksplit = ks_of(D); e.slab_stride = (long long)sstr;
                 RC(gemm_nt_launch(EPI_OUT_F32, g_bf, rs, W.proj.wT, D, Bp, D, D, e, s));
+                const bool fold_dk = dk && !dq && !(reinterpret_cast<size_t>(dk + r0 * D) & 15);
                 RC(attn_cls_bwd_launch(c->qkv[l] + r0 * 3 * D, c->qkvT_last + r0, c->rows, Bp, c->T, c->Tld, D, v->heads, v->qfold ? kLn2 : 0.125f,
-                                       c->cls_probs + (size_t)pass_begin * v->heads * c->Tld, slabs, e.ksplit, sstr, dqkv, s));
+                                       c->cls_probs + (size_t)pass_begin * v->heads * c->Tld, slabs, e.ksplit, sstr, dqkv, s, fold_dk ? dk + r0 * D : nullptr));
+                if (fold_dk) dk = nullptr;
             }
             g_after_mlp = g;
         } else if (g_live) {
```

Result: no change. 273.4 (median of 6 runs) (+0.7%).
